# ebanalyse/ebnerd-benchmark

Hardware: AMD Instinct MI355X
Metric: training impressions/sec (higher is better)
Workload: dtype f32

## Files before the change

ebnerd-benchmark_amd/csrc/ebn_attention_mfma.hip:

```cpp
#include <stdlib.h>

#include "ebn_common.h"

namespace {

typedef float f32x16 __attribute__((ext_vector_type(16)));

constexpr int ATT_WAVES = 4;

struct MfmaAttnArgs {
  const float* qkv;
  int64_t ld_qkv;
  const float* dout;
  int64_t ld_dout;
  float* out;
  int64_t ld_out;
  int64_t n_prob;
  int32_t L, h;
  const uint32_t* key_ptr;
  uint32_t thresh;
  float scale;
  const float* pool_w;
  const float* pool_d;
  int64_t ld_pool;
// ... 268 lines not shown
  p.row0 = static_cast<int64_t>(p.seq) * L;
  return p;
}

template <int D>
__host__ __device__ constexpr int fwd_wave_floats(int L) {
  return L * Tile<D>::STRIDE > TP_FLOATS ? L * Tile<D>::STRIDE : TP_FLOATS;
}

template <int D, int LC>
__global__ __launch_bounds__(64 * ATT_WAVES) void attn_mfma_fwd_kernel(MfmaAttnArgs a) {
  extern __shared__ __attribute__((aligned(16))) float smem[];
  const int lane = threadIdx.x & 63;
  const int wv = __builtin_amdgcn_readfirstlane(threadIdx.x >> 6);
  const int64_t prob = static_cast<int64_t>(xcd_chunked_block()) * ATT_WAVES + wv;
  if (prob >= a.n_prob) return;
  const int L = LC ? LC : a.L, E = a.h * D;
  float* sv = smem + wv * fwd_wave_floats<D>(L);
  const int row = lane & 31, hi = lane >> 5;
  const float inv2 = 1.44269504088896341f / sqrtf(static_cast<float>(D));
  const bool drop = a.key_ptr != nullptr;
  const uint32_t key = drop ? *a.key_ptr : 0u;

  const AttnProb p = attn_prob(prob, a.h, L);
  const float* qb = a.qkv + p.row0 * a.ld_qkv + p.head * D;
  float qr[D / 2], kr[D / 2];
  {
    Staged<D> tv;
    stage_load<D>(tv, qb + 2 * E, a.ld_qkv, L, lane);
    global_row_form<D>(qr, qb, a.ld_qkv, L, row, hi);
    global_row_form<D>(kr, qb + E, a.ld_qkv, L, row, hi);
    stage_store<D, false>(sv, tv, L, lane, 0u, 0u, 0, 0u, 0.f);
  }
  wave_lds_sync();
  float vc[16];
  lds_col_form<D>(vc, sv, L, row, hi);

  f32x16 P = mm_rows<D / 2>(kr, qr);
  softmax_in_lane(P, L, hi, inv2);
  wave_lds_sync();
  tile_transpose(P, sv, L, row, hi);
  const f32x16 O = mm_col_tile(vc, P);
  float* ob = a.out + p.row0 * a.ld_out + p.head * D;
  const uint64_t e0 = static_cast<uint64_t>(p.row0) * E + p.head * D;
  if (drop) tile_rows_to_global<D, true>(ob, a.ld_out, O, L, row, hi, 1.0f, key, e0, E, a.thresh, a.scale);
  else tile_rows_to_global<D, false>(ob, a.ld_out, O, L, row, hi, 1.0f, 0u, 0u, 0, 0u, 0.f);
}

template <int D>
__host__ __device__ constexpr int fwd_group_v_offset(int L) {
  return 2 * L * Tile<D>::STRIDE > TP_FLOATS ? 2 * L * Tile<D>::STRIDE : TP_FLOATS;
}
__host__ __device__ constexpr int group_tile_pad(int L);
template <int D>
__host__ __device__ constexpr int fwd_group_wave_floats(int L) {
  return fwd_group_v_offset<D>(L) + L * Tile<D>::STRIDE + group_tile_pad(L);
}

template <int D, int LC, int G>
__global__ __launch_bounds__(64 * G) void attn_mfma_fwd_group_kernel(MfmaAttnArgs a) {
  using T = Tile<D>;
  constexpr int NT = 64 * G;
  constexpr int GV = G * T::VPR;
  constexpr int ROUNDS = (32 * GV + NT - 1) / NT;
  extern __shared__ __attribute__((aligned(16))) float smem[];
  const int tid = threadIdx.x;
  const int lane = tid & 63;
  const int wv = __builtin_amdgcn_readfirstlane(tid >> 6);
  const int L = LC ? LC : a.L, E = a.h * D;
  const int region = L * T::STRIDE;
  const int wave_floats = fwd_group_wave_floats<D>(L), v_off = fwd_group_v_offset<D>(L);
  const int row = lane & 31, hi = lane >> 5;
  const float inv2 = 1.44269504088896341f / sqrtf(static_cast<float>(D));
  const bool drop = a.key_ptr != nullptr;
  const uint32_t key = drop ? *a.key_ptr : 0u;

  const AttnProb p0 = attn_prob(static_cast<int64_t>(xcd_chunked_block()) * G, a.h, L);
  const uint32_t gcol = p0.head * D;
  const float* gq = a.qkv + p0.row0 * a.ld_qkv + gcol;
  const int nvec = L * GV;
  {
    float4 vq[ROUNDS], vk[ROUNDS], vv[ROUNDS];
    uint32_t dst[ROUNDS];
#pragma unroll
    for (int t = 0; t < ROUNDS; ++t) {
      const int idx = tid + NT * t;
      const int idc = idx < nvec ? idx : 0;
      const uint32_t r = static_cast<uint32_t>(idc) / static_cast<uint32_t>(GV), c4g = static_cast<uint32_t>(idc) - r * GV;
      const uint32_t head = c4g / T::VPR, c4 = c4g - head * T::VPR;
      dst[t] = head * wave_floats + r * T::STRIDE + c4 * 4;
      const uint32_t off = r * static_cast<uint32_t>(a.ld_qkv) + c4g * 4;
      vq[t] = *reinterpret_cast<const float4*>(gq + off);
      vk[t] = *reinterpret_cast<const float4*>(gq + E + off);
      vv[t] = *reinterpret_cast<const float4*>(gq + 2 * E + off);
    }
#pragma unroll
    for (int t = 0; t < ROUNDS; ++t) {
      if (tid + NT * t < nvec) {
        *reinterpret_cast<float4*>(smem + dst[t]) = vq[t];
        *reinterpret_cast<float4*>(smem + dst[t] + region) = vk[t];
        *reinterpret_cast<float4*>(smem + dst[t] + v_off) = vv[t];
      }
    }
  }
  __syncthreads();

  float* sq = smem + wv * wave_floats;
  float* sk = sq + region;
  float* sv = sq + v_off;
  f32x16 P;
  {
    float qr[D / 2], kr[D / 2];
    lds_row_form<D>(qr, sq, L, row, hi);
    lds_row_form<D>(kr, sk, L, row, hi);
    P = mm_rows<D / 2>(kr, qr);
  }
  float vc[16];
  lds_col_form<D>(vc, sv, L, row, hi);
  softmax_in_lane(P, L, hi, inv2);
  wave_lds_sync();
  tile_transpose(P, sq, L, row, hi);
  {
    const f32x16 O = mm_col_tile(vc, P);
    tile_rows_to_lds<D>(sv, O, L, row, hi, 1.0f);
  }
  __syncthreads();

  float* go = a.out + p0.row0 * a.ld_out + gcol;
#pragma unroll
  for (int t = 0; t < ROUNDS; ++t) {
    const int idx = tid + NT * t;
    if (idx < nvec) {
      const uint32_t r = static_cast<uint32_t>(idx) / static_cast<uint32_t>(GV), c4g = static_cast<uint32_t>(idx) - r * GV;
      const uint32_t head = c4g / T::VPR, c4 = c4g - head * T::VPR;
      float4 y = *reinterpret_cast<const float4*>(smem + head * wave_floats + v_off + r * T::STRIDE + c4 * 4);
      if (drop) {
        const uint64_t pr = ((static_cast<uint64_t>(p0.row0) * E + gcol) >> 1) + ((r * static_cast<uint32_t>(E) + c4g * 4) >> 1);
        const uint32_t h0 = ebn_dropout_pair_hash(key, pr), h1 = ebn_dropout_pair_hash(key, pr + 1);
        y.x *= ((h0 & 0xFFFFu) >= a.thresh) ? a.scale : 0.f;
        y.y *= ((h0 >> 16) >= a.thresh) ? a.scale : 0.f;
        y.z *= ((h1 & 0xFFFFu) >= a.thresh) ? a.scale : 0.f;
        y.w *= ((h1 >> 16) >= a.thresh) ? a.scale : 0.f;
      }
      *reinterpret_cast<float4*>(go + (r * static_cast<uint32_t>(a.ld_out) + c4g * 4)) = y;
    }
  }
}

template <int D>
__host__ __device__ constexpr int bwd_wave_floats(int L) {
  return 3 * L * Tile<D>::STRIDE > L * Tile<D>::STRIDE + TP_FLOATS ? 3 * L * Tile<D>::STRIDE : L * Tile<D>::STRIDE + TP_FLOATS;
}

template <int D, int LC>
__global__ __launch_bounds__(64 * ATT_WAVES) void attn_mfma_bwd_kernel(MfmaAttnArgs a) {
  using T = Tile<D>;
  constexpr int KH = D / 2;
  extern __shared__ __attribute__((aligned(16))) float smem[];
  const int lane = threadIdx.x & 63;
  const int wv = __builtin_amdgcn_readfirstlane(threadIdx.x >> 6);
  const int64_t prob = static_cast<int64_t>(xcd_chunked_block()) * ATT_WAVES + wv;
  if (prob >= a.n_prob) return;
  const int L = LC ? LC : a.L, E = a.h * D;
  const int region = L * T::STRIDE;
  float* sq = smem + wv * bwd_wave_floats<D>(L);
  float* sk = sq + region;
  float* sg = sk + region;
  const int row = lane & 31, hi = lane >> 5;
  const float inv = 1.0f / sqrtf(static_cast<float>(D));
  const float inv2 = inv * 1.44269504088896341f;
  const bool drop = a.key_ptr != nullptr, pooled = a.pool_w != nullptr;
  const uint32_t key = drop ? *a.key_ptr : 0u;

  const AttnProb p = attn_prob(prob, a.h, L);
  const float* qb = a.qkv + p.row0 * a.ld_qkv + p.head * D;
  float vr[KH];
  {
    Staged<D> tq, tk, tg;
    stage_load<D>(tq, qb, a.ld_qkv, L, lane);
    stage_load<D>(tk, qb + E, a.ld_qkv, L, lane);
    stage_load<D>(tg, a.dout + p.row0 * a.ld_dout + p.head * D, a.ld_dout, L, lane);
    global_row_form<D>(vr, qb + 2 * E, a.ld_qkv, L, row, hi);
    if (pooled) {
      PoolTerm<D> pt;
      pool_load<D>(pt, a.pool_w + p.row0, a.pool_d + p.seq * a.ld_pool + p.head * D, L, lane);
      pool_add<D>(tg, pt);
    }
    stage_store<D, false>(sq, tq, L, lane, 0u, 0u, 0, 0u, 0.f);
    stage_store<D, false>(sk, tk, L, lane, 0u, 0u, 0, 0u, 0.f);
    if (drop) stage_store<D, true>(sg, tg, L, lane, key, static_cast<uint64_t>(p.row0) * E + p.head * D, E, a.thresh, a.scale);
    else stage_store<D, false>(sg, tg, L, lane, 0u, 0u, 0, 0u, 0.f);
  }
  wave_lds_sync();

  float* ob = a.out + p.row0 * a.ld_out + p.head * D;
  f32x16 P, dP;
  {
    float qr[KH], kr[KH];
    lds_row_form<D>(qr, sq, L, row, hi);
    lds_row_form<D>(kr, sk, L, row, hi);
    P = mm_rows<KH>(kr, qr);
  }
  softmax_in_lane(P, L, hi, inv2);
  {
    float gr[KH];
    lds_row_form<D>(gr, sg, L, row, hi);
    dP = mm_rows<KH>(gr, vr);
  }
  float rowdot = 0.f;
#pragma unroll
  for (int r = 0; r < 16; ++r) rowdot = fmaf(P[r], dP[r], rowdot);
  rowdot += __shfl_xor(rowdot, 32, 64);

  float col[16];
  lds_col_form<D>(col, sg, L, row, hi);
  {
    const f32x16 dV = mm_col_tile(col, P);
    tile_rows_to_global<D, false>(ob + 2 * E, a.ld_out, dV, L, row, hi, 1.0f, 0u, 0u, 0, 0u, 0.f);
  }
#pragma unroll
  for (int r = 0; r < 16; ++r) P[r] = P[r] * (dP[r] - rowdot);
  lds_col_form<D>(col, sk, L, row, hi);
  {
    const f32x16 dQ = mm_col_tile(col, P);
    tile_rows_to_global<D, false>(ob, a.ld_out, dQ, L, row, hi, inv, 0u, 0u, 0, 0u, 0.f);
  }
  wave_lds_sync();
  tile_transpose(P, sk, L, row, hi);
  lds_col_form<D>(col, sq, L, row, hi);
  {
    const f32x16 dK = mm_col_tile(col, P);
    tile_rows_to_global<D, false>(ob + E, a.ld_out, dK, L, row, hi, inv, 0u, 0u, 0, 0u, 0.f);
  }
}


template <int D>
__host__ __device__ constexpr int bwd_group_g_offset(int L) {
  return 2 * L * Tile<D>::STRIDE > TP_FLOATS ? 2 * L * Tile<D>::STRIDE : TP_FLOATS;
}
__host__ __device__ constexpr int group_tile_pad(int L) { return L == 30 ? 12 : 0; }
template <int D>
__host__ __device__ constexpr int bwd_group_wave_floats(int L) {
  return bwd_group_g_offset<D>(L) + L * Tile<D>::STRIDE + group_tile_pad(L);
}

template <int D, int LC, int G>
__global__ __launch_bounds__(64 * G) void attn_mfma_bwd_group_kernel(MfmaAttnArgs a) {
  using T = Tile<D>;
  constexpr int KH = D / 2;
  constexpr int NT = 64 * G;
  constexpr int GV = G * T::VPR;
  constexpr int ROUNDS = (32 * GV + NT - 1) / NT;
  extern __shared__ __attribute__((aligned(16))) float smem[];
  const int tid = threadIdx.x;
  const int lane = tid & 63;
  const int wv = __builtin_amdgcn_readfirstlane(tid >> 6);
  const int L = LC ? LC : a.L, E = a.h * D;
  const int region = L * T::STRIDE;
  const int wave_floats = bwd_group_wave_floats<D>(L), g_off = bwd_group_g_offset<D>(L);
  const int row = lane & 31, hi = lane >> 5;
  const float inv = 1.0f / sqrtf(static_cast<float>(D));
  const float inv2 = inv * 1.44269504088896341f;
  const bool drop = a.key_ptr != nullptr, pooled = a.pool_w != nullptr;
  const uint32_t key = drop ? *a.key_ptr : 0u;

  stagger_first_round(a);
  const AttnProb p0 = attn_prob(static_cast<int64_t>(xcd_chunked_block()) * G, a.h, L);
  const uint32_t gcol = p0.head * D;
  const float* gq = a.qkv + p0.row0 * a.ld_qkv + gcol;
  const float* gd = a.dout + p0.row0 * a.ld_dout + gcol;
  const int nvec = L * GV;
  float vr[KH];
  global_row_form<D>(vr, gq + 2 * E + wv * D, a.ld_qkv, L, row, hi);
  {
    float4 vq[ROUNDS], vk[ROUNDS], vg[ROUNDS];
    uint32_t dst[ROUNDS];
#pragma unroll
    for (int t = 0; t < ROUNDS; ++t) {
      const int idx = tid + NT * t;
      const int idc = idx < nvec ? idx : 0;
      const uint32_t r = static_cast<uint32_t>(idc) / static_cast<uint32_t>(GV), c4g = static_cast<uint32_t>(idc) - r * GV;
      const uint32_t head = c4g / T::VPR, c4 = c4g - head * T::VPR;
      dst[t] = head * wave_floats + r * T::STRIDE + c4 * 4;
      const uint32_t off = r * static_cast<uint32_t>(a.ld_qkv) + c4g * 4;
      vq[t] = *reinterpret_cast<const float4*>(gq + off);
      vk[t] = *reinterpret_cast<const float4*>(gq + E + off);
      vg[t] = *reinterpret_cast<const float4*>(gd + (r * static_cast<uint32_t>(a.ld_dout) + c4g * 4));
      if (pooled) {
        const float w = a.pool_w[p0.row0 + r];
        const float4 pd = *reinterpret_cast<const float4*>(a.pool_d + p0.seq * a.ld_pool + gcol + c4g * 4);
        vg[t].x = fmaf(w, pd.x, vg[t].x);
        vg[t].y = fmaf(w, pd.y, vg[t].y);
        vg[t].z = fmaf(w, pd.z, vg[t].z);
        vg[t].w = fmaf(w, pd.w, vg[t].w);
      }
      if (drop) {
        const uint64_t pr = ((static_cast<uint64_t>(p0.row0) * E + gcol) >> 1) + ((r * static_cast<uint32_t>(E) + c4g * 4) >> 1);
        const uint32_t h0 = ebn_dropout_pair_hash(key, pr), h1 = ebn_dropout_pair_hash(key, pr + 1);
        vg[t].x *= ((h0 & 0xFFFFu) >= a.thresh) ? a.scale : 0.f;
        vg[t].y *= ((h0 >> 16) >= a.thresh) ? a.scale : 0.f;
        vg[t].z *= ((h1 & 0xFFFFu) >= a.thresh) ? a.scale : 0.f;
        vg[t].w *= ((h1 >> 16) >= a.thresh) ? a.scale : 0.f;
      }
    }
#pragma unroll
    for (int t = 0; t < ROUNDS; ++t) {
      if (tid + NT * t < nvec) {
        *reinterpret_cast<float4*>(smem + dst[t]) = vq[t];
        *reinterpret_cast<float4*>(smem + dst[t] + region) = vk[t];
        *reinterpret_cast<float4*>(smem + dst[t] + g_off) = vg[t];
      }
    }
  }
  __syncthreads();

  float* sq = smem + wv * wave_floats;
  float* sk = sq + region;
  float* sg = sq + g_off;
  f32x16 P, dP;
  {
    float qr[KH], kr[KH];
    lds_row_form<D>(qr, sq, L, row, hi);
    lds_row_form<D>(kr, sk, L, row, hi);
    P = mm_rows<KH>(kr, qr);
  }
  softmax_in_lane(P, L, hi, inv2);
  {
    float gr[KH];
    lds_row_form<D>(gr, sg, L, row, hi);
    dP = mm_rows<KH>(gr, vr);
  }
  float rowdot = 0.f;
#pragma unroll
  for (int r = 0; r < 16; ++r) rowdot = fmaf(P[r], dP[r], rowdot);
  rowdot += __shfl_xor(rowdot, 32, 64);

  float col[16], colq[16];
  lds_col_form<D>(col, sg, L, row, hi);
  lds_col_form<D>(colq, sq, L, row, hi);
  wave_lds_sync();
  {
    const f32x16 dV = mm_col_tile(col, P);
    tile_rows_to_lds<D>(sg, dV, L, row, hi, 1.0f);
  }
#pragma unroll
  for (int r = 0; r < 16; ++r) P[r] = P[r] * (dP[r] - rowdot);
  lds_col_form<D>(col, sk, L, row, hi);
  const f32x16 dQ = mm_col_tile(col, P);
  wave_lds_sync();
  tile_transpose(P, sq, L, row, hi);
  wave_lds_sync();
  tile_rows_to_lds<D>(sq, dQ, L, row, hi, inv);
  {
    const f32x16 dK = mm_col_tile(colq, P);
    tile_rows_to_lds<D>(sk, dK, L, row, hi, inv);
  }
  __syncthreads();

  float* go = a.out + p0.row0 * a.ld_out + gcol;
#pragma unroll
  for (int t = 0; t < ROUNDS; ++t) {
    const int idx = tid + NT * t;
    if (idx < nvec) {
      const uint32_t r = static_cast<uint32_t>(idx) / static_cast<uint32_t>(GV), c4g = static_cast<uint32_t>(idx) - r * GV;
      const uint32_t head = c4g / T::VPR, c4 = c4g - head * T::VPR;
      const float* src = smem + head * wave_floats + r * T::STRIDE + c4 * 4;
      const float4 q4 = *reinterpret_cast<const float4*>(src);
      const float4 k4 = *reinterpret_cast<const float4*>(src + region);
      const float4 v4 = *reinterpret_cast<const float4*>(src + g_off);
      float* d = go + (r * static_cast<uint32_t>(a.ld_out) + c4g * 4);
      *reinterpret_cast<float4*>(d) = q4;
      *reinterpret_cast<float4*>(d + E) = k4;
      *reinterpret_cast<float4*>(d + 2 * E) = v4;
    }
  }
}


constexpr int ATT2_WAVES = 2;
constexpr int NB2 = 2;

__device__ __forceinline__ void mm_col_tile_acc(f32x16& acc, const float (&a)[16], const f32x16& z) {
#pragma unroll
  for (int s = 0; s < 16; ++s) acc = __builtin_amdgcn_mfma_f32_32x32x2f32(a[s], z[s], acc, 0, 0, 0);
}
// ... 246 lines not shown
        const float rdi = __shfl(rowdot[ib], crow(r, hi), 64);
        P[r] = P[r] * (dP[r] - rdi);
      }
      float col[16];
      lds_col_form<D>(col, sq + 32 * ib * T::STRIDE, L - 32 * ib, row, hi);
      mm_col_tile_acc(dK, col, P);
    }
    wave_lds_sync();
    tile_rows_to_lds<D>(sv + 32 * jb * T::STRIDE, dK, L - 32 * jb, row, hi, inv);
    wave_lds_sync();
    stage_out<D, false>(sv + 32 * jb * T::STRIDE, ob + E + 32 * jb * a.ld_out, a.ld_out, L - 32 * jb, lane, 0u, 0u, 0, 0u, 0.f);
  }
}

}

constexpr int BWD_GROUP = 4;
constexpr int64_t FWD_GROUP_MIN_QKV_BYTES = 200'000'000;
constexpr int64_t BWD_GROUP_MIN_PROBLEMS = 4096;
static uint32_t stagger_shift_of_device() {
  static const uint32_t shift = [] {
    int dev = 0, cus = 0;
    if (hipGetDevice(&dev) != hipSuccess || hipDeviceGetAttribute(&cus, hipDeviceAttributeMultiprocessorCount, dev) != hipSuccess) return 0u;
    if (cus < 16 || (cus & (cus - 1)) != 0) return 0u;
    uint32_t s = 0;
    while ((1 << s) < cus) ++s;
    return s;
  }();
  return shift;
}

static bool bwd_group_off() {
  static const bool off = [] { const char* e = getenv("EBN_ATTN_BWD_PER_WAVE"); return e && e[0] == '1'; }();
  return off;
}

static bool mfma_path_ok(int32_t L, int32_t d, int64_t lda, int64_t ldb, int64_t ldc, const void* p0,
                         const void* p1, const void* p2) {
  if (L > 64 || !(d == 16 || d == 20 || d == 32)) return false;
  if ((lda % 4) || (ldb % 4) || (ldc % 4)) return false;
  if (lda >= (1 << 24) || ldb >= (1 << 24) || ldc >= (1 << 24)) return false;
  return ebn_aligned16(p0) && ebn_aligned16(p1) && ebn_aligned16(p2);
}

template <class K>
static void allow_lds(K kernel, size_t bytes) {
  if (bytes > 64 * 1024) (void)hipFuncSetAttribute(reinterpret_cast<const void*>(kernel), hipFuncAttributeMaxDynamicSharedMemorySize, static_cast<int>(bytes));
}

template <class K>
static void launch_waves(K kernel, size_t lds, const MfmaAttnArgs& a, hipStream_t s) {
#ifdef EBN_ATTN_EXP_PAD_LDS
  static const size_t pad = getenv("EBN_ATTN_PAD_LDS") ? static_cast<size_t>(atol(getenv("EBN_ATTN_PAD_LDS"))) : 0;
  lds += pad;
#endif
  allow_lds(kernel, lds);
  EBN_LAUNCH(kernel, dim3(static_cast<unsigned>(ebn_ceil_div(a.n_prob, ATT_WAVES))), dim3(64 * ATT_WAVES), lds, s, a);
}

template <int D, int LC>
static void launch_mfma2_lc(bool bwd, const MfmaAttnArgs& a, hipStream_t s) {
  const dim3 grid(static_cast<unsigned>(ebn_ceil_div(a.n_prob, ATT2_WAVES))), block(64 * ATT2_WAVES);
  const size_t lds = static_cast<size_t>(ATT2_WAVES) * (bwd ? 4 : 3) * a.L * Tile<D>::STRIDE * sizeof(float);
  if (bwd) {
    allow_lds(attn_mfma2_bwd_kernel<D, LC>, lds);
    EBN_LAUNCH((attn_mfma2_bwd_kernel<D, LC>), grid, block, lds, s, a);
  } else {
    allow_lds(attn_mfma2_fwd_kernel<D, LC>, lds);
    EBN_LAUNCH((attn_mfma2_fwd_kernel<D, LC>), grid, block, lds, s, a);
  }
}

template <int D>
static void launch_mfma2(bool bwd, const MfmaAttnArgs& a, hipStream_t s) {
  if (D == 20 && a.L == 50 && !bwd) launch_mfma2_lc<D, 50>(bwd, a, s);
  else launch_mfma2_lc<D, 0>(bwd, a, s);
}

int ebn_attn_mfma_fwd(const float* qkv, int64_t ld_qkv, float* out, int64_t ld_out, int64_t n_seq, int32_t L,
                      int32_t h, int32_t d, const EbnDrop& dr, hipStream_t s, bool* handled) {
  *handled = mfma_path_ok(L, d, ld_qkv, ld_out, ld_out, qkv, out, out) && n_seq * h < (int64_t{1} << 31);
  if (!*handled) return EBN_OK;
  MfmaAttnArgs a{qkv, ld_qkv, nullptr, 0, out, ld_out, n_seq * h, L, h, dr.key_ptr, dr.thresh, dr.scale, nullptr, nullptr, 0, 0u, 0u, 1u};
  if (L > 32) {
    if (d == 16) launch_mfma2<16>(false, a, s);
    else if (d == 20) launch_mfma2<20>(false, a, s);
    else launch_mfma2<32>(false, a, s);
    EBN_CHECK_LAUNCH();
    return EBN_OK;
  }
  const bool big = a.n_prob * L * 3 * d * static_cast<int64_t>(sizeof(float)) >= FWD_GROUP_MIN_QKV_BYTES;
  if (d == 20 && (h % BWD_GROUP) == 0 && big && !bwd_group_off()) {
    const size_t lds = static_cast<size_t>(BWD_GROUP) * fwd_group_wave_floats<20>(L) * sizeof(float);
    const dim3 grid(static_cast<unsigned>(a.n_prob / BWD_GROUP)), block(64 * BWD_GROUP);
    if (L == 30) {
      allow_lds(attn_mfma_fwd_group_kernel<20, 30, BWD_GROUP>, lds);
      EBN_LAUNCH((attn_mfma_fwd_group_kernel<20, 30, BWD_GROUP>), grid, block, lds, s, a);
    } else {
      allow_lds(attn_mfma_fwd_group_kernel<20, 0, BWD_GROUP>, lds);
      EBN_LAUNCH((attn_mfma_fwd_group_kernel<20, 0, BWD_GROUP>), grid, block, lds, s, a);
    }
    EBN_CHECK_LAUNCH();
    return EBN_OK;
  }
  const size_t wb = static_cast<size_t>(ATT_WAVES) * sizeof(float);
  if (d == 16) launch_waves(attn_mfma_fwd_kernel<16, 0>, wb * fwd_wave_floats<16>(L), a, s);
  else if (d == 20 && L == 30) launch_waves(attn_mfma_fwd_kernel<20, 30>, wb * fwd_wave_floats<20>(L), a, s);
  else if (d == 20 && L == 20) launch_waves(attn_mfma_fwd_kernel<20, 20>, wb * fwd_wave_floats<20>(L), a, s);
  else if (d == 20) launch_waves(attn_mfma_fwd_kernel<20, 0>, wb * fwd_wave_floats<20>(L), a, s);
  else launch_waves(attn_mfma_fwd_kernel<32, 0>, wb * fwd_wave_floats<32>(L), a, s);
  EBN_CHECK_LAUNCH();
  return EBN_OK;
}

int ebn_attn_mfma_bwd(const float* qkv, int64_t ld_qkv, const float* dout, int64_t ld_dout, float* dqkv,
                      int64_t ld_dqkv, int64_t n_seq, int32_t L, int32_t h, int32_t d, const EbnDrop& dr,
                      hipStream_t s, bool* handled, const float* pool_w, const float* pool_d, int64_t ld_pool) {
  *handled = mfma_path_ok(L, d, ld_qkv, ld_dout, ld_dqkv, qkv, dout, dqkv) && n_seq * h < (int64_t{1} << 31) &&
             (pool_w == nullptr || ((ld_pool % 4) == 0 && ebn_aligned16(pool_d)));
  if (!*handled) return EBN_OK;
  MfmaAttnArgs a{qkv, ld_qkv, dout, ld_dout, dqkv, ld_dqkv, n_seq * h, L, h, dr.key_ptr, dr.thresh, dr.scale, pool_w, pool_d, ld_pool, 0u, 0u, 1u};
  if (L > 32) {
    if (d == 16) launch_mfma2<16>(true, a, s);
    else if (d == 20) launch_mfma2<20>(true, a, s);
    else launch_mfma2<32>(true, a, s);
    EBN_CHECK_LAUNCH();
    return EBN_OK;
  }
  if (d == 20 && (h % BWD_GROUP) == 0 && a.n_prob >= BWD_GROUP_MIN_PROBLEMS && !bwd_group_off()) {
    const size_t lds = static_cast<size_t>(BWD_GROUP) * bwd_group_wave_floats<20>(L) * sizeof(float);
    const dim3 grid(static_cast<unsigned>(a.n_prob / BWD_GROUP)), block(64 * BWD_GROUP);
    a.stagger_shift = stagger_shift_of_device();
    a.stagger_units = a.stagger_shift != 0u ? 7u : 0u;
    a.stagger_mod = 5u;
    if (L == 30) {
      allow_lds(attn_mfma_bwd_group_kernel<20, 30, BWD_GROUP>, lds);
      EBN_LAUNCH((attn_mfma_bwd_group_kernel<20, 30, BWD_GROUP>), grid, block, lds, s, a);
    } else {
      allow_lds(attn_mfma_bwd_group_kernel<20, 0, BWD_GROUP>, lds);
      EBN_LAUNCH((attn_mfma_bwd_group_kernel<20, 0, BWD_GROUP>), grid, block, lds, s, a);
    }
    EBN_CHECK_LAUNCH();
    return EBN_OK;
  }
  const size_t wb = static_cast<size_t>(ATT_WAVES) * sizeof(float);
  if (d == 16) launch_waves(attn_mfma_bwd_kernel<16, 0>, wb * bwd_wave_floats<16>(L), a, s);
  else if (d == 20 && L == 30) launch_waves(attn_mfma_bwd_kernel<20, 30>, wb * bwd_wave_floats<20>(L), a, s);
  else if (d == 20 && L == 20) launch_waves(attn_mfma_bwd_kernel<20, 20>, wb * bwd_wave_floats<20>(L), a, s);
  else if (d == 20) launch_waves(attn_mfma_bwd_kernel<20, 0>, wb * bwd_wave_floats<20>(L), a, s);
  else launch_waves(attn_mfma_bwd_kernel<32, 0>, wb * bwd_wave_floats<32>(L), a, s);
  EBN_CHECK_LAUNCH();
  return EBN_OK;
}
```

ebnerd-benchmark_amd/csrc/ebn_encoder.hip:

```cpp
#include "ebn_common.h"

#define EBN_TRY(call)            \
  do {                           \
    int rc__ = (call);           \
    if (rc__ != EBN_OK) return rc__; \
  } while (0)

static int check_dims(const ebn_encoder_dims* d) {
  EBN_REQUIRE(d, EBN_ERR_BAD_ARG);
  EBN_REQUIRE(d->n_seq >= 0 && d->L > 0 && d->Din > 0 && d->h > 0 && d->d > 0 && d->A > 0, EBN_ERR_BAD_ARG);
  return EBN_OK;
}

extern "C" int ebn_encoder_fwd_f32(const ebn_encoder_dims* dims, const ebn_encoder_params* p,
                                   const ebn_encoder_acts* a, const ebn_encoder_scratch* s,
                                   const ebn_step_state* st, ebn_stream_t stream) {
  EBN_TRY(check_dims(dims));
  EBN_REQUIRE(p && a && p->Wqkv && p->W && p->b && p->q, EBN_ERR_BAD_ARG);
  EBN_REQUIRE(a->X && a->QKV && a->Y && a->U && a->w && a->out, EBN_ERR_BAD_ARG);
  const int64_t R = dims->n_seq * dims->L;
  const int E = dims->h * dims->d;
  if (R == 0) return EBN_OK;
  float* ws = s ? s->gemm_ws : nullptr;
  const int64_t ws_n = s ? s->gemm_ws_floats : 0;
  EBN_TRY(ebn_gemm_f32_site(0, 0, R, 3 * E, dims->Din, 1.0f, a->X, dims->Din, p->Wqkv, 3 * E, 0.0f, a->QKV, 3 * E, ws, ws_n,
                            1, stream));
  EBN_TRY(ebn_attn_fwd_f32(a->QKV, 3 * E, a->Y, E, dims->n_seq, dims->L, dims->h, dims->d, st, dims->drop_site,
                           dims->drop_p, stream));
  EBN_TRY(ebn_gemm_f32_ws(0, 0, R, dims->A, E, 1.0f, a->Y, E, p->W, dims->A, 0.0f, a->U, dims->A, ws, ws_n, stream));
  EBN_TRY(ebn_attpool_fwd_f32(a->U, p->b, p->q, a->Y, a->out, a->w, dims->n_seq, dims->L, E, dims->A, stream));
  return EBN_OK;
}

extern "C" int ebn_encoder_fwd_gather_f32(const ebn_encoder_dims* dims, const ebn_encoder_params* p, const ebn_encoder_acts* a,
                                          const ebn_encoder_scratch* s, const int32_t* ids, const float* table, int64_t table_rows,
                                          int32_t* oob_flag, ebn_stream_t stream) {
  EBN_TRY(check_dims(dims));
  EBN_REQUIRE(p && a && ids && table && p->Wqkv && p->W && p->b && p->q, EBN_ERR_BAD_ARG);
  EBN_REQUIRE(a->QKV && a->Y && a->U && a->w && a->out, EBN_ERR_BAD_ARG);
  EBN_REQUIRE(dims->drop_p <= 0.0f, EBN_ERR_UNSUPPORTED);
  const int64_t R = dims->n_seq * dims->L;
  const int E = dims->h * dims->d;
  if (R == 0) return EBN_OK;
  float* ws = s ? s->gemm_ws : nullptr;
  const int64_t ws_n = s ? s->gemm_ws_floats : 0;
  EBN_TRY(ebn_gemm_f32_rowmap(ids, table_rows, R, 3 * E, dims->Din, table, dims->Din, p->Wqkv, 3 * E, a->QKV, 3 * E, oob_flag, stream));
  EBN_TRY(ebn_attn_fwd_f32(a->QKV, 3 * E, a->Y, E, dims->n_seq, dims->L, dims->h, dims->d, nullptr, -1, 0.0f, stream));
  EBN_TRY(ebn_gemm_f32_ws(0, 0, R, dims->A, E, 1.0f, a->Y, E, p->W, dims->A, 0.0f, a->U, dims->A, ws, ws_n, stream));
  EBN_TRY(ebn_attpool_fwd_f32(a->U, p->b, p->q, a->Y, a->out, a->w, dims->n_seq, dims->L, E, dims->A, stream));
  return EBN_OK;
}

extern "C" int ebn_encoder_bwd_f32(const ebn_encoder_dims* dims, const ebn_encoder_params* p,
                                   const ebn_encoder_acts* a, const float* dout, const ebn_encoder_grads* g,
                                   const ebn_encoder_scratch* s, float* dX, int32_t accumulate,
                                   const ebn_step_state* st, ebn_stream_t stream) {
  EBN_TRY(check_dims(dims));
  EBN_REQUIRE(p && a && g && s && dout, EBN_ERR_BAD_ARG);
  EBN_REQUIRE(p->Wqkv && p->W && p->q, EBN_ERR_BAD_ARG);
  EBN_REQUIRE(a->X && a->QKV && a->Y && a->U && a->w, EBN_ERR_BAD_ARG);
  EBN_REQUIRE(g->dWqkv && g->dW && g->db && g->dq, EBN_ERR_BAD_ARG);
  EBN_REQUIRE(s->dY && s->dQKV && s->de && s->partials, EBN_ERR_BAD_ARG);
  const int64_t R = dims->n_seq * dims->L;
  const int E = dims->h * dims->d;
  const int A = dims->A;
  if (R == 0) return EBN_OK;
  const float beta = accumulate ? 1.0f : 0.0f;
  EBN_TRY(ebn_attpool_bwd_pool_f32(a->Y, a->w, dout, nullptr, s->de, dims->n_seq, dims->L, E, stream));
  EBN_TRY(ebn_attpool_bwd_dpre_f32(a->U, p->q, s->de, g->dq, g->db, s->partials, R, A, accumulate, stream));
  const bool fold = ebn_attn_bwd_pooled_supported(dims->L, dims->d) != 0 && (E % 4) == 0 && ebn_aligned16(dout) &&
                    ebn_aligned16(s->dY) && ebn_aligned16(a->QKV) && ebn_aligned16(s->dQKV);
  if (fold) {
    EBN_TRY(ebn_dense_bwd_pair_f32(R, E, A, a->Y, E, a->U, A, p->W, A, beta, g->dW, A, s->dY, E, s->gemm_ws, s->gemm_ws_floats,
                                   stream));
    EBN_TRY(ebn_attn_bwd_pooled_f32(a->QKV, 3 * E, s->dY, E, a->w, dout, E, s->dQKV, 3 * E, dims->n_seq, dims->L, dims->h,
                                    dims->d, st, dims->drop_site, dims->drop_p, stream));
  } else {
    EBN_TRY(ebn_gemm_f32_ws(1, 0, E, A, R, 1.0f, a->Y, E, a->U, A, beta, g->dW, A, s->gemm_ws, s->gemm_ws_floats, stream));
    EBN_TRY(ebn_gemm_f32_rank1(R, E, A, 1.0f, a->U, A, p->W, A, s->dY, E, a->w, dout, E, dims->L, s->gemm_ws,
                               s->gemm_ws_floats, stream));
    EBN_TRY(ebn_attn_bwd_f32(a->QKV, 3 * E, s->dY, E, s->dQKV, 3 * E, dims->n_seq, dims->L, dims->h, dims->d, st, dims->drop_site,
                             dims->drop_p, stream));
  }
  if (dX != nullptr)
    return ebn_dense_bwd_pair_f32(R, dims->Din, 3 * E, a->X, dims->Din, s->dQKV, 3 * E, p->Wqkv, 3 * E, beta, g->dWqkv, 3 * E, dX,
                                  dims->Din, s->gemm_ws, s->gemm_ws_floats, stream);
  EBN_TRY(ebn_gemm_f32_ws(1, 0, dims->Din, 3 * E, R, 1.0f, a->X, dims->Din, s->dQKV, 3 * E, beta, g->dWqkv, 3 * E,
                          s->gemm_ws, s->gemm_ws_floats, stream));
  return EBN_OK;
}

extern "C" int ebn_user_stage_train_f32(const ebn_encoder_dims* dims, const ebn_encoder_params* p, const ebn_encoder_acts* a,
                                        const float* cand, const float* labels, float* scores, float* probs, float* loss_rows,
                                        float* loss_out, float* dcand, float* duser, const ebn_encoder_grads* g,
                                        const ebn_encoder_scratch* s, float* head_partials, float* dX, int32_t C,
                                        int32_t loss_kind, float inv_batch, const ebn_step_state* st, ebn_stream_t stream) {
  EBN_TRY(check_dims(dims));
  EBN_REQUIRE(p && a && g && s && cand && labels && scores && probs && loss_rows && loss_out && dcand && duser && dX, EBN_ERR_BAD_ARG);
  EBN_REQUIRE(p->Wqkv && p->W && p->b && p->q && a->X && a->QKV && a->Y && a->U && a->w && a->out, EBN_ERR_BAD_ARG);
  EBN_REQUIRE(g->dWqkv && g->dW && g->db && g->dq && s->dY && s->dQKV && s->de && s->partials, EBN_ERR_BAD_ARG);
  EBN_REQUIRE(C > 0 && dims->drop_p <= 0.0f, EBN_ERR_BAD_ARG);
  const int64_t B = dims->n_seq, R = dims->n_seq * dims->L;
  const int E = dims->h * dims->d, A = dims->A, L = dims->L;
  if (R == 0) return EBN_OK;
  const bool fused = head_partials != nullptr && ebn_user_head_supported(L, C, E, A) != 0 &&
                     ebn_attn_bwd_pooled_supported(L, dims->d) != 0 && ebn_aligned16(a->U) && ebn_aligned16(a->Y) &&
                     ebn_aligned16(cand) && ebn_aligned16(dcand) && ebn_aligned16(duser) && ebn_aligned16(a->out) &&
                     ebn_aligned16(p->b) && ebn_aligned16(p->q) && ebn_aligned16(s->dY) && ebn_aligned16(a->QKV) &&
                     ebn_aligned16(s->dQKV);
  if (!fused) {
    EBN_TRY(ebn_encoder_fwd_f32(dims, p, a, s, st, stream));
    EBN_TRY(ebn_score_loss_train_f32(cand, a->out, labels, scores, probs, loss_rows, loss_out, dcand, duser, B, C, E, loss_kind,
                                     inv_batch, stream));
    return ebn_encoder_bwd_f32(dims, p, a, duser, g, s, dX, 0, st, stream);
  }
  float* ws = s->gemm_ws;
  const int64_t ws_n = s->gemm_ws_floats;
  EBN_TRY(ebn_gemm_f32_site(0, 0, R, 3 * E, dims->Din, 1.0f, a->X, dims->Din, p->Wqkv, 3 * E, 0.0f, a->QKV, 3 * E, ws, ws_n, 1, stream));
  EBN_TRY(ebn_attn_fwd_f32(a->QKV, 3 * E, a->Y, E, B, L, dims->h, dims->d, nullptr, -1, 0.0f, stream));
  EBN_TRY(ebn_gemm_f32_ws(0, 0, R, A, E, 1.0f, a->Y, E, p->W, A, 0.0f, a->U, A, ws, ws_n, stream));
  EBN_TRY(ebn_user_head_train_f32(a->U, p->b, p->q, a->Y, cand, labels, a->w, a->out, scores, probs, loss_rows, loss_out, dcand,
                                  duser, s->de, g->dq, g->db, head_partials, B, L, C, E, A, loss_kind, inv_batch, stream));
  EBN_TRY(ebn_dense_bwd_pair_f32(R, E, A, a->Y, E, a->U, A, p->W, A, 0.0f, g->dW, A, s->dY, E, ws, ws_n, stream));
  EBN_TRY(ebn_attn_bwd_pooled_f32(a->QKV, 3 * E, s->dY, E, a->w, duser, E, s->dQKV, 3 * E, B, L, dims->h, dims->d, nullptr, -1, 0.0f,
                                  stream));
  return ebn_dense_bwd_pair_f32(R, dims->Din, 3 * E, a->X, dims->Din, s->dQKV, 3 * E, p->Wqkv, 3 * E, 0.0f, g->dWqkv, 3 * E, dX,
                                dims->Din, ws, ws_n, stream);
}
```

ebnerd-benchmark_amd/csrc/ebn_gemm.hip:

```cpp
#include <stdlib.h>

#include "ebn_common.h"
#include "ebn_finish.h"
#include "ebn_tn_finale.h"

typedef float ebn_f32x4 __attribute__((ext_vector_type(4)));
typedef int ebn_i32x4 __attribute__((ext_vector_type(4)));
__device__ ebn_f32x4 ebn_raw_buffer_load_x4(ebn_i32x4 rsrc, int voffset, int soffset, int aux) __asm("llvm.amdgcn.raw.buffer.load.v4f32");
__device__ void ebn_raw_buffer_load_lds(ebn_i32x4 rsrc, __attribute__((address_space(3))) void* lds, int size, int voffset,
                                        int soffset, int offset, int aux) __asm("llvm.amdgcn.raw.buffer.load.lds");

int ebn_gemm_direct_tn_slices(int64_t M, int64_t N, int64_t K);
int ebn_gemm_direct_tn_launch(int64_t M, int64_t N, int64_t K, float alpha, const float* A, int64_t lda, const float* B, int64_t ldb,
                              float* part, hipStream_t s);
bool ebn_gemm_direct_wanted(int32_t transA, int32_t transB, int64_t M, int64_t N, int64_t K);
int ebn_gemm_direct_launch(int32_t transB, int64_t M, int64_t N, int64_t K, float alpha, const float* A, int64_t lda, const float* B,
                           int64_t ldb, float* C, int64_t ldc, hipStream_t s);

namespace {

typedef float f32x16 __attribute__((ext_vector_type(16)));


typedef float f32x4n __attribute__((ext_vector_type(4)));
// ... 728 lines not shown
        const bool okb__ = (B_KC ? (v__ % (SBK / 4)) * 4 : v__ / (T / 4)) < krem__;                     \
        const float4 ta__ = bload4(arsrc, oka__ ? oa[i] + sa__ : 0u, 0u);                                 \
        const float4 tb__ = bload4(brsrc, okb__ ? ob[i] + sb__ : 0u, 0u);                                 \
        ra[SET][i] = make_float4(oka__ ? ta__.x : 0.f, oka__ ? ta__.y : 0.f, oka__ ? ta__.z : 0.f, oka__ ? ta__.w : 0.f); \
        rb[SET][i] = make_float4(okb__ ? tb__.x : 0.f, okb__ ? tb__.y : 0.f, okb__ ? tb__.z : 0.f, okb__ ? tb__.w : 0.f); \
      }                                                                                                   \
    }                                                                                                     \
  } while (0)
#define EBN_SM_STORE(SET, BUF)                                            \
  do {                                                                    \
    small_store_t<A_KC, T>(smem_small + (BUF) * 2 * TILE, ra[SET], tid);       \
    small_store_t<B_KC, T>(smem_small + (BUF) * 2 * TILE + TILE, rb[SET], tid); \
    if (do_colsum) {                                                      \
      _Pragma("unroll") for (int i = 0; i < SPT; ++i) {                   \
        csum.x += rb[SET][i].x;                                           \
        csum.y += rb[SET][i].y;                                           \
        csum.z += rb[SET][i].z;                                           \
        csum.w += rb[SET][i].w;                                           \
      }                                                                   \
    }                                                                     \
  } while (0)
  const int r16 = lane & 15, kq = lane >> 4;
  const int ca0 = (4 * kq) ^ ((((wm * 16 + r16) >> 2) & 7) << 2), ca1 = ca0 ^ 16;
  const int cb0 = (4 * kq) ^ ((((wn * 16 + r16) >> 2) & 7) << 2), cb1 = cb0 ^ 16;
#define EBN_SM_READ(SET, g)                                                     \
  do {                                                                          \
    fa__[SET][0] = *reinterpret_cast<const float4*>(ap__ + 32 * (g) + ca0);     \
    fa__[SET][1] = *reinterpret_cast<const float4*>(ap__ + 32 * (g) + ca1);     \
    fb__[SET][0] = *reinterpret_cast<const float4*>(bp__ + 32 * (g) + cb0);     \
    fb__[SET][1] = *reinterpret_cast<const float4*>(bp__ + 32 * (g) + cb1);     \
  } while (0)
#define EBN_SM_MUL(SET)                                                                             \
  do {                                                                                              \
    acc0 = __builtin_amdgcn_mfma_f32_16x16x4f32(fa__[SET][0].x, fb__[SET][0].x, acc0, 0, 0, 0);     \
    acc1 = __builtin_amdgcn_mfma_f32_16x16x4f32(fa__[SET][0].y, fb__[SET][0].y, acc1, 0, 0, 0);     \
    acc2 = __builtin_amdgcn_mfma_f32_16x16x4f32(fa__[SET][0].z, fb__[SET][0].z, acc2, 0, 0, 0);     \
    acc3 = __builtin_amdgcn_mfma_f32_16x16x4f32(fa__[SET][0].w, fb__[SET][0].w, acc3, 0, 0, 0);     \
    acc0 = __builtin_amdgcn_mfma_f32_16x16x4f32(fa__[SET][1].x, fb__[SET][1].x, acc0, 0, 0, 0);     \
    acc1 = __builtin_amdgcn_mfma_f32_16x16x4f32(fa__[SET][1].y, fb__[SET][1].y, acc1, 0, 0, 0);     \
    acc2 = __builtin_amdgcn_mfma_f32_16x16x4f32(fa__[SET][1].z, fb__[SET][1].z, acc2, 0, 0, 0);     \
    acc3 = __builtin_amdgcn_mfma_f32_16x16x4f32(fa__[SET][1].w, fb__[SET][1].w, acc3, 0, 0, 0);     \
  } while (0)
#define EBN_SM_MMA(BUF, KT)                                                                                         \
  do {                                                                                                              \
    const float* ap__ = smem_small + (BUF) * 2 * TILE + (wm * 16 + r16) * SLV;                                      \
    const float* bp__ = smem_small + (BUF) * 2 * TILE + TILE + (wn * 16 + r16) * SLV;                               \
    float4 fa__[2][2], fb__[2][2];                                                                                  \
    if ((KT) < nk_full) {                                                                                           \
      EBN_SM_READ(0, 0);                                                                                            \
      EBN_SM_READ(1, 1);                                                                                            \
      __builtin_amdgcn_sched_barrier(0);      \
      EBN_SM_MUL(0);                                                                                                \
      __builtin_amdgcn_sched_barrier(0);                                                                            \
      EBN_SM_READ(0, 2);                                                                                            \
      __builtin_amdgcn_sched_barrier(0);                                                                            \
      EBN_SM_MUL(1);                                                                                                \
      __builtin_amdgcn_sched_barrier(0);                                                                            \
      EBN_SM_READ(1, 3);                                                                                            \
      __builtin_amdgcn_sched_barrier(0);                                                                            \
      EBN_SM_MUL(0);                                                                                                \
      EBN_SM_MUL(1);                                                                                                \
    } else {                                                                                                        \
      const int groups__ = static_cast<int>((K - static_cast<int64_t>(KT) * SBK + 31) / 32);                        \
      for (int g = 0; g < groups__; ++g) {                                                                          \
        EBN_SM_READ(0, g);                                                                                          \
        EBN_SM_MUL(0);                                                                                              \
      }                                                                                                             \
    }                                                                                                               \
  } while (0)
  EBN_SM_LOAD(0, 0);
  if (nk > 1) EBN_SM_LOAD(1, 1);
  EBN_SM_STORE(0, 0);
  __syncthreads();
  for (int kt = 0; kt < nk; kt += 2) {
    if (kt + 2 < nk) EBN_SM_LOAD(0, kt + 2);
    EBN_SM_MMA(0, kt);
    if (kt + 1 < nk) EBN_SM_STORE(1, 1);
    __syncthreads();
    if (kt + 1 >= nk) break;
    if (kt + 3 < nk) EBN_SM_LOAD(1, kt + 3);
    EBN_SM_MMA(1, kt + 1);
    if (kt + 2 < nk) EBN_SM_STORE(0, 0);
    __syncthreads();
  }
#undef EBN_SM_LOAD
#undef EBN_SM_STORE
#undef EBN_SM_MMA
#undef EBN_SM_READ
#undef EBN_SM_MUL
  const f32x4 acc = (acc0 + acc1) + (acc2 + acc3);
  if (do_colsum) {
    constexpr int CG = T / 4, KR = THREADS / CG;
    float* sc = smem_small;
    *reinterpret_cast<float4*>(&sc[(tid / CG) * (T + 4) + (tid % CG) * 4]) = csum;
    __syncthreads();
    if (tid < T && n0 + tid < N) {
      float t = 0.f;
      for (int r = 0; r < KR; ++r) t += sc[r * (T + 4) + tid];
      epi.colsum[n0 + tid] = t;
      if (FIN) ebn_adam_flat_apply(fin->adam, fin->adam.st->adam_alpha, (epi.colsum + n0 + tid) - fin->adam.grad, t);
    }
  }
  const int64_t col = n0 + wn * 16 + r16;
  if (col < N) {
    const float al = FIN ? fin->adam.st->adam_alpha : 0.f;
#pragma unroll
    for (int r = 0; r < 4; ++r) {
      const int64_t row = m0 + wm * 16 + 4 * kq + r;
      if (row >= M) continue;
      float v = alpha * acc[r];
      if (beta != 0.f) v += beta * C[row * ldc + col];
      if (epi.rs != nullptr)
        v = fmaf(epi.rs[row], epi.cv[static_cast<int64_t>(static_cast<uint32_t>(row) / static_cast<uint32_t>(epi.L)) * epi.ldcv + col], v);
      if (epi.bias != nullptr) v = fmaxf(v + epi.bias[col], 0.f);
      if (epi.l2w != nullptr) v = fmaf(epi.two_lambda, epi.l2w[row * ldc + col], v);
      C[row * ldc + col] = v;
      if (FIN) ebn_adam_flat_apply(fin->adam, al, (C + row * ldc + col) - fin->adam.grad, v);
    }
  }
}

template <bool TA, bool TB, int T>
__global__ __launch_bounds__(T * T / 4) void gemm_small_vec_kernel(int64_t M, int64_t N, int64_t K, float alpha,
                                                                      const float* __restrict__ A, int64_t lda,
                                                                      const float* __restrict__ B, int64_t ldb, float beta,
                                                                      float* __restrict__ C, int64_t ldc, GemmEpi epi) {
  small_vec_body<TA, TB, T>(M, N, K, alpha, A, lda, B, ldb, beta, C, ldc, epi, blockIdx.x, blockIdx.y);
}

struct SmallProblem {
  int64_t M, N, K;
  float alpha;
  const float* A;
  int64_t lda;
  const float* B;
  int64_t ldb;
  float beta;
  float* C;
  int64_t ldc;
  int32_t tiles_x, tiles;
};

__global__ __launch_bounds__(GEMM_THREADS) void gemm_small_pair_kernel(SmallProblem p0, SmallProblem p1) {
  const GemmEpi none{nullptr, nullptr, 0, 1, nullptr};
  const int b = blockIdx.x;
  if (b < p0.tiles)
    small_vec_body<true, false, 32>(p0.M, p0.N, p0.K, p0.alpha, p0.A, p0.lda, p0.B, p0.ldb, p0.beta, p0.C, p0.ldc, none,
                                    b % p0.tiles_x, b / p0.tiles_x);
  else
    small_vec_body<false, true, 32>(p1.M, p1.N, p1.K, p1.alpha, p1.A, p1.lda, p1.B, p1.ldb, p1.beta, p1.C, p1.ldc, none,
                                    (b - p0.tiles) % p1.tiles_x, (b - p0.tiles) / p1.tiles_x);
}

struct SmallGroup {
  SmallProblem p[EBN_TN_GROUP_MAX];
  float* colsum[EBN_TN_GROUP_MAX];
  const float* l2w[EBN_TN_GROUP_MAX];
  float two_lambda[EBN_TN_GROUP_MAX];
  int32_t first[EBN_TN_GROUP_MAX + 1];
  int32_t n;
};

__device__ __forceinline__ int xcd_chunked_tile(int v, int nwg) {
  const int q = nwg >> 3, r = nwg & 7, xcd = v & 7, idx = v >> 3;
  return ((xcd < r) ? xcd * (q + 1) : r * (q + 1) + (xcd - r) * q) + idx;
}

template <int T>
__global__ __launch_bounds__(T * T / 4) void gemm_small_tn_group_kernel(SmallGroup g) {
  const int b = xcd_chunked_tile(blockIdx.x, gridDim.x);
  int i = 0;
  while (i + 1 < g.n && b >= g.first[i + 1]) ++i;
  const SmallProblem& p = g.p[i];
  GemmEpi epi{nullptr, nullptr, 0, 1, nullptr};
  epi.colsum = g.colsum[i];
  epi.l2w = g.l2w[i];
  epi.two_lambda = g.two_lambda[i];
  const int t = b - g.first[i];
  small_vec_body<true, false, T>(p.M, p.N, p.K, p.alpha, p.A, p.lda, p.B, p.ldb, p.beta, p.C, p.ldc, epi, t % p.tiles_x, t / p.tiles_x);
}

static_assert(EBN_TN_FINALE_MAX_REST == EBN_DVN_FINALE_MAX_REST, "ebn_tn_finale.h / ebnerd_hip.h");
struct SmallGroupFin {
  SmallGroup g;
  EbnTnFinale f;
};

template <int T>
__global__ __launch_bounds__(T * T / 4) void gemm_small_tn_finale_kernel(SmallGroupFin gf) {
  extern __shared__ __attribute__((aligned(16))) float smem_small[];
  const SmallGroup& g = gf.g;
  const EbnTnFinale& f = gf.f;
  const int nwg = gridDim.x, tid = threadIdx.x, b = xcd_chunked_tile(blockIdx.x, nwg);
  constexpr int NT = T * T / 4;
  if (b < g.first[g.n]) {
    int i = 0;
    while (i + 1 < g.n && b >= g.first[i + 1]) ++i;
    const SmallProblem& p = g.p[i];
    GemmEpi epi{nullptr, nullptr, 0, 1, nullptr};
    epi.colsum = g.colsum[i];
    epi.l2w = g.l2w[i];
    epi.two_lambda = g.two_lambda[i];
    const int t = b - g.first[i];
    small_vec_body<true, false, T, true>(p.M, p.N, p.K, p.alpha, p.A, p.lda, p.B, p.ldb, p.beta, p.C, p.ldc, epi, t % p.tiles_x, t / p.tiles_x, &f);
  }
  const float al = f.adam.st->adam_alpha;
  {
    const int64_t per = (f.rest_total + nwg - 1) / nwg, e0 = static_cast<int64_t>(b) * per;
    const int64_t e1 = e0 + per < f.rest_total ? e0 + per : f.rest_total;
    for (int64_t e = e0 + tid; e < e1; e += NT) {
      int64_t off = e;
      int r = 0;
      while (r + 1 < f.n_rest && off >= f.rest_len[r]) off -= f.rest_len[r++];
      off += f.rest_off[r];
      ebn_adam_flat_apply(f.adam, al, off, f.adam.grad[off]);
    }
  }
  const int nh = (2 * f.A + 255) / 256 + 1;
  if (f.head_partials != nullptr && b < nh) {
    __syncthreads();
    ebn_user_head_finish_body(smem_small, b, nh, f.head_partials, f.B, f.A, f.dq, f.db, f.loss_rows, f.loss_out);
    if (b < nh - 1) {
      const int idx = b * 256 + tid;
      if (tid < 256 && idx < 2 * f.A) {
        const int sidx = idx / f.A, k = idx - sidx * f.A;
        float* gp = (sidx == 0 ? f.dq : f.db) + k;
        ebn_adam_flat_apply(f.adam, al, gp - f.adam.grad, *gp);
      }
    } else if (tid == 0 && f.n_l2 > 0) {
      float tot = 0.f;
      for (int l = 0; l < f.n_l2; ++l) {
        float tl = 0.f;
        for (int j = 0; j < f.l2_tiles[l]; ++j) tl += f.l2_part[l * f.l2_slots + j];
        tot += tl;
      }
      f.loss_out[0] += f.l2 * tot;
    }
  }
}

int launch_gemm_small(int transA, int transB, int64_t M, int64_t N, int64_t K, float alpha, const float* A, int64_t lda,
                      const float* B, int64_t ldb, float beta, float* C, int64_t ldc, int vecA, int vecB, hipStream_t s,
                      GemmEpi epi) {
  const dim3 grid(static_cast<unsigned>(ebn_ceil_div(N, SBN)), static_cast<unsigned>(ebn_ceil_div(M, SBM))), block(GEMM_THREADS);
  constexpr size_t lds = static_cast<size_t>(2) * 2 * SBM * SLD * sizeof(float);
#define EBN_SMALL_ONE(TA, TB, VA, VB)                                                                                     \
  do {                                                                                                                     \
    static const hipError_t attr__ = hipFuncSetAttribute(reinterpret_cast<const void*>(&gemm_small_kernel<TA, TB, VA, VB>), \
                                                         hipFuncAttributeMaxDynamicSharedMemorySize, static_cast<int>(lds)); \
    if (attr__ != hipSuccess) return static_cast<int>(attr__);                                                            \
    EBN_LAUNCH((gemm_small_kernel<TA, TB, VA, VB>), grid, block, lds, s, M, N, K, alpha, A, lda, B, ldb, beta, C, ldc, epi); \
  } while (0)
#define EBN_SMALL_VEC_T(TA, TB, T)                                                                                         \
  do {                                                                                                                     \
    constexpr size_t lds_t = static_cast<size_t>(2) * 2 * (T) * SLV * sizeof(float);                                       \
    static const hipError_t attr__ = hipFuncSetAttribute(reinterpret_cast<const void*>(&gemm_small_vec_kernel<TA, TB, T>), \
                                                         hipFuncAttributeMaxDynamicSharedMemorySize, static_cast<int>(lds_t)); \
    if (attr__ != hipSuccess) return static_cast<int>(attr__);                                                            \
    const dim3 grid_t(static_cast<unsigned>(ebn_ceil_div(N, T)), static_cast<unsigned>(ebn_ceil_div(M, T)));               \
    EBN_LAUNCH((gemm_small_vec_kernel<TA, TB, T>), grid_t, dim3((T) * (T) / 4), lds_t, s, M, N, K, alpha, A, lda, B, ldb, \
                       beta, C, ldc, epi);                                                                                 \
  } while (0)
#define EBN_SMALL_VEC(TA, TB) EBN_SMALL_VEC_T(TA, TB, 32)
  const bool fits32 = (K + SBK) * (transA ? lda : 1) * 4 + 64 * lda * 4 < (int64_t{1} << 31) &&
                      (K + SBK) * (transB ? 1 : ldb) * 4 + 64 * ldb * 4 < (int64_t{1} << 31);
#define EBN_SMALL(TA, TB)                              \
  do {                                                 \
    if (vecA && vecB && fits32) EBN_SMALL_VEC(TA, TB); \
    else EBN_SMALL_ONE(TA, TB, false, false);          \
  } while (0)
  if (!transA && !transB) EBN_SMALL(false, false);
  else if (!transA && transB) EBN_SMALL(false, true);
  else if (transA && !transB) EBN_SMALL(true, false);
  else EBN_SMALL(true, true);
#undef EBN_SMALL
#undef EBN_SMALL_VEC
#undef EBN_SMALL_VEC_T
#undef EBN_SMALL_ONE
  EBN_CHECK_LAUNCH();
  return EBN_OK;
}

}

struct GemmPlan {
  int bm, bn;
  int splits;
  int64_t kps;
  double cost;
};

static GemmPlan gemm_plan(int64_t M, int64_t N, int64_t K, int64_t ws_floats) {
  int64_t max_split = K / (4 * BK);
  if (max_split > 64) max_split = 64;
  const int64_t max_by_ws = (M * N > 0) ? ws_floats / (M * N) : 0;
  if (max_split > max_by_ws) max_split = max_by_ws;
  if (max_split < 1 || M * N >= (static_cast<int64_t>(1) << 31)) max_split = 1;
  static const struct {
    int bm, bn;
    double ts_full, ts_lone;
    int resident;
    int family;
  } kTiles[4] = {{128, 128, 1.15, 1.5, 3, 128}, {256, 64, 1.17, 1.5, 3, 256}, {64, 64, 0.32, 0.48, 4, 64}, {128, 64, 0.60, 0.8, 3, 96}};
  const double out_mb = static_cast<double>(M) * static_cast<double>(N) * 4e-6;
  GemmPlan best{128, 128, 1, ebn_ceil_div(K > 0 ? K : 1, BK) * BK, 1e300};
  {
// ... 102 lines not shown
    rc = launch_gemm<128, 64, 2>(transA, transB, M, N, K, alpha, A, lda, B, ldb, beta, C, ldc, vecA, vecB, splits, kps,
                                 workspace, s, site, epi);
  else if (plan.bm == 128)
    rc = launch_gemm<128, 128, 2>(transA, transB, M, N, K, alpha, A, lda, B, ldb, beta, C, ldc, vecA, vecB, splits, kps,
                                  workspace, s, site, epi);
  else
    rc = launch_gemm<64, 64, 2>(transA, transB, M, N, K, alpha, A, lda, B, ldb, beta, C, ldc, vecA, vecB, splits, kps,
                                workspace, s, site, epi);
  if (rc != EBN_OK) return rc;
  if (splits > 1 && defer_parts != nullptr) {
    *defer_parts = splits;
    return EBN_OK;
  }
  if (splits > 1) {
    int64_t grid = ebn_ceil_div(M * N, 256);
    if (grid > 4096) grid = 4096;
    EBN_LAUNCH(splitk_reduce_kernel, dim3(static_cast<unsigned>(grid)), dim3(256), 0, s, workspace,
                       splits, M, N, beta, C, ldc, epi);
    EBN_CHECK_LAUNCH();
  }
  return EBN_OK;
}

extern "C" int64_t ebn_gemm_partials_workspace_floats(int64_t M, int64_t N, int64_t K) {
  if (!ebn_dim_ok(M, N, K)) return 0;
  const GemmPlan p = gemm_plan(M, N, K, INT64_MAX / 4);
  int64_t slices = p.splits > 1 ? p.splits : 1;
  const int64_t tn = ebn_gemm_direct_tn_slices(M, N, K);
  if (tn > slices) slices = tn;
  return ebn_sat_mul(slices * M, N);
}

extern "C" int ebn_gemm_f32_partials(int32_t transA, int32_t transB, int64_t M, int64_t N, int64_t K, float alpha, const float* A,
                                     int64_t lda, const float* B, int64_t ldb, float* workspace, int64_t workspace_floats,
                                     int32_t* n_parts, ebn_stream_t stream) {
  EBN_REQUIRE(M > 0 && N > 0 && K >= 0 && n_parts, EBN_ERR_BAD_ARG);
  EBN_REQUIRE(A && B && workspace && workspace_floats >= M * N, EBN_ERR_BAD_ARG);
  EBN_REQUIRE(lda >= (transA ? M : K) && ldb >= (transB ? K : N), EBN_ERR_BAD_ARG);
  return gemm_dispatch(transA, transB, M, N, K, alpha, A, lda, B, ldb, 0.0f, workspace, N, workspace, workspace_floats, 0,
                       GemmEpi{nullptr, nullptr, 0, 1, nullptr}, ebn_stream(stream), n_parts);
}

extern "C" int ebn_gemm_f32_site(int32_t transA, int32_t transB, int64_t M, int64_t N, int64_t K, float alpha,
                                 const float* A, int64_t lda, const float* B, int64_t ldb, float beta, float* C,
                                 int64_t ldc, float* workspace, int64_t workspace_floats, int32_t site,
                                 ebn_stream_t stream) {
  EBN_REQUIRE(M >= 0 && N >= 0 && K >= 0, EBN_ERR_BAD_ARG);
  if (M == 0 || N == 0) return EBN_OK;
  EBN_REQUIRE(A && B && C, EBN_ERR_BAD_ARG);
  EBN_REQUIRE(lda >= (transA ? M : K) && ldb >= (transB ? K : N) && ldc >= N, EBN_ERR_BAD_ARG);
  return gemm_dispatch(transA, transB, M, N, K, alpha, A, lda, B, ldb, beta, C, ldc, workspace, workspace_floats, site,
                       GemmEpi{nullptr, nullptr, 0, 1, nullptr}, ebn_stream(stream));
}

namespace {
__global__ __launch_bounds__(256) void rank1_fill_kernel(float* __restrict__ C, int64_t ldc, int64_t M, int64_t N,
                                                         GemmEpi epi) {
  const int64_t total = M * N;
  for (int64_t i = static_cast<int64_t>(blockIdx.x) * 256 + threadIdx.x; i < total; i += static_cast<int64_t>(gridDim.x) * 256) {
    const int64_t row = i / N, col = i - row * N;
    C[row * ldc + col] = epi.rs[row] * epi.cv[(row / epi.L) * epi.ldcv + col];
  }
}
}

extern "C" int ebn_gemm_f32_rank1(int64_t M, int64_t N, int64_t K, float alpha, const float* A, int64_t lda,
                                  const float* B, int64_t ldb, float* C, int64_t ldc, const float* row_scale,
                                  const float* seq_rows, int64_t ld_seq, int32_t L, float* workspace,
                                  int64_t workspace_floats, ebn_stream_t stream) {
  EBN_REQUIRE(M >= 0 && N >= 0 && K >= 0 && L > 0, EBN_ERR_BAD_ARG);
  EBN_REQUIRE(M < (static_cast<int64_t>(1) << 31), EBN_ERR_UNSUPPORTED);
  if (M == 0 || N == 0) return EBN_OK;
  EBN_REQUIRE(A && B && C && row_scale && seq_rows, EBN_ERR_BAD_ARG);
  EBN_REQUIRE(lda >= K && ldb >= K && ldc >= N && ld_seq >= N, EBN_ERR_BAD_ARG);
  const GemmEpi epi{row_scale, seq_rows, ld_seq, L, nullptr};
  hipStream_t s = ebn_stream(stream);
  const bool vec = (lda % 4) == 0 && ebn_aligned16(A) && (ldb % 4) == 0 && ebn_aligned16(B) && (K % 4) == 0;
  if (vec)
    return gemm_dispatch(0, 1, M, N, K, alpha, A, lda, B, ldb, 0.0f, C, ldc, workspace, workspace_floats, 0, epi, s);
  int64_t grid = ebn_ceil_div(M * N, 256);
  if (grid > 4096) grid = 4096;
  EBN_LAUNCH(rank1_fill_kernel, dim3(static_cast<unsigned>(grid)), dim3(256), 0, s, C, ldc, M, N, epi);
  EBN_CHECK_LAUNCH();
  return gemm_dispatch(0, 1, M, N, K, alpha, A, lda, B, ldb, 1.0f, C, ldc, workspace, workspace_floats, 0,
                       GemmEpi{nullptr, nullptr, 0, 1, nullptr}, s);
}

extern "C" int ebn_dense_relu_fwd_f32(int64_t M, int64_t N, int64_t K, const float* A, int64_t lda, const float* B,
                                      int64_t ldb, const float* bias, float* C, int64_t ldc, float* workspace,
                                      int64_t workspace_floats, ebn_stream_t stream) {
  EBN_REQUIRE(M >= 0 && N >= 0 && K >= 0, EBN_ERR_BAD_ARG);
  if (M == 0 || N == 0) return EBN_OK;
  EBN_REQUIRE(A && B && C && bias, EBN_ERR_BAD_ARG);
  EBN_REQUIRE(lda >= K && ldb >= N && ldc >= N, EBN_ERR_BAD_ARG);
  hipStream_t s = ebn_stream(stream);
  const bool vec = (lda % 4) == 0 && ebn_aligned16(A) && (K % 4) == 0 && (ldb % 4) == 0 && ebn_aligned16(B) && (N % 4) == 0;
  if (vec)
    return gemm_dispatch(0, 0, M, N, K, 1.0f, A, lda, B, ldb, 0.0f, C, ldc, workspace, workspace_floats, 0,
                         GemmEpi{nullptr, nullptr, 0, 1, bias}, s);
  const int rc = gemm_dispatch(0, 0, M, N, K, 1.0f, A, lda, B, ldb, 0.0f, C, ldc, workspace, workspace_floats, 0,
                               GemmEpi{nullptr, nullptr, 0, 1, nullptr}, s);
  if (rc != EBN_OK) return rc;
  for (int64_t r = 0; ldc != N && r < M; ++r) {
    const int rr = ebn_bias_relu_f32(C + r * ldc, bias, C + r * ldc, 1, static_cast<int32_t>(N), stream);
    if (rr != EBN_OK) return rr;
  }
  return (ldc == N) ? ebn_bias_relu_f32(C, bias, C, M, static_cast<int32_t>(N), stream) : EBN_OK;
}

extern "C" int ebn_gemm_f32_ws(int32_t transA, int32_t transB, int64_t M, int64_t N, int64_t K, float alpha,
                               const float* A, int64_t lda, const float* B, int64_t ldb, float beta,
                               float* C, int64_t ldc, float* workspace, int64_t workspace_floats,
                               ebn_stream_t stream) {
  return ebn_gemm_f32_site(transA, transB, M, N, K, alpha, A, lda, B, ldb, beta, C, ldc, workspace, workspace_floats, 0,
                           stream);
}

extern "C" int ebn_dense_bwd_pair_f32(int64_t R, int64_t K_in, int64_t N_out, const float* X, int64_t ldx, const float* dY,
                                      int64_t lddy, const float* W, int64_t ldw, float beta_w, float* dW, int64_t lddw,
                                      float* dX, int64_t lddx, float* workspace, int64_t workspace_floats,
                                      ebn_stream_t stream) {
  EBN_REQUIRE(R >= 0 && K_in >= 0 && N_out >= 0, EBN_ERR_BAD_ARG);
  if (K_in == 0 || N_out == 0) return EBN_OK;
  EBN_REQUIRE(X && dY && W && dW && dX, EBN_ERR_BAD_ARG);
  EBN_REQUIRE(ldx >= K_in && lddy >= N_out && ldw >= N_out && lddw >= N_out && lddx >= K_in, EBN_ERR_BAD_ARG);
  hipStream_t s = ebn_stream(stream);
  const bool aligned = (ldx % 4) == 0 && (lddy % 4) == 0 && (ldw % 4) == 0 && ebn_aligned16(X) && ebn_aligned16(dY) &&
                       ebn_aligned16(W) && (K_in % 4) == 0 && (N_out % 4) == 0;
  const int64_t span = (R + SBK) * (ldx > lddy ? ldx : lddy) * 4 + 64 * ((ldx > lddy ? ldx : lddy) > ldw ? (ldx > lddy ? ldx : lddy) : ldw) * 4;
  const bool small = R > 0 && gemm_plan(K_in, N_out, R, workspace ? workspace_floats : 0).bm == 32 &&
                     gemm_plan(R, K_in, N_out, workspace ? workspace_floats : 0).bm == 32;
  if (aligned && small && span < (int64_t{1} << 31)) {
    SmallProblem p0{K_in, N_out, R, 1.0f, X, ldx, dY, lddy, beta_w, dW, lddw, static_cast<int32_t>(ebn_ceil_div(N_out, SBN)), 0};
    p0.tiles = p0.tiles_x * static_cast<int32_t>(ebn_ceil_div(K_in, SBM));
    SmallProblem p1{R, K_in, N_out, 1.0f, dY, lddy, W, ldw, 0.0f, dX, lddx, static_cast<int32_t>(ebn_ceil_div(K_in, SBN)), 0};
    p1.tiles = p1.tiles_x * static_cast<int32_t>(ebn_ceil_div(R, SBM));
    constexpr size_t lds = static_cast<size_t>(2) * 2 * SBM * SLV * sizeof(float);
    static const hipError_t attr = hipFuncSetAttribute(reinterpret_cast<const void*>(&gemm_small_pair_kernel),
                                                       hipFuncAttributeMaxDynamicSharedMemorySize, static_cast<int>(lds));
    if (attr != hipSuccess) return static_cast<int>(attr);
    EBN_LAUNCH(gemm_small_pair_kernel, dim3(static_cast<unsigned>(p0.tiles + p1.tiles)), dim3(GEMM_THREADS), lds, s, p0, p1);
    EBN_CHECK_LAUNCH();
    return EBN_OK;
  }
  const GemmEpi none{nullptr, nullptr, 0, 1, nullptr};
  if (R == 0) {
    return gemm_dispatch(1, 0, K_in, N_out, 0, 1.0f, X, ldx, dY, lddy, beta_w, dW, lddw, workspace, workspace_floats, 0, none, s);
  }
  const int rc = gemm_dispatch(1, 0, K_in, N_out, R, 1.0f, X, ldx, dY, lddy, beta_w, dW, lddw, workspace, workspace_floats, 0, none, s);
  if (rc != EBN_OK) return rc;
  return gemm_dispatch(0, 1, R, K_in, N_out, 1.0f, dY, lddy, W, ldw, 0.0f, dX, lddx, workspace, workspace_floats, 0, none, s);
}

extern "C" int ebn_gemm_f32_rowmap(const int32_t* ids, int64_t table_rows, int64_t M, int64_t N, int64_t K, const float* table,
                                   int64_t ldt, const float* B, int64_t ldb, float* C, int64_t ldc, int32_t* oob_flag, ebn_stream_t stream) {
  EBN_REQUIRE(ebn_dim_ok(M, N, K) && table_rows > 0, EBN_ERR_BAD_ARG);
  if (M == 0 || N == 0) return EBN_OK;
  EBN_REQUIRE(ids && table && B && C && ldt >= K && ldb >= N && ldc >= N && K > 0, EBN_ERR_BAD_ARG);
  const bool ok = M >= 256 && (ldt % 4) == 0 && (ldb % 4) == 0 && (K % 4) == 0 && (N % 4) == 0 && ebn_aligned16(table) && ebn_aligned16(B) &&
                  (table_rows * ldt + K + 16) * 4 < (int64_t{1} << 32) && ((K + 16) * ldb + 256) * 4 < (int64_t{1} << 32);
  if (!ok) return EBN_ERR_UNSUPPORTED;
  GemmEpi epi{nullptr, nullptr, 0, 1, nullptr};
  epi.rowmap = ids;
  epi.rowmap_rows = table_rows;
  epi.oob = oob_flag;
  return launch_gemm<256, 64, 4>(0, 0, M, N, K, 1.0f, table, ldt, B, ldb, 0.0f, C, ldc, 1, 1, 1, ebn_ceil_div(K, BK) * BK, nullptr,
                                 ebn_stream(stream), 0, epi);
}

extern "C" int ebn_gemm_tn_group_f32(const ebn_tn_problem* problems, int32_t n, ebn_stream_t stream) {
  EBN_REQUIRE(problems != nullptr && n >= 1 && n <= EBN_TN_GROUP_MAX, EBN_ERR_BAD_ARG);
  int64_t tiles64 = 0;
  for (int i = 0; i < n; ++i) {
    const ebn_tn_problem& q = problems[i];
    EBN_REQUIRE(ebn_dim_ok(q.M, q.N, q.K) && q.K >= 1, EBN_ERR_BAD_ARG);
    if (q.M == 0 || q.N == 0) continue;
    EBN_REQUIRE(q.A && q.B && q.C, EBN_ERR_BAD_ARG);
    EBN_REQUIRE(q.lda >= q.M && q.ldb >= q.N && q.ldc >= q.N, EBN_ERR_BAD_ARG);
    EBN_REQUIRE((q.lda % 4) == 0 && (q.ldb % 4) == 0 && (q.M % 4) == 0 && (q.N % 4) == 0 && ebn_aligned16(q.A) && ebn_aligned16(q.B),
                EBN_ERR_UNSUPPORTED);
    EBN_REQUIRE((q.K + SBK) * (q.lda > q.ldb ? q.lda : q.ldb) * 4 + 64 * 4 < (int64_t{1} << 31), EBN_ERR_UNSUPPORTED);
    tiles64 += ebn_ceil_div(q.M, 64) * ebn_ceil_div(q.N, 64);
  }
  const int T = tiles64 >= 192 ? 64 : 32;
  SmallGroup g{};
  int64_t total = 0;
  g.n = 0;
  for (int i = 0; i < n; ++i) {
    const ebn_tn_problem& q = problems[i];
    if (q.M == 0 || q.N == 0) continue;
    const int j = g.n++;
    g.p[j] = SmallProblem{q.M, q.N, q.K, 1.0f, q.A, q.lda, q.B, q.ldb, 0.0f, q.C, q.ldc, static_cast<int32_t>(ebn_ceil_div(q.N, T)), 0};
    g.p[j].tiles = g.p[j].tiles_x * static_cast<int32_t>(ebn_ceil_div(q.M, T));
    g.colsum[j] = q.colsum;
    g.l2w[j] = q.l2_W;
    g.two_lambda[j] = q.two_lambda;
    g.first[j] = static_cast<int32_t>(total);
    total += g.p[j].tiles;
    EBN_REQUIRE(total < (int64_t{1} << 30), EBN_ERR_UNSUPPORTED);
  }
  if (g.n == 0) return EBN_OK;
  g.first[g.n] = static_cast<int32_t>(total);
#define EBN_TN_GROUP(TT)                                                                                                          \
  do {                                                                                                                            \
    constexpr size_t lds = static_cast<size_t>(2) * 2 * (TT) * SLV * sizeof(float);                                               \
    static const hipError_t attr = hipFuncSetAttribute(reinterpret_cast<const void*>(&gemm_small_tn_group_kernel<TT>),            \
                                                       hipFuncAttributeMaxDynamicSharedMemorySize, static_cast<int>(lds));        \
    if (attr != hipSuccess) return static_cast<int>(attr);                                                                        \
    EBN_LAUNCH(gemm_small_tn_group_kernel<TT>, dim3(static_cast<unsigned>(total)), dim3((TT) * (TT) / 4), lds, ebn_stream(stream), g); \
  } while (0)
  if (T == 64) EBN_TN_GROUP(64);
  else EBN_TN_GROUP(32);
#undef EBN_TN_GROUP
  EBN_CHECK_LAUNCH();
  return EBN_OK;
}

int ebn_tn_group_finale_launch(const ebn_tn_problem* problems, int32_t n, const EbnTnFinale& fin, hipStream_t s) {
  EBN_REQUIRE(problems != nullptr && n >= 1 && n <= EBN_TN_GROUP_MAX, EBN_ERR_BAD_ARG);
  int64_t tiles64 = 0;
  for (int i = 0; i < n; ++i) {
    const ebn_tn_problem& q = problems[i];
    EBN_REQUIRE(ebn_dim_ok(q.M, q.N, q.K) && q.K >= 1 && q.M > 0 && q.N > 0, EBN_ERR_BAD_ARG);
    EBN_REQUIRE(q.A && q.B && q.C, EBN_ERR_BAD_ARG);
    EBN_REQUIRE(q.lda >= q.M && q.ldb >= q.N && q.ldc >= q.N, EBN_ERR_BAD_ARG);
    EBN_REQUIRE((q.lda % 4) == 0 && (q.ldb % 4) == 0 && (q.M % 4) == 0 && (q.N % 4) == 0 && ebn_aligned16(q.A) && ebn_aligned16(q.B),
                EBN_ERR_UNSUPPORTED);
    EBN_REQUIRE((q.K + SBK) * (q.lda > q.ldb ? q.lda : q.ldb) * 4 + 64 * 4 < (int64_t{1} << 31), EBN_ERR_UNSUPPORTED);
    tiles64 += ebn_ceil_div(q.M, 64) * ebn_ceil_div(q.N, 64);
  }
  const int T = tiles64 >= 192 ? 64 : 32;
  SmallGroupFin gf{};
  gf.f = fin;
  SmallGroup& g = gf.g;
  int64_t total = 0;
  g.n = n;
  for (int i = 0; i < n; ++i) {
    const ebn_tn_problem& q = problems[i];
    g.p[i] = SmallProblem{q.M, q.N, q.K, 1.0f, q.A, q.lda, q.B, q.ldb, 0.0f, q.C, q.ldc, static_cast<int32_t>(ebn_ceil_div(q.N, T)), 0};
    g.p[i].tiles = g.p[i].tiles_x * static_cast<int32_t>(ebn_ceil_div(q.M, T));
    g.colsum[i] = q.colsum;
    g.l2w[i] = q.l2_W;
    g.two_lambda[i] = q.two_lambda;
    g.first[i] = static_cast<int32_t>(total);
    total += g.p[i].tiles;
    EBN_REQUIRE(total < (int64_t{1} << 30), EBN_ERR_UNSUPPORTED);
  }
  g.first[n] = static_cast<int32_t>(total);
  const int64_t nh = (2 * static_cast<int64_t>(fin.A) + 255) / 256 + 1, nwg = total > nh ? total : nh;
#define EBN_TN_FINALE(TT)                                                                                                         \
  do {                                                                                                                            \
    constexpr size_t lds = static_cast<size_t>(2) * 2 * (TT) * SLV * sizeof(float);                                               \
    static const hipError_t attr = hipFuncSetAttribute(reinterpret_cast<const void*>(&gemm_small_tn_finale_kernel<TT>),           \
                                                       hipFuncAttributeMaxDynamicSharedMemorySize, static_cast<int>(lds));        \
    if (attr != hipSuccess) return static_cast<int>(attr);                                                                        \
    EBN_LAUNCH(gemm_small_tn_finale_kernel<TT>, dim3(static_cast<unsigned>(nwg)), dim3((TT) * (TT) / 4), lds, s, gf);             \
  } while (0)
  if (T == 64) EBN_TN_FINALE(64);
  else EBN_TN_FINALE(32);
#undef EBN_TN_FINALE
  EBN_CHECK_LAUNCH();
  return EBN_OK;
}

extern "C" int ebn_gemm_f32(int32_t transA, int32_t transB, int64_t M, int64_t N, int64_t K, float alpha,
                            const float* A, int64_t lda, const float* B, int64_t ldb, float beta, float* C,
                            int64_t ldc, ebn_stream_t stream) {
  return ebn_gemm_f32_ws(transA, transB, M, N, K, alpha, A, lda, B, ldb, beta, C, ldc, nullptr, 0, stream);
}
```

ebnerd-benchmark_amd/ebrec/models/newsrec/_engine.py:

```python
from __future__ import annotations

import ctypes
import math

import numpy as np
import torch

from ebrec import _hip

BETA1, BETA2, ADAM_EPS = 0.9, 0.999, 1e-7
_ALIGN = 64

from ._engine_segments import SegmentsMixin
from ._engine_staging import StagingMixin

LOSS_KIND = {"cross_entropy_loss": 0, "log_loss": 1}
BCE_ON = ("logits", "probs")


def loss_kind_of(loss: str, bce_on: str) -> int:
    if bce_on not in BCE_ON:
        raise ValueError(f"bce_on must be one of {BCE_ON}, got {bce_on}")
    return 0 if loss == "cross_entropy_loss" else (1 if bce_on == "logits" else 2)

# ... 2 lines not shown
    if not torch.cuda.is_available():
        raise RuntimeError("the MI355X NRMS path needs a visible GPU (no CPU fallback); "
                           "torch.cuda.is_available() is False")
    _hip.lib()
    return torch.device("cuda", torch.cuda.current_device())


def eval_loss_from_news(eng, news_all: torch.Tensor, his_idx, pred_idx, y):
    his_idx, pred_idx = np.asarray(his_idx), np.asarray(pred_idx)
    B, C = his_idx.shape[0], pred_idx.shape[1]
    H, E = his_idx.shape[1], eng.E
    idx = torch.from_numpy(np.ascontiguousarray(np.concatenate([his_idx.reshape(-1), pred_idx.reshape(-1)]), dtype=np.int32)).to(eng.device)
    NE = torch.empty(B * (H + C), E, device=eng.device)
    S = _hip.stream_handle
    _hip.call("ebn_gather_rows_f32", _hip.ptr(idx), _hip.ptr(news_all), _hip.ptr(NE), B * (H + C), E, news_all.shape[0], None, -1,
              ctypes.c_float(0.0), None, S())
    user = eng.encode_users_from_news(NE[: B * H].view(B, H, E))
    cand = NE[B * H:]
    scores, probs = torch.empty(B, C, device=eng.device), torch.empty(B, C, device=eng.device)
    _hip.call("ebn_score_fwd_f32", _hip.ptr(cand), _hip.ptr(user), _hip.ptr(scores), _hip.ptr(probs), B, C, E, 0, S())
    labels = (y if isinstance(y, torch.Tensor) else torch.from_numpy(np.ascontiguousarray(np.asarray(y, dtype=np.float32))))
    labels = labels.to(device=eng.device, dtype=torch.float32).reshape(B, C).contiguous()
    rows, junk_c, junk_u = torch.empty(B, device=eng.device), torch.empty(B * C, E, device=eng.device), torch.empty(B, E, device=eng.device)
    loss = torch.empty(1, device=eng.device)
    _hip.call("ebn_score_loss_bwd_f32", _hip.ptr(cand), _hip.ptr(user), _hip.ptr(scores), _hip.ptr(labels), _hip.ptr(rows),
              _hip.ptr(junk_c), _hip.ptr(junk_u), B, C, E, eng.loss_kind, ctypes.c_float(1.0 / B), S())
    _hip.call("ebn_sum_f32", _hip.ptr(rows), B, ctypes.c_float(1.0), _hip.ptr(loss), 0, S())
    return loss, probs


def glorot_uniform_np(shape, seed):
    rng = np.random.default_rng(seed)
    lim = math.sqrt(6.0 / (shape[0] + shape[-1]))
    return rng.uniform(-lim, lim, size=shape).astype(np.float32)


class FlatParams:

    def __init__(self, shapes: dict, device):
        self.shapes = dict(shapes)
        self.offsets = {}
        off = 0
        for name, shp in shapes.items():
            self.offsets[name] = off
            off += -(-int(np.prod(shp)) // _ALIGN) * _ALIGN
        self.numel = off
        self.data = torch.zeros(off, device=device)
        self.grad = torch.zeros(off, device=device)
        self.m = torch.zeros(off, device=device)
        self.v = torch.zeros(off, device=device)

    def view(self, name, buf=None):
        buf = self.data if buf is None else buf
        n = int(np.prod(self.shapes[name]))
        return buf[self.offsets[name]: self.offsets[name] + n].view(*self.shapes[name])

    def g(self, name):
        return self.view(name, self.grad)


class EncoderBuffers:

    def __init__(self, n_seq, L, Din, E, A, device, own_input, need_dx):
        R = n_seq * L
        self.n_seq, self.L, self.Din, self.E, self.A, self.R = n_seq, L, Din, E, A, R
        f = lambda *s: torch.empty(*s, device=device)
        self.X = f(R, Din) if own_input else None
        self.QKV, self.Y, self.U, self.w = f(R, 3 * E), f(R, E), f(R, A), f(R)
        self.out = f(n_seq, E)
        self.dY, self.dQKV, self.de = f(R, E), f(R, 3 * E), f(R)
        self.partials = f(int(_hip.lib().ebn_attpool_partials_len(R, A)))
        wsf = _hip.lib().ebn_gemm_workspace_floats
        ws = max(int(wsf(Din, 3 * E, R)), int(wsf(E, A, R)), int(wsf(R, 3 * E, Din)), int(wsf(R, A, E)), int(wsf(R, E, A)),
                 int(wsf(R, Din, 3 * E)), 1)
        self.ws = f(ws)
        self.fwd_scratch = _hip.EncoderScratch(None, None, None, None, self.ws.data_ptr(), self.ws.numel())
        self.dX = f(R, Din) if need_dx else None


class NRMSEngine(StagingMixin, SegmentsMixin):
    def __init__(self, table: np.ndarray, title_size: int, history_size: int, head_num: int, head_dim: int,
                 attention_hidden_dim: int, dropout: float, learning_rate: float, loss: str, seed=None,
                 train_embedding: bool = True, device=None, process_group=None, shard_table: bool = False,
                 shard_mode: str = "alltoall", deterministic: bool = True, units=None, l2: float = 0.0,
                 shard_partition: str | None = None, shard_capacity_factor: float = 1.25, table_grad_exchange: str = "auto",
                 bce_on: str = "logits", precision: str = "exact"):
        self.device = require_gpu() if device is None else torch.device(device)
        if precision not in ("exact", "split"):
            raise ValueError(f"precision must be 'exact' (fp32 MFMA, the default) or 'split' (bf16x6 split on the bf16 matrix pipe, "
                             f"fp32-accurate, fp32 accumulate), got {precision}")
        self.precision = precision
        if loss not in LOSS_KIND:
            raise ValueError(f"this loss not defined {loss}")
        loss_kind_of(loss, bce_on)
        self.bce_on = bce_on
        self.T, self.H = int(title_size), int(history_size)
        self.h, self.d, self.A = int(head_num), int(head_dim), int(attention_hidden_dim)
        self.E = self.h * self.d
        self.p = float(dropout)
        self.loss = loss
        self.seed = seed
        self.train_embedding = bool(train_embedding)
        if table_grad_exchange not in ("auto", "dense", "sparse"):
            raise ValueError(f"table_grad_exchange must be auto | dense | sparse, got {table_grad_exchange}")
        self.table_grad_exchange = table_grad_exchange
        self._sparse_pin = None
        self.pg = process_group
        table = np.ascontiguousarray(table, dtype=np.float32)
        self.V, self.D = table.shape
        self.exchange = None
        if shard_table:
            from ._dist import ShardedTableExchange

            self.exchange = ShardedTableExchange(self.V, self.D, group=process_group, mode=shard_mode, partition=shard_partition,
                                                 capacity_factor=shard_capacity_factor)
            table = self.exchange.shard_of(table)
        self.table = torch.from_numpy(np.ascontiguousarray(table)).to(self.device)
        D, E, A = self.D, self.E, self.A
        self.units = [int(u) for u in units] if units else []
        if self.units and self.precision == "split":
            raise ValueError("precision='split' covers the news encoder without the optional per-token Dense stack "
                             "(newsencoder_units_per_layer); use precision='exact' with it")
        if self.units and self.units[-1] != E:
            raise ValueError(f"newsencoder_units_per_layer must end with head_num*head_dim = {E} (the news vector is dotted with "
                             f"the {E}-wide user vector, nrms.py:201), got {self.units}")
        shapes = {"n_Wqkv": (D, 3 * E)}
        if self.units:
            from ._mlp import MLPStack

            shapes.update(MLPStack.shapes("n_", E, self.units))
        shapes.update({"n_W": (E, A), "n_b": (A,), "n_q": (A,), "u_Wqkv": (E, 3 * E), "u_W": (E, A), "u_b": (A,), "u_q": (A,)})
        self.params = FlatParams(shapes, self.device)
        self._graphs = {}
        self.mlp = MLPStack(self.params, "n_", E, self.units, self.device, l2, on_realloc=lambda: self._graphs.clear()) if self.units else None
        self._init_weights(seed)
        self.deterministic = bool(deterministic)
        if self.train_embedding:
            self.table_grad = torch.zeros_like(self.table)
            self.table_m = torch.zeros_like(self.table)
            self.table_v = torch.zeros_like(self.table)
            if self.deterministic:
                self.table_acc = torch.zeros(self.table.shape, dtype=torch.int64, device=self.device)
        st = _hip.StepState()
        st.step, st.seed, st.lr, st.adam_alpha = 0, (0 if seed is None else int(seed)) & 0xFFFFFFFF, learning_rate, 0.0
        self.state = torch.frombuffer(bytearray(bytes(st)), dtype=torch.uint8).to(self.device)
        self._lr = float(learning_rate)
        self._bufs = {}
        self.oob_flag = torch.zeros(1, dtype=torch.int32, device=self.device)
        self.keep_table_grad = False
        self.range_flag = torch.zeros(1, dtype=torch.int32, device=self.device)
        self.loss_dev = torch.zeros(1, device=self.device)
        self.use_graph = False
        self.fuse_user_head = True
        self.fuse_eval_gather = True
        self.defer_finish = True
        self.atomic_table_grad = False
        self.graph_collectives = False
        self.overlap_collectives = True
        self.skip_collectives = False
        self._pending = []
        self.defer_flag_checks = False
        self.trace = None
        self.world = 1
        if process_group is not None or (torch.distributed.is_available() and torch.distributed.is_initialized()):
            self.world = torch.distributed.get_world_size(process_group)
        self.guard = None
        if self.world > 1:
            from ._dist import LockStepGuard

            self.guard = LockStepGuard(process_group)
        self.force_collectives = False
        self.adam_in_finish = True
        self._adam_done_in_finish = False

    @property
    def multi(self) -> bool:
        return self.world > 1 or self.force_collectives

    @property
    def loss_kind(self) -> int:
        return loss_kind_of(self.loss, self.bce_on)

    def _init_weights(self, seed):
        D, E, A = self.D, self.E, self.A
        s = (lambda: seed) if seed is not None else (lambda: None)
        pv = self.params.view
        with torch.no_grad():
            for pre, din in (("n", D), ("u", E)):
                w = np.concatenate([glorot_uniform_np((din, E), s()) for _ in range(3)], axis=1)
                pv(f"{pre}_Wqkv").copy_(torch.from_numpy(w))
                pv(f"{pre}_W").copy_(torch.from_numpy(glorot_uniform_np((E, A), s())))
                pv(f"{pre}_b").zero_()
                pv(f"{pre}_q").copy_(torch.from_numpy(glorot_uniform_np((A, 1), s())[:, 0]))
        if self.mlp is not None:
            self.mlp.init_weights((lambda k: None) if seed is None else (lambda k: int(seed) * 1000 + k), glorot_uniform_np)

    def weight_names(self):
        base = ["news.emb", "news.attn.WQ", "news.attn.WK", "news.attn.WV"]
        if self.mlp is not None:
            base += self.mlp.weight_names("news")
        return base + ["news.att.W", "news.att.b", "news.att.q", "user.attn.WQ", "user.attn.WK", "user.attn.WV", "user.att.W",
                       "user.att.b", "user.att.q"]

    def get_weights(self):
        E = self.E
        out = [self._full_table().cpu().numpy()]
        for pre in ("n", "u"):
            w = self.params.view(f"{pre}_Wqkv").cpu().numpy()
            out += [w[:, :E].copy(), w[:, E:2 * E].copy(), w[:, 2 * E:].copy()]
            if pre == "n" and self.mlp is not None:
                out += self.mlp.get_weights()
            out += [self.params.view(f"{pre}_W").cpu().numpy(), self.params.view(f"{pre}_b").cpu().numpy(),
                    self.params.view(f"{pre}_q").cpu().numpy().reshape(-1, 1)]
        return out

    def set_weights(self, weights):
        n_mlp = 6 * len(self.units)
        if len(weights) != 13 + n_mlp:
            raise ValueError(f"expected {13 + n_mlp} weight arrays (emb, 2x[WQ,WK,WV,W,b,q]{' + 6 per Dense/BN layer' if n_mlp else ''}), "
                             f"got {len(weights)}")
        w = [np.asarray(a, dtype=np.float32) for a in weights]
        if n_mlp:
            self.mlp.set_weights([torch.from_numpy(np.ascontiguousarray(a)) for a in w[4:4 + n_mlp]])
            w = w[:4] + w[4 + n_mlp:]
        if w[0].shape != (self.V, self.D):
            raise ValueError(f"embedding shape {w[0].shape} != {(self.V, self.D)}")
        with torch.no_grad():
            t0 = w[0] if self.exchange is None else self.exchange.shard_of(w[0])
            self.table.copy_(torch.from_numpy(np.ascontiguousarray(t0)))
            i = 1
            for pre in ("n", "u"):
                self.params.view(f"{pre}_Wqkv").copy_(torch.from_numpy(np.concatenate(w[i:i + 3], axis=1)))
                self.params.view(f"{pre}_W").copy_(torch.from_numpy(w[i + 3]))
                self.params.view(f"{pre}_b").copy_(torch.from_numpy(w[i + 4].reshape(-1)))
                self.params.view(f"{pre}_q").copy_(torch.from_numpy(w[i + 5].reshape(-1)))
                i += 6

    def _full_table(self) -> torch.Tensor:
        if self.exchange is None or self.exchange.world == 1:
            return self.table
        per = self.exchange.per
        mine = torch.zeros(per, self.D, device=self.device)
        mine[: self.table.shape[0]] = self.table
        parts = [torch.empty_like(mine) for _ in range(self.exchange.world)]
        torch.distributed.all_gather(parts, mine, group=self.pg)
        return self.exchange.unshard(parts)

    def count_params(self):
        return self.V * self.D + sum(int(np.prod(s)) for s in self.params.shapes.values()) + 2 * sum(self.units)

    @property
    def _planned(self) -> bool:
        return self.exchange is not None and self.exchange.mode == "alltoall"

    @property
    def _adam_from_acc(self) -> bool:
        return (self.train_embedding and self.deterministic and self.exchange is None and not self.multi
                and not self.keep_table_grad)

    def _sparse_dp(self, n_tok: int) -> bool:
        if not (self.multi and self.train_embedding and self.exchange is None and self.deterministic and not self.keep_table_grad):
            return False
        if self.table_grad_exchange != "auto":
            return self.table_grad_exchange == "sparse"
        return self.pin_table_grad_exchange(n_tok)

    def pin_table_grad_exchange(self, n_tok_full: int) -> bool:
        if self._sparse_pin is None:
            self._sparse_pin = bool(self.world * int(n_tok_full) < self.V)
        return self._sparse_pin

    @property
    def needs_equal_batches(self) -> bool:
        if self.world <= 1:
            return False
        if self.exchange is not None:
            return True
        if not (self.train_embedding and self.deterministic and not self.keep_table_grad):
            return False
        if self.table_grad_exchange != "auto":
            return self.table_grad_exchange == "sparse"
        return True if self._sparse_pin is None else self._sparse_pin

    @property
    def graph_capable(self) -> bool:
        return self.exchange is None or self._planned

    def allreduce_bytes(self, n_tok: int = 0) -> int:
        n = self.params.numel * 4
        if self.train_embedding and self.exchange is None:
            n += n_tok * (4 + self.D * 4) if self._sparse_dp(n_tok) else self.table_grad.numel() * 4
        return n

    def enable_graphs(self, flag=True):
        self.use_graph = bool(flag)
        if not flag:
            self._graphs = {}
        return self

    @property
    def learning_rate(self):
        return self._lr

    @learning_rate.setter
    def learning_rate(self, lr):
        self._lr = float(lr)
# ... 394 lines not shown
        pred = pred if isinstance(pred, torch.Tensor) else np.asarray(pred)
        B, C = his.shape[0], pred.shape[1]
        advanced = False
        if indexed:
            if his.ndim != 2 or his.shape[1] != self.H or pred.ndim != 2 or pred.shape[0] != B:
                raise ValueError(f"indexed batches must be (B, {self.H}) and (B, C), got {tuple(his.shape)} {tuple(pred.shape)}")
            nb, ub = self._train_bufs(B, C)
            y, advanced = self._stage_indexed(nb, his, pred, y)
        else:
            self._check_shapes(his, pred)
            nb, ub = self._train_bufs(B, C)
            if self._device_batch(his, pred, y):
                nh = his.numel()
                _hip.call("ebn_copy3_advance", _hip.ptr(his), _hip.ptr(nb.ids), nh * 4, _hip.ptr(pred), _hip.ptr(nb.ids[nh:]),
                          pred.numel() * 4, _hip.ptr(y), _hip.ptr(nb.labels), y.numel() * 4, _hip.ptr(self.state), BETA1, BETA2,
                          _hip.stream_handle())
                y, advanced = None, True
            elif not isinstance(his, torch.Tensor) and not isinstance(pred, torch.Tensor) and not isinstance(y, torch.Tensor):
                for a in (his, pred):
                    if a.size and (a.min() < 0 or a.max() >= self.V):
                        raise IndexError(f"token id out of range [0, {self.V}) for the embedding table")
                self._stage_host([his, pred], nb.ids, y, nb.labels)
                y, advanced = None, True
            else:
                self._upload_ids(nb.ids, his, pred)
        if y is not None:
            labels = (y if isinstance(y, torch.Tensor) else torch.from_numpy(np.ascontiguousarray(np.asarray(y, dtype=np.float32))))
            nb.labels[: B * C].copy_(labels.reshape(-1).to(device=self.device, dtype=torch.float32), non_blocking=True)
        if self.use_graph and self.graph_capable:
            key = self._graph_key(B, C, advanced)
            run = self._graphs.get(key)
            if run is None:
                run = self._capture(B, C, advanced)
            if self.trace is not None:
                self.trace.run(run, self._graph_desc.get(key, []))
            else:
                for fn in run:
                    fn()
        elif self.trace is not None:
            segs = self._segments(B, C, advanced)
            self.trace.run([fn for _kind, fn in segs], [self.SEG_KINDS.get(kind, kind) + (f": {fn.what}" if hasattr(fn, "what") else "") for kind, fn in segs])
        else:
            for _kind, fn in self._segments(B, C, advanced):
                fn()
        if return_probs:
            return self.loss_dev, nb.probs[: B * C].view(B, C), nb.labels[: B * C].view(B, C)
        return self.loss_dev

    def _train_bufs(self, B, C):
        N, E = B * (self.H + C), self.E
        nb = self._news_bufs(N, True)
        ub = self._user_bufs(B, True)
        if not hasattr(nb, "dNE"):
            nb.dNE = torch.empty(nb.n_seq, E, device=self.device)
            nb.scores = torch.empty(nb.n_seq, device=self.device)
            nb.probs = torch.empty(nb.n_seq, device=self.device)
            nb.labels = torch.empty(nb.n_seq, device=self.device)
        if self._deferred(C):
            self._defer_bufs(nb)
        if not hasattr(ub, "duser"):
            ub.duser = torch.empty(ub.n_seq, E, device=self.device)
            ub.loss_rows = torch.empty(ub.n_seq, device=self.device)
            ub.head_partials = torch.empty(max(int(_hip.lib().ebn_user_head_partials_len(ub.n_seq, self.A)), 1), device=self.device)
        return nb, ub

    SEG_KINDS = {"k": "kernels", "c": "collective", "a": "collective started asynchronously", "w": "wait for the started collectives"}

    def _fwd_bwd_kernels(self, B, C, sparse_table_grads=False, part="all"):
        H, E = self.H, self.E
        N = B * (H + C)
        S = _hip.stream_handle
        nb, ub = self._train_bufs(B, C)
        st = _hip.ptr(self.state)
        site1, p1 = (1, self.p) if self.p > 0 else (-1, 0.0)
        deferred = self._deferred(C)
        if part in ("all", "a"):
            self._adam_done_in_finish = False
        if part == "b":
            if deferred:
                return self._news_bwd_deferred(nb, ub, B, N, "p2")
            return self._news_bwd_p2(nb, N, nb.X, nb.dNE, site1, p1)
        if part in ("all", "a"):
            if deferred:
                self._news_forward(nb, N, True, B * H, looked_up=True)
                self._user_stage_deferred(B, C, nb, ub)
            else:
                self._fwd_user_stage_kernels(B, C, nb, ub)
        if part == "a":
            if deferred:
                return self._news_bwd_deferred(nb, ub, B, N, "p1")
            return self._news_bwd_p1(nb, N, nb.dNE)
        if part == "all" and deferred:
            self._news_bwd_deferred(nb, ub, B, N, "p1")
            self._adam_done_in_finish = self._adam_fused(C)
            if self._adam_done_in_finish:
                self._news_bwd_deferred(nb, ub, B, N, "p2a")
                if nb.dX is not None:
                    self._news_bwd_p3(nb, N, nb.dX)
                self._news_bwd_deferred(nb, ub, B, N, "p2b")
            else:
                self._news_bwd_deferred(nb, ub, B, N, "p2")
                if nb.dX is not None:
                    self._news_bwd_p3(nb, N, nb.dX)
        elif part == "all":
            self._encoder_bwd("n", nb, N, nb.X, nb.dNE, nb.dX, B * H)
        elif nb.dX is not None:
            self._news_bwd_p3(nb, N, nb.dX)
        self._table_grad_kernels(nb, N, sparse_table_grads)

    def _deferred(self, C) -> bool:
        L = _hip.lib()
        return bool(self.defer_finish and self.mlp is None and self.precision == "exact" and self.fuse_user_head
                    and self._fold_pooling(self.T) and self._fold_pooling(self.H)
                    and int(L.ebn_user_head_supported(self.H, C, self.E, self.A)) != 0)

    def _adam_fused(self, C) -> bool:
        return bool(self.adam_in_finish and not self.multi and self._deferred(C))

    def _adam_flat_args(self):
        a = getattr(self, "_adam_flat", None)
        if a is None:
            P = self.params
            a = _hip.AdamFlat()
            a.theta, a.grad, a.m, a.v, a.numel = P.data.data_ptr(), P.grad.data_ptr(), P.m.data_ptr(), P.v.data_ptr(), P.numel
            a.beta1, a.beta2, a.eps, a.grad_scale = BETA1, BETA2, ADAM_EPS, 1.0
            rest = sorted((P.offsets[k], int(np.prod(P.shapes[k]))) for k in ("u_Wqkv", "u_W"))
            a.n_rest = len(rest)
            for i, (off, n) in enumerate(rest):
                a.rest_off[i], a.rest_len[i] = off, n
            self._adam_flat = a
        return a

    def _defer_bufs(self, nb):
        if getattr(nb, "ws_dw", None) is None:
            L = _hip.lib()
            nb.ws_dw = torch.empty(max(int(L.ebn_gemm_partials_workspace_floats(self.E, self.A, nb.R)), 1), device=self.device)
            nb.ws_dwqkv = torch.empty(max(int(L.ebn_gemm_partials_workspace_floats(self.D, 3 * self.E, nb.R)), 1), device=self.device)
            nb.finish_jobs = {}
        return nb

    def _user_stage_deferred(self, B, C, nb, ub):
        S, H, E, A = _hip.stream_handle, self.H, self.E, self.A
        R = B * H
        pv, g = self.params.view, self.params.g
        ws, wsn = _hip.ptr(ub.ws), ub.ws.numel()
        one, zero = ctypes.c_float(1.0), ctypes.c_float(0.0)
        X, cand, dcand = nb.out, nb.out[B * H:], nb.dNE[B * H:]
        _hip.call("ebn_gemm_f32_site", 0, 0, R, 3 * E, E, one, _hip.ptr(X), E, _hip.ptr(pv("u_Wqkv")), 3 * E, zero, _hip.ptr(ub.QKV), 3 * E, ws, wsn, 1, S())
        _hip.call("ebn_attn_fwd_f32", _hip.ptr(ub.QKV), 3 * E, _hip.ptr(ub.Y), E, B, H, self.h, self.d, None, -1, zero, S())
        _hip.call("ebn_gemm_f32_ws", 0, 0, R, A, E, one, _hip.ptr(ub.Y), E, _hip.ptr(pv("u_W")), A, zero, _hip.ptr(ub.U), A, ws, wsn, S())
        _hip.call("ebn_user_head_train_f32", _hip.ptr(ub.U), _hip.ptr(pv("u_b")), _hip.ptr(pv("u_q")), _hip.ptr(ub.Y), _hip.ptr(cand), _hip.ptr(nb.labels),
                  _hip.ptr(ub.w), _hip.ptr(ub.out), _hip.ptr(nb.scores), _hip.ptr(nb.probs), _hip.ptr(ub.loss_rows), _hip.ptr(self.loss_dev), _hip.ptr(dcand),
                  _hip.ptr(ub.duser), _hip.ptr(ub.de), None, None, _hip.ptr(ub.head_partials), B, H, C, E, A, self.loss_kind, ctypes.c_float(1.0 / B), S())
        _hip.call("ebn_dense_bwd_pair_f32", R, E, A, _hip.ptr(ub.Y), E, _hip.ptr(ub.U), A, _hip.ptr(pv("u_W")), A, zero, _hip.ptr(g("u_W")), A,
                  _hip.ptr(ub.dY), E, ws, wsn, S())
        _hip.call("ebn_attn_bwd_pooled_f32", _hip.ptr(ub.QKV), 3 * E, _hip.ptr(ub.dY), E, _hip.ptr(ub.w), _hip.ptr(ub.duser), E, _hip.ptr(ub.dQKV), 3 * E,
                  B, H, self.h, self.d, None, -1, zero, S())
        _hip.call("ebn_dense_bwd_pair_f32", R, E, 3 * E, _hip.ptr(X), E, _hip.ptr(ub.dQKV), 3 * E, _hip.ptr(pv("u_Wqkv")), 3 * E, zero, _hip.ptr(g("u_Wqkv")),
                  3 * E, _hip.ptr(nb.dNE), E, ws, wsn, S())

    def _news_bwd_deferred(self, nb, ub, B, N, part):
        S, E, A, T, D = _hip.stream_handle, self.E, self.A, self.T, self.D
        R = N * T
        pv, g = self.params.view, self.params.g
        one, zero = ctypes.c_float(1.0), ctypes.c_float(0.0)
        L = _hip.lib()
        self._defer_bufs(nb)
        if part == "p1":
            _hip.call("ebn_attpool_bwd_pool_f32", _hip.ptr(nb.Y), _hip.ptr(nb.w), _hip.ptr(nb.dNE), None, _hip.ptr(nb.de), N, T, E, S())
            _hip.call("ebn_attpool_bwd_dpre_f32", _hip.ptr(nb.U), _hip.ptr(pv("n_q")), _hip.ptr(nb.de), None, None, _hip.ptr(nb.partials), R, A, 0, S())
            n = ctypes.c_int32(0)
            _hip.call("ebn_gemm_f32_partials", 1, 0, E, A, R, one, _hip.ptr(nb.Y), E, _hip.ptr(nb.U), A, _hip.ptr(nb.ws_dw), nb.ws_dw.numel(), ctypes.byref(n), S())
            nb.finish_jobs["dW"] = int(n.value)
            _hip.call("ebn_gemm_f32_ws", 0, 1, R, E, A, one, _hip.ptr(nb.U), A, _hip.ptr(pv("n_W")), A, zero, _hip.ptr(nb.dY), E, _hip.ptr(nb.ws), nb.ws.numel(), S())
            return
        site, p = (1, self.p) if self.p > 0 else (-1, 0.0)
        if part in ("p2", "p2a"):
            _hip.call("ebn_attn_bwd_pooled_f32", _hip.ptr(nb.QKV), 3 * E, _hip.ptr(nb.dY), E, _hip.ptr(nb.w), _hip.ptr(nb.dNE), E, _hip.ptr(nb.dQKV), 3 * E,
                      N, T, self.h, self.d, _hip.ptr(self.state), site, ctypes.c_float(p), S())
            n = ctypes.c_int32(0)
            _hip.call("ebn_gemm_f32_partials", 1, 0, D, 3 * E, R, one, _hip.ptr(nb.X), D, _hip.ptr(nb.dQKV), 3 * E, _hip.ptr(nb.ws_dwqkv), nb.ws_dwqkv.numel(),
                      ctypes.byref(n), S())
            nb.finish_jobs["dWqkv"] = int(n.value)
            if part == "p2a":
                return
        jobs = (_hip.FinishJob * 4)()
        jobs[0] = _hip.FinishJob(_hip.FINISH_COLRED, int(L.ebn_attpool_partials_len(R, A)) // (2 * A), 1, A, nb.partials.data_ptr(), g("n_q").data_ptr(),
                                 g("n_b").data_ptr(), A, 0.0, 1.0, None, None)
        jobs[1] = _hip.FinishJob(_hip.FINISH_HEAD, 1, B, A, ub.head_partials.data_ptr(), g("u_q").data_ptr(), g("u_b").data_ptr(), A, 0.0, 1.0,
                                 ub.loss_rows.data_ptr(), self.loss_dev.data_ptr())
        jobs[2] = _hip.FinishJob(_hip.FINISH_SPLITK, nb.finish_jobs["dW"], E, A, nb.ws_dw.data_ptr(), g("n_W").data_ptr(), None, A, 0.0, 1.0, None, None)
        jobs[3] = _hip.FinishJob(_hip.FINISH_SPLITK, nb.finish_jobs["dWqkv"], D, 3 * E, nb.ws_dwqkv.data_ptr(), g("n_Wqkv").data_ptr(), None, 3 * E, 0.0, 1.0, None, None)
        if part == "p2b":
            _hip.call("ebn_grad_finish_adam_f32", jobs, 4, ctypes.byref(self._adam_flat_args()), _hip.ptr(self.state), S())
        else:
            _hip.call("ebn_grad_finish_f32", jobs, 4, S())

    def _fwd_user_stage_kernels(self, B, C, nb, ub):
        H, E = self.H, self.E
        N = B * (H + C)
        S = _hip.stream_handle
        st = _hip.ptr(self.state)
        self._news_forward(nb, N, True, B * H, looked_up=True)
        cand, dcand = nb.out[B * H:], nb.dNE[B * H:]
        dims, params, acts = self._enc_structs("u", ub, B, nb.out, -1, 0.0)
        g = self.params.g
        grads = _hip.EncoderGrads(g("u_Wqkv").data_ptr(), g("u_W").data_ptr(), g("u_b").data_ptr(), g("u_q").data_ptr())
        scratch = _hip.EncoderScratch(ub.dY.data_ptr(), ub.dQKV.data_ptr(), ub.de.data_ptr(), ub.partials.data_ptr(),
                                      ub.ws.data_ptr(), ub.ws.numel())
        _hip.call("ebn_user_stage_train_f32", ctypes.byref(dims), ctypes.byref(params), ctypes.byref(acts), _hip.ptr(cand),
                  _hip.ptr(nb.labels), _hip.ptr(nb.scores), _hip.ptr(nb.probs), _hip.ptr(ub.loss_rows), _hip.ptr(self.loss_dev),
                  _hip.ptr(dcand), _hip.ptr(ub.duser), ctypes.byref(grads), ctypes.byref(scratch),
                  _hip.ptr(ub.head_partials) if self.fuse_user_head else None, _hip.ptr(nb.dNE), C, self.loss_kind,
                  ctypes.c_float(1.0 / B), st, S())

    def _accumulate_fixed(self, ids, dX, n_tok, st, site, p):
        _hip.call("ebn_embedding_grad_scatter_fixed_atomic" if self.atomic_table_grad else "ebn_embedding_grad_scatter_fixed", _hip.ptr(ids),
                  _hip.ptr(dX), _hip.ptr(self.table_acc), n_tok, self.D, self.V, st, site, ctypes.c_float(p), _hip.ptr(self.range_flag),
                  _hip.stream_handle())

    def _table_grad_kernels(self, nb, N, sparse_table_grads):
        S = _hip.stream_handle
        st = _hip.ptr(self.state)
        if self.train_embedding and not self._planned and not sparse_table_grads:
            if self.exchange is not None or not self.deterministic:
                self.table_grad.zero_()
            site, p = (0, self.p) if self.p > 0 else (-1, 0.0)
            if self.exchange is not None:
                d_uniq = torch.zeros_like(nb.rows_uniq)
                _hip.call("ebn_embedding_grad_scatter_f32", _hip.ptr(nb.plan.inv), _hip.ptr(nb.dX), _hip.ptr(d_uniq),
                          N * self.T, self.D, d_uniq.shape[0], st, site, ctypes.c_float(p), S())
                self.exchange.scatter_grads(nb.plan, d_uniq, self._local_scatter_add)
            elif self.deterministic:
                self._accumulate_fixed(nb.ids, nb.dX, N * self.T, st, site, p)
                if not self._adam_from_acc:
                    _hip.call("ebn_fixed_to_f32", _hip.ptr(self.table_acc), _hip.ptr(self.table_grad), self.table.numel(),
                              _hip.ptr(self.range_flag), S())
            else:
                _hip.call("ebn_embedding_grad_scatter_f32", _hip.ptr(nb.ids), _hip.ptr(nb.dX), _hip.ptr(self.table_grad),
                          N * self.T, self.D, self.V, st, site, ctypes.c_float(p), S())

    def _optimizer_kernels(self, from_acc=None):
        from_acc = self._adam_from_acc if from_acc is None else from_acc
        S = _hip.stream_handle
        st = _hip.ptr(self.state)
        gs = ctypes.c_float(1.0 / self.world)
        P = self.params
        if not self._adam_done_in_finish:
            _hip.call("ebn_adam_keras_step_f32", _hip.ptr(P.data), _hip.ptr(P.grad), _hip.ptr(P.m), _hip.ptr(P.v), P.numel,
                      st, BETA1, BETA2, ADAM_EPS, gs, S())
        if self.train_embedding and from_acc:
            _hip.call("ebn_adam_keras_step_fixed_f32", _hip.ptr(self.table), _hip.ptr(self.table_acc), _hip.ptr(self.table_m),
                      _hip.ptr(self.table_v), self.table.numel(), st, BETA1, BETA2, ADAM_EPS, gs, _hip.ptr(self.range_flag), S())
        elif self.train_embedding:
            _hip.call("ebn_adam_keras_step_f32", _hip.ptr(self.table), _hip.ptr(self.table_grad), _hip.ptr(self.table_m),
                      _hip.ptr(self.table_v), self.table.numel(), st, BETA1, BETA2, ADAM_EPS, gs, S())
```

ebnerd-benchmark_amd/ebrec/models/newsrec/_engine_docvec.py:

```python
from __future__ import annotations

import ctypes

import numpy as np
import torch

from ebrec import _hip

from ._engine import ADAM_EPS, BETA1, BETA2, LOSS_KIND, loss_kind_of, EncoderBuffers, FlatParams, glorot_uniform_np, require_gpu
from ._mlp import MLPStack


class DocVecEngine:
    def __init__(self, doc_dim: int, units, history_size: int, head_num: int, head_dim: int, attention_hidden_dim: int,
                 dropout: float, learning_rate: float, loss: str, l2: float, seed=None, device=None, process_group=None,
                 bce_on: str = "logits"):
        self.device = require_gpu() if device is None else torch.device(device)
        if loss not in LOSS_KIND:
            raise ValueError(f"this loss not defined {loss}")
        loss_kind_of(loss, bce_on)
        self.bce_on = bce_on
        self.Din, self.units, self.H = int(doc_dim), [int(u) for u in (units or [])], int(history_size)
        self.h, self.d, self.A = int(head_num), int(head_dim), int(attention_hidden_dim)
        self.E = self.h * self.d
        self.p, self.loss, self.l2, self.seed, self.pg = float(dropout), loss, float(l2), seed, process_group
        E, A = self.E, self.A
        shapes = MLPStack.shapes("", self.Din, self.units)
        prev = self.units[-1] if self.units else self.Din
        shapes.update({"out_W": (prev, E), "out_b": (E,), "u_Wqkv": (E, 3 * E), "u_W": (E, A), "u_b": (A,), "u_q": (A,)})
        self.params = FlatParams(shapes, self.device)
        self.use_graph, self._graphs = False, {}
        self.fuse_user_head = True
        self.fuse_news_mlp = True
        self.fuse_finale = True
        self._dvn_dirty = False
        self.mlp = MLPStack(self.params, "", self.Din, self.units, self.device, self.l2, on_realloc=lambda: self._graphs.clear())
        self.bn_mean, self.bn_var = self.mlp.bn_mean, self.mlp.bn_var
        self._init_weights(seed)
        st = _hip.StepState()
        st.step, st.seed, st.lr, st.adam_alpha = 0, (0 if seed is None else int(seed)) & 0xFFFFFFFF, learning_rate, 0.0
        self.state = torch.frombuffer(bytearray(bytes(st)), dtype=torch.uint8).to(self.device)
        self._lr = float(learning_rate)
        self._bufs = {}
        self.loss_dev = torch.zeros(1, device=self.device)
        self.reg_dev = torch.zeros(1, device=self.device)
        self.range_flag = torch.zeros(1, dtype=torch.int32, device=self.device)
        self.world = 1
        if process_group is not None or (torch.distributed.is_available() and torch.distributed.is_initialized()):
            self.world = torch.distributed.get_world_size(process_group)
        self.guard = None
        if self.world > 1:
            from ._dist import LockStepGuard

            self.guard = LockStepGuard(process_group)
        self.force_collectives = False

    @property
    def multi(self) -> bool:
        return self.world > 1 or self.force_collectives

    @property
    def loss_kind(self) -> int:
        return loss_kind_of(self.loss, self.bce_on)

    def _init_weights(self, seed):
        rng_seed = (lambda k: None) if seed is None else (lambda k: int(seed) * 1000 + k)
        pv = self.params.view
        self.mlp.init_weights(rng_seed, glorot_uniform_np)
        with torch.no_grad():
            prev = self.mlp.out_dim
            pv("out_W").copy_(torch.from_numpy(glorot_uniform_np((prev, self.E), rng_seed(99))))
            s = (lambda: seed) if seed is not None else (lambda: None)
            pv("u_Wqkv").copy_(torch.from_numpy(np.concatenate([glorot_uniform_np((self.E, self.E), s()) for _ in range(3)], 1)))
            pv("u_W").copy_(torch.from_numpy(glorot_uniform_np((self.E, self.A), s())))
            pv("u_q").copy_(torch.from_numpy(glorot_uniform_np((self.A, 1), s())[:, 0]))

    def weight_names(self):
        return self.mlp.weight_names("news") + ["news.out.kernel", "news.out.bias", "user.attn.WQ", "user.attn.WK",
                                                 "user.attn.WV", "user.att.W", "user.att.b", "user.att.q"]

    def get_weights(self):
        pv, E = self.params.view, self.E
        w = pv("u_Wqkv").cpu().numpy()
        return self.mlp.get_weights() + [pv("out_W").cpu().numpy(), pv("out_b").cpu().numpy(), w[:, :E].copy(), w[:, E:2 * E].copy(),
                                         w[:, 2 * E:].copy(), pv("u_W").cpu().numpy(), pv("u_b").cpu().numpy(),
                                         pv("u_q").cpu().numpy().reshape(-1, 1)]

    def set_weights(self, weights):
        n = 6 * len(self.units) + 8
        if len(weights) != n:
            raise ValueError(f"expected {n} weight arrays, got {len(weights)}")
        w = [torch.from_numpy(np.ascontiguousarray(np.asarray(a, dtype=np.float32))) for a in weights]
        pv = self.params.view
        self.mlp.set_weights(w)
        i = 6 * len(self.units)
        with torch.no_grad():
            pv("out_W").copy_(w[i]); pv("out_b").copy_(w[i + 1])
            pv("u_Wqkv").copy_(torch.cat(w[i + 2:i + 5], dim=1))
            pv("u_W").copy_(w[i + 5]); pv("u_b").copy_(w[i + 6].reshape(-1)); pv("u_q").copy_(w[i + 7].reshape(-1))

    def count_params(self):
        return sum(int(np.prod(s)) for s in self.params.shapes.values()) + 2 * sum(self.units)

    @property
    def learning_rate(self):
        return self._lr

    @learning_rate.setter
    def learning_rate(self, lr):
        self._lr = float(lr)
        st = self.read_state()
        st.lr = self._lr
        self.state.copy_(torch.frombuffer(bytearray(bytes(st)), dtype=torch.uint8))

    def read_state(self):
        return _hip.StepState.from_buffer_copy(self.state.cpu().numpy().tobytes())

    def _mlp_bufs(self, N):
        b = self._bufs.get("mlp")
        if b is None or b["N"] < N:
            f = lambda *s: torch.empty(*s, device=self.device)
            b = {"N": N, "X0": f(N, self.Din), "NE": f(N, self.E), "dNE": f(N, self.E), "dXl": f(N, self.mlp.out_dim),
                 "scores": f(N), "probs": f(N), "labels": f(N)}
            b["partials"] = f(int(_hip.lib().ebn_colsum_partials_len(N, self.E)))
            wsf = _hip.lib().ebn_gemm_workspace_floats
            b["ws"] = f(max(int(wsf(self.mlp.out_dim, self.E, N)), int(wsf(N, self.E, self.mlp.out_dim)), int(wsf(N, self.mlp.out_dim, self.E)), 1))
            self.mlp.bufs(N)
            self._bufs["mlp"] = b
            self._graphs.clear()
        return b

    def _user_bufs(self, B, H=None):
        H = self.H if H is None else int(H)
        key = "user" if H == self.H else ("user", H)
        b = self._bufs.get(key)
        if b is None or b.n_seq < B:
            b = EncoderBuffers(B, H, self.E, self.E, self.A, self.device, own_input=False, need_dx=False)
            b.duser = torch.empty(B, self.E, device=self.device)
            b.loss_rows = torch.empty(B, device=self.device)
            b.head_partials = torch.empty(max(int(_hip.lib().ebn_user_head_partials_len(B, self.A)), 1), device=self.device)
            self._bufs[key] = b
            if H == self.H:
                self._graphs.clear()
        return b

    def _gemm(self, tA, tB, M, N, K, A, lda, B, ldb, beta, C, ldc, ws=None):
        _hip.call("ebn_gemm_f32_ws", tA, tB, M, N, K, ctypes.c_float(1.0), _hip.ptr(A), lda, _hip.ptr(B), ldb,
                  ctypes.c_float(beta), _hip.ptr(C), ldc, _hip.ptr(ws), 0 if ws is None else ws.numel(), _hip.stream_handle())

    def _dvn(self, mb, n_hist, n_cand):
        if self._dvn_dirty:
            for k, v in mb.items():
                if isinstance(k, tuple) and k[0] == "dvn_stat":
                    v.zero_()
            self._dvn_dirty = False
        if not (self.fuse_news_mlp and self.units):
            return None
        fin_args = self._finale_args() if self._finale_live(n_cand // max(n_hist // self.H, 1) if n_hist else 0) else None
        fin = fin_args is not None
        key = ("dvn", n_hist, n_cand, self.p, self.l2, fin)
        a = mb.get(key)
        if a is None:
            L, N, pv, g, b = len(self.units), mb["N"], self.params.view, self.params.g, self.mlp.bufs(mb["N"])
            a = _hip.DvnArgs()
            a.n_layers, a.din, a.e_out, a.n0, a.n1, a.drop_p, a.l2 = L, self.Din, self.E, n_hist, n_cand, self.p, self.l2
            for l, u in enumerate(self.units):
                a.units[l] = u
            if not _hip.lib().ebn_dvn_supported(ctypes.byref(a)):
                mb[key] = False
                return None
            f = lambda *s: torch.empty(*s, device=self.device)
            if "dvn_dY" not in mb:
                mb["dvn_dY"] = [f(N, u) for u in self.units]
                mb["dvn_dP"] = [f(N, u) for u in self.units] + [f(N, self.E)]
            mb[("dvn_stat", n_hist, n_cand, self.p, self.l2, fin)] = stat = torch.zeros(int(_hip.lib().ebn_dvn_stat_floats(ctypes.byref(a))), device=self.device)
            for l in range(L):
                a.W[l], a.b[l] = pv(f"d{l}_W").data_ptr(), pv(f"d{l}_b").data_ptr()
                a.gamma[l], a.beta[l] = pv(f"bn{l}_g").data_ptr(), pv(f"bn{l}_b").data_ptr()
                a.moving_mean[l], a.moving_var[l] = self.bn_mean[l].data_ptr(), self.bn_var[l].data_ptr()
                a.R[l], a.Xn[l] = b["R"][l].data_ptr(), b["Xn"][l].data_ptr()
                a.dY[l], a.dP[l] = mb["dvn_dY"][l].data_ptr(), mb["dvn_dP"][l].data_ptr()
                a.ggamma[l], a.gbeta[l] = g(f"bn{l}_g").data_ptr(), g(f"bn{l}_b").data_ptr()
            a.W[L], a.b[L], a.dP[L] = pv("out_W").data_ptr(), pv("out_b").data_ptr(), mb["dvn_dP"][L].data_ptr()
            a.X0, a.NE, a.dNE, a.stat = mb["X0"].data_ptr(), mb["NE"].data_ptr(), mb["dNE"].data_ptr(), stat.data_ptr()
            a.loss = None if fin else self.loss_dev.data_ptr()
# ... 99 lines not shown
        B, C = his.shape[0], pred.shape[1]
        n_hist, n_cand = B * self.H, B * C
        for arr, r0, n in ((his, 0, n_hist), (pred, n_hist, n_cand)):
            t = arr if isinstance(arr, torch.Tensor) else torch.from_numpy(np.ascontiguousarray(np.asarray(arr, dtype=np.float32)))
            mb["X0"][r0:r0 + n].copy_(t.reshape(n, self.Din).to(device=self.device, dtype=torch.float32), non_blocking=True)
        return n_hist, n_cand

    def _check_shapes(self, his, pred):
        if his.ndim != 3 or his.shape[1] != self.H or his.shape[2] != self.Din:
            raise ValueError(f"his_input_title must be (B, {self.H}, {self.Din}), got {tuple(his.shape)}")
        if pred.ndim != 3 or pred.shape[0] != his.shape[0] or pred.shape[2] != self.Din:
            raise ValueError(f"pred_input_title must be (B, C, {self.Din}), got {tuple(pred.shape)}")

    def encode_news(self, vecs, chunk=65536) -> torch.Tensor:
        vecs = vecs if isinstance(vecs, torch.Tensor) else np.asarray(vecs, dtype=np.float32)
        N = vecs.shape[0]
        out = torch.empty(N, self.E, device=self.device)
        for s in range(0, N, chunk):
            n = min(chunk, N - s)
            mb = self._mlp_bufs(min(chunk, N))
            t = vecs[s:s + n] if isinstance(vecs, torch.Tensor) else torch.from_numpy(np.ascontiguousarray(vecs[s:s + n]))
            mb["X0"][:n].copy_(t.to(device=self.device, dtype=torch.float32))
            self._news_forward(mb, n, 0, False)
            out[s:s + n].copy_(mb["NE"][:n])
        return out

    def encode_users_from_news(self, NEh: torch.Tensor) -> torch.Tensor:
        B, H = NEh.shape[0], NEh.shape[1]
        ub = self._user_bufs(B, H)
        X = NEh.reshape(B * H, self.E).contiguous()
        dims, params, acts = self._enc(ub, B, X)
        _hip.call("ebn_encoder_fwd_f32", ctypes.byref(dims), ctypes.byref(params), ctypes.byref(acts), ctypes.byref(self._fwd_scratch(ub)), None, _hip.stream_handle())
        return ub.out[:B].clone()

    def encode_users(self, his) -> torch.Tensor:
        his = np.asarray(his, dtype=np.float32) if not isinstance(his, torch.Tensor) else his
        B, H = his.shape[0], his.shape[1]
        return self.encode_users_from_news(self.encode_news(his.reshape(B * H, self.Din)).view(B, H, self.E))

    def forward(self, his, pred, mode="softmax"):
        his = his if isinstance(his, torch.Tensor) else np.asarray(his)
        pred = pred if isinstance(pred, torch.Tensor) else np.asarray(pred)
        self._check_shapes(his, pred)
        B, C = his.shape[0], pred.shape[1]
        mb, ub = self._mlp_bufs(B * (self.H + C)), self._user_bufs(B)
        n_hist, n_cand = self._upload(mb, his, pred)
        self._news_forward(mb, n_hist, n_cand, False)
        dims, params, acts = self._enc(ub, B, mb["NE"])
        _hip.call("ebn_encoder_fwd_f32", ctypes.byref(dims), ctypes.byref(params), ctypes.byref(acts), ctypes.byref(self._fwd_scratch(ub)), None, _hip.stream_handle())
        scores, probs = torch.empty(B, C, device=self.device), torch.empty(B, C, device=self.device)
        _hip.call("ebn_score_fwd_f32", _hip.ptr(mb["NE"][n_hist:]), _hip.ptr(ub.out), _hip.ptr(scores), _hip.ptr(probs), B, C,
                  self.E, 0 if mode == "softmax" else 1, _hip.stream_handle())
        return probs, scores

    def eval_loss(self, his, pred, y):
        probs, scores = self.forward(his, pred)
        B, C = scores.shape
        labels = torch.as_tensor(np.asarray(y, dtype=np.float32)).to(self.device).reshape(B, C).contiguous()
        mb, ub = self._mlp_bufs(B * (self.H + C)), self._user_bufs(B)
        rows, jc, ju = torch.empty(B, device=self.device), torch.empty(B * C, self.E, device=self.device), torch.empty(B, self.E, device=self.device)
        loss = torch.empty(1, device=self.device)
        _hip.call("ebn_score_loss_bwd_f32", _hip.ptr(mb["NE"][B * self.H:]), _hip.ptr(ub.out), _hip.ptr(scores), _hip.ptr(labels),
                  _hip.ptr(rows), _hip.ptr(jc), _hip.ptr(ju), B, C, self.E, self.loss_kind, ctypes.c_float(1.0 / B), _hip.stream_handle())
        _hip.call("ebn_sum_f32", _hip.ptr(rows), B, ctypes.c_float(1.0), _hip.ptr(loss), 0, _hip.stream_handle())
        return loss, probs

    def pair_scores(self, user, news, u_idx, n_idx, sigmoid=True):
        n = u_idx.numel()
        out = torch.empty(n, device=self.device)
        _hip.call("ebn_pair_score_f32", _hip.ptr(user), _hip.ptr(news), _hip.ptr(u_idx), _hip.ptr(n_idx), _hip.ptr(out), n,
                  self.E, 1 if sigmoid else 0, _hip.stream_handle())
        return out

    def enable_graphs(self, flag=True):
        self.use_graph = bool(flag)
        if not flag:
            self._graphs = {}
        return self

    def set_article_matrix(self, matrix) -> None:
        m = np.asarray(matrix)
        if m.ndim != 2 or m.shape[1] != self.Din or not np.issubdtype(m.dtype, np.floating):
            raise ValueError(f"article matrix must be float (n_articles+1, {self.Din}), got {m.dtype} {m.shape}")
        self.article_matrix = torch.from_numpy(np.ascontiguousarray(m.astype(np.float32))).to(self.device)
        self._article_matrix_src = matrix
        self._oob = torch.zeros(1, dtype=torch.int32, device=self.device)

    def _stage_indexed(self, mb, his_idx, pred_idx, y=None):
        n = his_idx.shape[0] * (self.H + pred_idx.shape[1])
        if "art_idx" not in mb:
            mb["art_idx"] = torch.empty(mb["N"], dtype=torch.int32, device=self.device)
        same_dev = lambda t: t.is_cuda and (self.device.index is None or t.device.index == self.device.index)
        ok = lambda t, dt: isinstance(t, torch.Tensor) and same_dev(t) and t.dtype == dt and t.is_contiguous()
        if ok(his_idx, torch.int32) and ok(pred_idx, torch.int32) and ok(y, torch.float32):
            _hip.call("ebn_docvec_stage_gather_f32", _hip.ptr(his_idx), his_idx.numel(), _hip.ptr(pred_idx), pred_idx.numel(), _hip.ptr(y),
                      _hip.ptr(mb["labels"]), y.numel(), _hip.ptr(self.article_matrix), self.article_matrix.shape[0], self.Din,
                      _hip.ptr(mb["X0"]), _hip.ptr(self._oob), _hip.ptr(self.state), BETA1, BETA2, _hip.stream_handle())
            self._advanced = True
            return None
        elif not isinstance(his_idx, torch.Tensor) and not isinstance(pred_idx, torch.Tensor) and y is not None and not isinstance(y, torch.Tensor):
            B, C = his_idx.shape[0], pred_idx.shape[1]
            n_lab, tot = B * C, n + B * C
            st = getattr(self, "_host_stage", None)
            if st is None or st["pinned"][0].numel() < tot:
                st = self._host_stage = {"pinned": [torch.empty(2 * tot, dtype=torch.int32).pin_memory() for _ in range(2)],
                                         "dev": torch.empty(2 * tot, dtype=torch.int32, device=self.device), "ev": [None, None], "k": 0}
            k = st["k"] = st["k"] ^ 1
            if st["ev"][k] is not None:
                st["ev"][k].synchronize()
            hs = st["pinned"][k].numpy()
            nh = B * self.H
            hs[:nh] = np.asarray(his_idx).reshape(-1)
            hs[nh:n] = np.asarray(pred_idx).reshape(-1)
            hs[n:tot].view(np.float32)[:] = np.asarray(y, dtype=np.float32).reshape(-1)
            st["dev"][:tot].copy_(st["pinned"][k][:tot], non_blocking=True)
            st["ev"][k] = torch.cuda.Event()
            st["ev"][k].record()
            _hip.call("ebn_docvec_stage_gather_f32", _hip.ptr(st["dev"]), n, None, 0, _hip.ptr(st["dev"][n:]), _hip.ptr(mb["labels"]), n_lab,
                      _hip.ptr(self.article_matrix), self.article_matrix.shape[0], self.Din, _hip.ptr(mb["X0"]), _hip.ptr(self._oob),
                      _hip.ptr(self.state), BETA1, BETA2, _hip.stream_handle())
            self._advanced = True
            return None
        else:
            off = 0
            for a in (his_idx, pred_idx):
                t = a if isinstance(a, torch.Tensor) else torch.from_numpy(np.ascontiguousarray(np.asarray(a).reshape(-1).astype(np.int32, copy=False)))
                t = t.reshape(-1)
                mb["art_idx"][off: off + t.numel()].copy_(t.to(device=self.device, dtype=torch.int32), non_blocking=True)
                off += t.numel()
        _hip.call("ebn_gather_rows_f32", _hip.ptr(mb["art_idx"]), _hip.ptr(self.article_matrix), _hip.ptr(mb["X0"]), n, self.Din,
                  self.article_matrix.shape[0], None, -1, ctypes.c_float(0.0), _hip.ptr(self._oob), _hip.stream_handle())
        return y

    def train_step(self, his, pred, y, return_probs=False, indexed=False):
        his = his if isinstance(his, torch.Tensor) else np.asarray(his)
        pred = pred if isinstance(pred, torch.Tensor) else np.asarray(pred)
        if not indexed:
            self._check_shapes(his, pred)
        elif his.ndim != 2 or his.shape[1] != self.H or pred.ndim != 2 or pred.shape[0] != his.shape[0]:
            raise ValueError(f"indexed batches must be (B, {self.H}) and (B, C), got {tuple(his.shape)} {tuple(pred.shape)}")
        B, C = his.shape[0], pred.shape[1]
        mb, ub = self._mlp_bufs(B * (self.H + C)), self._user_bufs(B)
        self._dvn(mb, B * self.H, B * C)
        self._advanced = False
        if indexed:
            y = self._stage_indexed(mb, his, pred, y)
        else:
            self._upload(mb, his, pred)
        if y is not None:
            labels = (y if isinstance(y, torch.Tensor) else torch.from_numpy(np.ascontiguousarray(np.asarray(y, dtype=np.float32))))
            mb["labels"][: B * C].copy_(labels.reshape(-1).to(device=self.device, dtype=torch.float32))
        if self.use_graph:
            adv = self._advanced
            gkey = (B, C, adv, bool(self.fuse_news_mlp), self.p, self.l2, bool(self.fuse_finale), bool(self.multi))
            g = self._graphs.get(gkey)
            if g is None:
                torch.cuda.synchronize()
                g1, g2 = torch.cuda.CUDAGraph(), torch.cuda.CUDAGraph()
                with _hip.capture(g1):
                    self._fwd_bwd_kernels(B, C, adv)
                if self._step_applied_adam(mb):
                    g2 = None
                else:
                    with _hip.capture(g2, pool=g1.pool()):
                        self._optimizer_kernels()
                g = self._graphs[gkey] = (g1, g2)
            g[0].replay()
            if g[1] is not None:
                self._allreduce_grads()
                g[1].replay()
        else:
            self._fwd_bwd_kernels(B, C, self._advanced)
            if not self._step_applied_adam(mb):
                self._allreduce_grads()
                self._optimizer_kernels()
        if return_probs:
            return self.loss_dev, mb["probs"][: B * C].view(B, C), mb["labels"][: B * C].view(B, C)
        return self.loss_dev

    @staticmethod
    def _step_applied_adam(mb) -> bool:
        a = mb.get("dvn_live")
        return a is not None and a._finale is not None

    def _fwd_bwd_kernels(self, B, C, advanced=False):
        E = self.E
        S = _hip.stream_handle
        mb, ub = self._mlp_bufs(B * (self.H + C)), self._user_bufs(B)
        n_hist, n_cand = B * self.H, B * C
        st = _hip.ptr(self.state)
        if not advanced:
            _hip.call("ebn_step_advance", st, BETA1, BETA2, S())
        self._news_forward(mb, n_hist, n_cand, True)
        a = mb.get("dvn_live")
        if a is not None and a._finale is not None:
            self._user_stage_deferred(B, C, mb, ub)
            self._news_backward(mb, n_hist, n_cand)
            return
        dims, params, acts = self._enc(ub, B, mb["NE"])
        cand = mb["NE"][n_hist:]
        g = self.params.g
        grads = _hip.EncoderGrads(g("u_Wqkv").data_ptr(), g("u_W").data_ptr(), g("u_b").data_ptr(), g("u_q").data_ptr())
        scratch = _hip.EncoderScratch(ub.dY.data_ptr(), ub.dQKV.data_ptr(), ub.de.data_ptr(), ub.partials.data_ptr(),
                                      ub.ws.data_ptr(), ub.ws.numel())
        _hip.call("ebn_user_stage_train_f32", ctypes.byref(dims), ctypes.byref(params), ctypes.byref(acts), _hip.ptr(cand),
                  _hip.ptr(mb["labels"]), _hip.ptr(mb["scores"]), _hip.ptr(mb["probs"]), _hip.ptr(ub.loss_rows), _hip.ptr(self.loss_dev),
                  _hip.ptr(mb["dNE"][n_hist:]), _hip.ptr(ub.duser), ctypes.byref(grads), ctypes.byref(scratch),
                  _hip.ptr(ub.head_partials) if self.fuse_user_head else None, _hip.ptr(mb["dNE"]), C, self.loss_kind,
                  ctypes.c_float(1.0 / B), st, S())
        self._news_backward(mb, n_hist, n_cand)

    def _user_stage_deferred(self, B, C, mb, ub):
        S, H, E, A = _hip.stream_handle, self.H, self.E, self.A
        R = B * H
        pv, g = self.params.view, self.params.g
        ws, wsn = _hip.ptr(ub.ws), ub.ws.numel()
        one, zero = ctypes.c_float(1.0), ctypes.c_float(0.0)
        X, cand, dcand = mb["NE"], mb["NE"][R:], mb["dNE"][R:]
        _hip.call("ebn_gemm_f32_site", 0, 0, R, 3 * E, E, one, _hip.ptr(X), E, _hip.ptr(pv("u_Wqkv")), 3 * E, zero, _hip.ptr(ub.QKV), 3 * E, ws, wsn, 1, S())
        _hip.call("ebn_attn_fwd_f32", _hip.ptr(ub.QKV), 3 * E, _hip.ptr(ub.Y), E, B, H, self.h, self.d, None, -1, zero, S())
        _hip.call("ebn_gemm_f32_ws", 0, 0, R, A, E, one, _hip.ptr(ub.Y), E, _hip.ptr(pv("u_W")), A, zero, _hip.ptr(ub.U), A, ws, wsn, S())
        _hip.call("ebn_user_head_train_f32", _hip.ptr(ub.U), _hip.ptr(pv("u_b")), _hip.ptr(pv("u_q")), _hip.ptr(ub.Y), _hip.ptr(cand), _hip.ptr(mb["labels"]),
                  _hip.ptr(ub.w), _hip.ptr(ub.out), _hip.ptr(mb["scores"]), _hip.ptr(mb["probs"]), _hip.ptr(ub.loss_rows), _hip.ptr(self.loss_dev), _hip.ptr(dcand),
                  _hip.ptr(ub.duser), _hip.ptr(ub.de), None, None, _hip.ptr(ub.head_partials), B, H, C, E, A, self.loss_kind, ctypes.c_float(1.0 / B), S())
        _hip.call("ebn_dense_bwd_pair_f32", R, E, A, _hip.ptr(ub.Y), E, _hip.ptr(ub.U), A, _hip.ptr(pv("u_W")), A, zero, _hip.ptr(g("u_W")), A,
                  _hip.ptr(ub.dY), E, ws, wsn, S())
        _hip.call("ebn_attn_bwd_pooled_f32", _hip.ptr(ub.QKV), 3 * E, _hip.ptr(ub.dY), E, _hip.ptr(ub.w), _hip.ptr(ub.duser), E, _hip.ptr(ub.dQKV), 3 * E,
                  B, H, self.h, self.d, None, -1, zero, S())
        _hip.call("ebn_dense_bwd_pair_f32", R, E, 3 * E, _hip.ptr(X), E, _hip.ptr(ub.dQKV), 3 * E, _hip.ptr(pv("u_Wqkv")), 3 * E, zero, _hip.ptr(g("u_Wqkv")),
                  3 * E, _hip.ptr(mb["dNE"]), E, ws, wsn, S())

    def _allreduce_grads(self):
        if self.multi:
            torch.distributed.all_reduce(self.params.grad, group=self.pg)

    def _optimizer_kernels(self):
        S = _hip.stream_handle
        st = _hip.ptr(self.state)
        P = self.params
        _hip.call("ebn_adam_keras_step_f32", _hip.ptr(P.data), _hip.ptr(P.grad), _hip.ptr(P.m), _hip.ptr(P.v), P.numel, st,
                  BETA1, BETA2, ADAM_EPS, ctypes.c_float(1.0 / self.world), S())

    def roofline_kernels(self, B, C):
        mb = self._mlp_bufs(B * (self.H + C))
        n = B * (self.H + C)
        S = _hip.stream_handle

        def make_gather(rows):
            def gather():
                _hip.call("ebn_gather_rows_f32", _hip.ptr(rows), _hip.ptr(self.article_matrix), _hip.ptr(mb["X0"]), n, self.Din,
                          self.article_matrix.shape[0], None, -1, ctypes.c_float(0.0), _hip.ptr(self._oob), S())

            return gather

        out = {"gather": make_gather}
        a = self._dvn(mb, B * self.H, B * C)
        if a is not None:
            out["dw_group_flops"] = float(sum(2.0 * q.M * q.N * q.K for q in a._probs))
            out["dw_group_bytes"] = float(sum(4.0 * (q.K * (q.M + q.N) + q.M * q.N) for q in a._probs))
            if a._finale is not None:
                P, f = self.params, _hip.DvnFinale()
                ctypes.memmove(ctypes.byref(f), ctypes.byref(a._finale), ctypes.sizeof(f))
                shadow = mb.setdefault("finale_shadow", [P.data.clone(), P.m.clone(), P.v.clone()])
                f.theta, f.m, f.v = (t.data_ptr() for t in shadow)
                ub = self._user_bufs(B)
                f.head_partials, f.loss_rows, f.B = ub.head_partials.data_ptr(), ub.loss_rows.data_ptr(), B
                out["dw_group"] = lambda: _hip.call("ebn_dvn_finale_f32", ctypes.byref(a), a._probs, len(a._probs), ctypes.byref(f), _hip.ptr(self.state), S())
                out["dw_group_bytes"] += 4.0 * 7 * P.numel
                out["dw_group_is_finale"] = True
            else:
                out["dw_group"] = lambda: _hip.call("ebn_gemm_tn_group_f32", a._probs, len(a._probs), S())
        return out

    def check_oob(self):
        oob = getattr(self, "_oob", None)
        flags = torch.cat([oob if oob is not None else torch.zeros(1, dtype=torch.int32, device=self.device), self.range_flag])
        if self.world > 1:
            torch.distributed.all_reduce(flags, op=torch.distributed.ReduceOp.MAX, group=self.pg)
        bad_rows, bad_range = (int(v) != 0 for v in flags.cpu().tolist())
        if bad_rows and oob is not None:
            oob.zero_()
        if bad_range:
            self.range_flag.zero_()
            self._dvn_dirty = True
        if bad_rows:
            raise IndexError(f"article row out of range [0, {self.article_matrix.shape[0]}) for the document-vector matrix")
        if bad_range:
            raise FloatingPointError("a column sum of the news encoder's BatchNormalization left the range of its fixed-point accumulator or was not "
                                     "finite: the run has diverged (fuse_news_mlp=False runs the separate passes, which propagate NaN instead)")

    def sync_moving_statistics(self) -> None:
        if self.world > 1:
            self.mlp.sync_moving_statistics(self.pg)

    def l2_penalty(self) -> float:
        return self.mlp.l2_penalty()

    def extra_state(self):
        return {}
```

ebnerd-benchmark_amd/ebrec/models/newsrec/_engine_segments.py:

```python
from __future__ import annotations

import ctypes

import numpy as np
import torch

from ebrec import _hip

BETA1, BETA2, ADAM_EPS = 0.9, 0.999, 1e-7


def _named(kind, fn, what):
    fn.what = what
    return kind, fn


class SegmentsMixin:
    def _lookup_segments(self, b, N):
        ex, n_tok = self.exchange, N * self.T

        def plan(ids, n, cap, ws, slot_rows, inv, counts):
            _hip.call("ebn_shard_plan_i32", _hip.ptr(ids), n, self.V, ex.world, 1 if ex.cyclic else 0, cap, _hip.ptr(ws),
                      _hip.ptr(slot_rows), _hip.ptr(inv), _hip.ptr(counts), _hip.stream_handle())

        def serve(local_rows, out):
            _hip.call("ebn_gather_rows_f32", _hip.ptr(local_rows), _hip.ptr(self.table), _hip.ptr(out), local_rows.numel(), self.D,
                      self.table.shape[0], None, -1, ctypes.c_float(0.0), None, _hip.stream_handle())

        return ex.lookup_segments(b.ids, n_tok, b.xb, plan, serve)

    def _table_grad_segments(self, b, N):
        ex, n_tok = self.exchange, N * self.T
        site, p = (0, self.p) if self.p > 0 else (-1, 0.0)

        def reduce_local(inv, d_slot):
            d_slot.zero_()
            _hip.call("ebn_embedding_grad_scatter_f32", _hip.ptr(inv), _hip.ptr(b.dX), _hip.ptr(d_slot), n_tok, self.D,
                      d_slot.shape[0], _hip.ptr(self.state), site, ctypes.c_float(p), _hip.stream_handle())

        def accumulate(local_rows, grads):
            self.table_grad.zero_()
            _hip.call("ebn_embedding_grad_scatter_f32", _hip.ptr(local_rows), _hip.ptr(grads), _hip.ptr(self.table_grad),
                      local_rows.numel(), self.D, self.table.shape[0], None, -1, ctypes.c_float(0.0), _hip.stream_handle())

        return ex.grad_segments(n_tok, b.xb, reduce_local, accumulate)

    def _local_gather(self, local_rows: torch.Tensor) -> torch.Tensor:
        m = local_rows.numel()
        out = torch.empty(m, self.D, device=self.device)
        if m:
            _hip.call("ebn_gather_rows_f32", _hip.ptr(local_rows), _hip.ptr(self.table), _hip.ptr(out), m, self.D,
                      self.table.shape[0], None, -1, ctypes.c_float(0.0), _hip.ptr(self.oob_flag), _hip.stream_handle())
        return out

    def _local_scatter_add(self, local_rows: torch.Tensor, grads: torch.Tensor) -> None:
        m = local_rows.numel()
        if m:
            _hip.call("ebn_embedding_grad_scatter_f32", _hip.ptr(local_rows), _hip.ptr(grads), _hip.ptr(self.table_grad),
                      m, self.D, self.table.shape[0], None, -1, ctypes.c_float(0.0), _hip.stream_handle())

    def _state_tensors(self):
        ts = [self.params.data, self.params.grad, self.params.m, self.params.v, self.state, self.loss_dev]
        if self.train_embedding:
            ts += [self.table, self.table_grad, self.table_m, self.table_v] + ([self.table_acc] if self.deterministic else [])
        return ts

    def verify_graph_collectives(self, his, pred, y) -> bool:
        if not (self.use_graph and self.graph_capable and self.multi):
            self.graph_collectives = False
            return False
        if torch.distributed.get_backend(self.pg) != "nccl":
            self.graph_collectives = False
            return False
        torch.cuda.synchronize()
        snap = [t.clone() for t in self._state_tensors()]

        def restore():
            for t, s in zip(self._state_tensors(), snap):
                t.copy_(s)

        def one_step(flag):
            self.graph_collectives = flag
            self._graphs.clear()
            self.train_step(his, pred, y)
            restore()
            self.train_step(his, pred, y)
            torch.cuda.synchronize()
            out = [t.clone() for t in self._state_tensors()]
            restore()
            return out

        ok = True
        try:
            ref = one_step(False)
            got = one_step(True)
            ok = all(torch.equal(a, b) for a, b in zip(ref, got))
        except Exception:
            ok = False
            restore()
        verdict = torch.tensor([1 if ok else 0], dtype=torch.int32, device=self.device)
        torch.distributed.all_reduce(verdict, op=torch.distributed.ReduceOp.MIN, group=self.pg)
        self.graph_collectives = bool(int(verdict.item()))
        self._graphs.clear()
        return self.graph_collectives

    def _graph_key(self, B, C, advanced=False):
        return (B, C, advanced, bool(self.adam_in_finish), bool(self.defer_finish), bool(self.multi))

    def _capture(self, B, C, advanced=False):
        torch.cuda.synchronize()
        key = self._graph_key(B, C, advanced)
        segs, run, pool, i = self._segments(B, C, advanced), [], None, 0
        desc = self.__dict__.setdefault("_graph_desc", {}).setdefault(key, [])
        desc.clear()
        if self.graph_collectives and self.multi:
            g = torch.cuda.CUDAGraph()
            with _hip.capture(g):
                for _kind, fn in segs:
                    fn()
            self._graph_objs = getattr(self, "_graph_objs", []) + [g]
            self._graphs[key] = [g.replay]
            desc.append("ONE hipGraph: " + " | ".join(self.SEG_KINDS[k] for k, _fn in segs))
            return self._graphs[key]
        while i < len(segs):
            if segs[i][0] != "k":
                run.append(segs[i][1])
                desc.append(f"{self.SEG_KINDS[segs[i][0]]}: {getattr(segs[i][1], 'what', 'unnamed')} (segment {i} of the step's {len(segs)})")
                i += 1
                continue
            j = i
            while j < len(segs) and segs[j][0] == "k":
                j += 1
            g = torch.cuda.CUDAGraph()
            with _hip.capture(g, pool=pool):
                for _kind, fn in segs[i:j]:
                    fn()
            pool = pool or g.pool()
            run.append(g.replay)
            desc.append(f"hipGraph replay of kernel segments {i}..{j - 1} of the step's {len(segs)}")
            self._graph_objs = getattr(self, "_graph_objs", []) + [g]
            i = j
        self._graphs[key] = run
        return run

    def _segments(self, B, C, advanced=False):
        N = B * (self.H + C)
        nb, _ub = self._train_bufs(B, C)
        multi = self.multi
        segs = [] if advanced else [("k", lambda: _hip.call("ebn_step_advance", _hip.ptr(self.state), BETA1, BETA2, _hip.stream_handle()))]
        if self._planned:
            segs += self._lookup_segments(nb, N)
        sparse = self._sparse_dp(N * self.T)
        if multi and self.mlp is None and self.overlap_collectives and self.train_embedding:
            segs.append(("k", lambda: (self._fwd_bwd_kernels(B, C, sparse, part="a"), self._fwd_bwd_kernels(B, C, sparse, part="b"))))
            segs.append(_named("a", lambda: self._allreduce_async(self.params.grad), "all-reduce of the flat dense-gradient bucket"))
            segs.append(("k", lambda: self._fwd_bwd_kernels(B, C, sparse, part="c")))
            if self._planned:
                segs += self._table_grad_segments(nb, N)
            if self.exchange is None and not sparse:
                segs.append(_named("c", lambda: self._allreduce_table_grad(), "all-reduce of the dense (V, D) table gradient"))
            if sparse:
                segs += self._sparse_table_grad_segments(nb, N)
            segs.append(("w", self._wait_collectives))
        else:
            segs.append(("k", lambda: self._fwd_bwd_kernels(B, C, sparse)))
            if self._planned and self.train_embedding:
                segs += self._table_grad_segments(nb, N)
            if multi:
                segs.append(_named("c", lambda: self._allreduce_grads(dense_table=not sparse),
                                   "all-reduce of the flat dense-gradient bucket" + (" and of the dense table gradient" if (self.train_embedding and self.exchange is None and not sparse) else "")))
            if sparse:
                segs += self._sparse_table_grad_segments(nb, N)
        segs.append(("k", lambda: self._optimizer_kernels(from_acc=self._adam_from_acc or sparse)))
        return segs

    def _allreduce_async(self, t):
        if self.multi and not self.skip_collectives:
            self._pending.append(torch.distributed.all_reduce(t, group=self.pg, async_op=True))

    def _wait_collectives(self):
        for w in self._pending:
            w.wait()
        self._pending = []

    def _allreduce_table_grad(self):
        if self.multi and not self.skip_collectives:
            torch.distributed.all_reduce(self.table_grad, group=self.pg)

    def _sparse_table_grad_segments(self, nb, N):
        n_tok, W = N * self.T, self.world
        if getattr(nb, "ids_all", None) is None or nb.ids_all.numel() < W * n_tok:
            nb.ids_all = torch.empty(W * nb.n_seq * self.T, dtype=torch.int32, device=self.device)
            nb.dX_all = torch.empty(W * nb.n_seq * self.T, self.D, device=self.device)
        ids_all, dX_all = nb.ids_all[: W * n_tok], nb.dX_all[: W * n_tok]
        site, p = (0, self.p) if self.p > 0 else (-1, 0.0)

        def gather():
            if self.skip_collectives:
                return
            torch.distributed.all_gather_into_tensor(ids_all, nb.ids[:n_tok], group=self.pg)
            torch.distributed.all_gather_into_tensor(dX_all, nb.dX[:n_tok], group=self.pg)

        def accumulate():
            for r in range(W):
                self._accumulate_fixed(ids_all[r * n_tok:], dX_all[r * n_tok:], n_tok, _hip.ptr(self.state), site, p)

        return [_named("c", gather, "all-gather of the per-token (id, gradient row) pairs (sparse table-gradient exchange)"), ("k", accumulate)]

    def _allreduce_grads(self, dense_table=True):
        if self.multi and not self.skip_collectives:
            torch.distributed.all_reduce(self.params.grad, group=self.pg)
            if self.train_embedding and self.exchange is None and dense_table:
                torch.distributed.all_reduce(self.table_grad, group=self.pg)
```

include/ebnerd_hip.h:

```cpp
#ifndef EBNERD_HIP_H
#define EBNERD_HIP_H

#include <stdint.h>

#ifdef __cplusplus
extern "C" {
#endif

#define EBN_ABI_VERSION 1

#define EBN_OK 0
#define EBN_ERR_BAD_ARG (-1)
#define EBN_ERR_UNSUPPORTED (-2)
#define EBN_ERR_ALIGN (-3)

typedef void* ebn_stream_t;

#define EBN_SITE_NEWS_IN 0
#define EBN_SITE_NEWS_ATT 1
#define EBN_SITE_MLP0 8
#define EBN_N_SITES 12

typedef struct ebn_step_state {
  uint32_t step;
  uint32_t seed;
  float adam_alpha;
  float lr;
  uint32_t drop_key[EBN_N_SITES];
} ebn_step_state;

int ebn_abi_version(void);
const char* ebn_error_string(int code);
int64_t ebn_launch_count(void);

int ebn_step_advance(ebn_step_state* st, double beta1, double beta2, ebn_stream_t stream);

int ebn_gather_rows_f32(const int32_t* ids, const float* table, float* out, int64_t n_tok,
                        int32_t D, int64_t V, const ebn_step_state* st, int32_t site,
                        float drop_p, int32_t* oob_flag, ebn_stream_t stream);

int ebn_expand_titles_i32(const int32_t* art_idx, const int32_t* token_matrix, int32_t* ids_out,
                          int64_t n_titles, int32_t T, int64_t n_rows, int32_t* oob_flag,
                          ebn_stream_t stream);

int ebn_embedding_grad_scatter_f32(const int32_t* ids, const float* dX, float* dTable,
                                   int64_t n_tok, int32_t D, int64_t V,
                                   const ebn_step_state* st, int32_t site, float drop_p,
                                   ebn_stream_t stream);

int ebn_embedding_grad_scatter_fixed(const int32_t* ids, const float* dX, int64_t* acc, int64_t n_tok,
                                     int32_t D, int64_t V, const ebn_step_state* st, int32_t site,
                                     float drop_p, int32_t* range_flag, ebn_stream_t stream);
int ebn_embedding_grad_scatter_fixed_atomic(const int32_t* ids, const float* dX, int64_t* acc, int64_t n_tok,
                                            int32_t D, int64_t V, const ebn_step_state* st, int32_t site,
                                            float drop_p, int32_t* range_flag, ebn_stream_t stream);
int ebn_fixed_to_f32(int64_t* acc, float* out, int64_t n, int32_t* range_flag, ebn_stream_t stream);
int ebn_adam_keras_step_fixed_f32(float* theta, int64_t* acc, float* m, float* v, int64_t n, const ebn_step_state* st,
                                  double beta1, double beta2, double eps, float grad_scale, int32_t* range_flag,
                                  ebn_stream_t stream);

int64_t ebn_gemm_split_workspace_bytes(int64_t M, int64_t N, int64_t K);
int ebn_gemm_f32_split(int32_t transA, int32_t transB, int64_t M, int64_t N, int64_t K, float alpha, const float* A,
                       int64_t lda, const float* B, int64_t ldb, float beta, float* C, int64_t ldc, void* workspace,
                       int64_t workspace_bytes, ebn_stream_t stream);
int64_t ebn_planes_bytes(int64_t rows, int64_t K);
int ebn_split_planes_f32(const float* src, int64_t ld, int64_t rows, int64_t K, int32_t trans, void* planes,
                         ebn_stream_t stream);
int ebn_gather_split_planes_f32(const int32_t* ids, const float* table, int64_t n_rows, int32_t D, int64_t V,
                                const ebn_step_state* st, int32_t site, float drop_p, int32_t* oob_flag, void* planes_n,
                                void* planes_t, ebn_stream_t stream);
int64_t ebn_gemm_planes_workspace_floats(int64_t M, int64_t N, int64_t K);
int ebn_gemm_planes_f32(const void* a_planes, int64_t M, const void* b_planes, int64_t N, int64_t K, float alpha, float beta,
                        float* C, int64_t ldc, float* workspace, int64_t workspace_floats, ebn_stream_t stream);
int64_t ebn_gemm_prec_workspace_bytes(int64_t M, int64_t N, int64_t K, int32_t precision);
int ebn_gemm_f32_prec(int32_t transA, int32_t transB, int64_t M, int64_t N, int64_t K, float alpha, const float* A,
                      int64_t lda, const float* B, int64_t ldb, float beta, float* C, int64_t ldc, void* workspace,
                      int64_t workspace_bytes, int32_t precision, ebn_stream_t stream);

int64_t ebn_shard_plan_workspace_ints(int64_t V, int32_t world);
int ebn_shard_plan_i32(const int32_t* ids, int64_t n_tok, int64_t V, int32_t world, int32_t cyclic, int64_t cap,
                       int32_t* workspace, int32_t* slot_rows, int32_t* inv, int32_t* counts, ebn_stream_t stream);

int ebn_gemm_f32(int32_t transA, int32_t transB, int64_t M, int64_t N, int64_t K, float alpha,
                 const float* A, int64_t lda, const float* B, int64_t ldb, float beta, float* C,
                 int64_t ldc, ebn_stream_t stream);
int64_t ebn_gemm_workspace_floats(int64_t M, int64_t N, int64_t K);
int ebn_gemm_plan(int64_t M, int64_t N, int64_t K, int64_t workspace_floats, int32_t* bm, int32_t* bn, int32_t* splits);
int ebn_gemm_f32_ws(int32_t transA, int32_t transB, int64_t M, int64_t N, int64_t K, float alpha,
                    const float* A, int64_t lda, const float* B, int64_t ldb, float beta, float* C,
                    int64_t ldc, float* workspace, int64_t workspace_floats, ebn_stream_t stream);

int64_t ebn_gemm_partials_workspace_floats(int64_t M, int64_t N, int64_t K);
int ebn_gemm_f32_partials(int32_t transA, int32_t transB, int64_t M, int64_t N, int64_t K, float alpha, const float* A,
                          int64_t lda, const float* B, int64_t ldb, float* workspace, int64_t workspace_floats,
                          int32_t* n_parts, ebn_stream_t stream);

#define EBN_FINISH_SPLITK 0
#define EBN_FINISH_COLRED 1
#define EBN_FINISH_HEAD 2
#define EBN_FINISH_MAX_JOBS 6
typedef struct {
  int32_t kind;
  int32_t n_parts;
  int64_t rows, cols;
  const float* partials;
  float* out0;
  float* out1;
  int64_t ld;
  float beta, scale;
  const float* loss_rows;
  float* loss_out;
} ebn_finish_job;
int ebn_grad_finish_f32(const ebn_finish_job* jobs, int32_t n_jobs, ebn_stream_t stream);

#define EBN_ADAM_FLAT_MAX_REST 12
typedef struct ebn_adam_flat {
  float* theta;
  const float* grad;
  float* m;
  float* v;
  int64_t numel;
  double beta1, beta2, eps;
  float grad_scale;
  int32_t n_rest;
  int64_t rest_off[EBN_ADAM_FLAT_MAX_REST];
  int64_t rest_len[EBN_ADAM_FLAT_MAX_REST];
} ebn_adam_flat;
int ebn_grad_finish_adam_f32(const ebn_finish_job* jobs, int32_t n_jobs, const ebn_adam_flat* adam, const ebn_step_state* st,
                             ebn_stream_t stream);

int ebn_gemm_f32_site(int32_t transA, int32_t transB, int64_t M, int64_t N, int64_t K, float alpha,
                      const float* A, int64_t lda, const float* B, int64_t ldb, float beta, float* C,
                      int64_t ldc, float* workspace, int64_t workspace_floats, int32_t site,
                      ebn_stream_t stream);

int ebn_attn_fwd_f32(const float* qkv, int64_t ld_qkv, float* out, int64_t ld_out, int64_t n_seq,
                     int32_t L, int32_t h, int32_t d, const ebn_step_state* st, int32_t site,
                     float drop_p, ebn_stream_t stream);
int ebn_attn_bwd_f32(const float* qkv, int64_t ld_qkv, const float* dout, int64_t ld_dout,
                     float* dqkv, int64_t ld_dqkv, int64_t n_seq, int32_t L, int32_t h, int32_t d,
                     const ebn_step_state* st, int32_t site, float drop_p, ebn_stream_t stream);
int ebn_attn_bwd_pooled_f32(const float* qkv, int64_t ld_qkv, const float* dout, int64_t ld_dout, const float* pool_w,
                            const float* pool_dout, int64_t ld_pool, float* dqkv, int64_t ld_dqkv, int64_t n_seq,
                            int32_t L, int32_t h, int32_t d, const ebn_step_state* st, int32_t site, float drop_p,
                            ebn_stream_t stream);
int ebn_attn_bwd_pooled_supported(int32_t L, int32_t d);

int ebn_gemm_f32_rank1(int64_t M, int64_t N, int64_t K, float alpha, const float* A, int64_t lda, const float* B,
                       int64_t ldb, float* C, int64_t ldc, const float* row_scale, const float* seq_rows,
                       int64_t ld_seq, int32_t L, float* workspace, int64_t workspace_floats, ebn_stream_t stream);

int ebn_dense_bwd_pair_f32(int64_t R, int64_t K_in, int64_t N_out, const float* X, int64_t ldx, const float* dY,
                           int64_t lddy, const float* W, int64_t ldw, float beta_w, float* dW, int64_t lddw, float* dX,
                           int64_t lddx, float* workspace, int64_t workspace_floats, ebn_stream_t stream);

int ebn_dense_relu_fwd_f32(int64_t M, int64_t N, int64_t K, const float* A, int64_t lda, const float* B, int64_t ldb,
                           const float* bias, float* C, int64_t ldc, float* workspace, int64_t workspace_floats,
                           ebn_stream_t stream);

int ebn_attpool_fwd_f32(float* U, const float* b, const float* q, const float* X, float* out,
                        float* w, int64_t n_seq, int32_t L, int32_t E, int32_t A,
                        ebn_stream_t stream);
int ebn_attpool_bwd_pool_f32(const float* X, const float* w, const float* dout, float* dX,
                             float* de, int64_t n_seq, int32_t L, int32_t E,
                             ebn_stream_t stream);
int64_t ebn_attpool_partials_len(int64_t R, int32_t A);
int ebn_attpool_bwd_dpre_f32(float* U, const float* q, const float* de, float* dq, float* db,
                             float* partials, int64_t R, int32_t A, int32_t accumulate,
                             ebn_stream_t stream);
typedef struct ebn_encoder_dims {
  int64_t n_seq;
  int32_t L;
  int32_t Din;
  int32_t h, d;
  int32_t A;
  int32_t drop_site;
  float drop_p;
} ebn_encoder_dims;

typedef struct ebn_encoder_params {
  const float* Wqkv;
  const float* W;
  const float* b;
  const float* q;
} ebn_encoder_params;

typedef struct ebn_encoder_acts {
  const float* X;
  float* QKV;
  float* Y;
  float* U;
  float* w;
  float* out;
} ebn_encoder_acts;

typedef struct ebn_encoder_grads {
  float* dWqkv;
  float* dW;
  float* db;
  float* dq;
} ebn_encoder_grads;

typedef struct ebn_encoder_scratch {
  float* dY;
  float* dQKV;
  float* de;
  float* partials;
  float* gemm_ws;
  int64_t gemm_ws_floats;
} ebn_encoder_scratch;

int ebn_encoder_fwd_f32(const ebn_encoder_dims* dims, const ebn_encoder_params* params,
                        const ebn_encoder_acts* acts, const ebn_encoder_scratch* scratch,
                        const ebn_step_state* st, ebn_stream_t stream);
int ebn_encoder_fwd_gather_f32(const ebn_encoder_dims* dims, const ebn_encoder_params* params, const ebn_encoder_acts* acts,
                               const ebn_encoder_scratch* scratch, const int32_t* ids, const float* table, int64_t table_rows,
                               int32_t* oob_flag, ebn_stream_t stream);
int ebn_gemm_f32_rowmap(const int32_t* ids, int64_t table_rows, int64_t M, int64_t N, int64_t K, const float* table,
                        int64_t ldt, const float* B, int64_t ldb, float* C, int64_t ldc, int32_t* oob_flag, ebn_stream_t stream);

int ebn_encoder_bwd_f32(const ebn_encoder_dims* dims, const ebn_encoder_params* params,
                        const ebn_encoder_acts* acts, const float* dout,
                        const ebn_encoder_grads* grads, const ebn_encoder_scratch* scratch,
                        float* dX, int32_t accumulate, const ebn_step_state* st,
                        ebn_stream_t stream);

int ebn_user_stage_train_f32(const ebn_encoder_dims* dims, const ebn_encoder_params* p, const ebn_encoder_acts* a,
                             const float* cand, const float* labels, float* scores, float* probs, float* loss_rows,
                             float* loss_out, float* dcand, float* duser, const ebn_encoder_grads* g,
                             const ebn_encoder_scratch* s, float* head_partials, float* dX, int32_t C, int32_t loss_kind,
                             float inv_batch, const ebn_step_state* st, ebn_stream_t stream);

int ebn_score_fwd_f32(const float* cand, const float* user, float* scores, float* probs,
                      int64_t B, int32_t C, int32_t E, int32_t mode, ebn_stream_t stream);
int ebn_score_loss_bwd_f32(const float* cand, const float* user, const float* scores,
                           const float* labels, float* loss_rows, float* dcand, float* duser,
                           int64_t B, int32_t C, int32_t E, int32_t loss_kind, float inv_batch,
                           ebn_stream_t stream);
int ebn_score_loss_train_f32(const float* cand, const float* user, const float* labels, float* scores, float* probs,
                             float* loss_rows, float* loss_out, float* dcand, float* duser, int64_t B, int32_t C,
                             int32_t E, int32_t loss_kind, float inv_batch, ebn_stream_t stream);
int ebn_user_head_supported(int32_t L, int32_t C, int32_t E, int32_t A);
int64_t ebn_user_head_partials_len(int64_t B, int32_t A);
int ebn_user_head_train_f32(float* U, const float* b, const float* q, const float* X, const float* cand, const float* labels,
                            float* w, float* user, float* scores, float* probs, float* loss_rows, float* loss_out,
                            float* dcand, float* duser, float* de, float* dq, float* db, float* partials, int64_t B,
                            int32_t L, int32_t C, int32_t E, int32_t A, int32_t loss_kind, float inv_batch,
                            ebn_stream_t stream);
int ebn_auc_hist_f32(const float* probs, const float* labels, int64_t n, const double* thresholds, int32_t n_thresholds,
                     int64_t* pos_hist, int64_t* neg_hist, ebn_stream_t stream);
int ebn_pair_score_f32(const float* user, const float* news, const int32_t* u_idx,
                       const int32_t* n_idx, float* out, int64_t n_pairs, int32_t E, int32_t mode,
                       ebn_stream_t stream);

int ebn_adam_keras_step_f32(float* theta, const float* g, float* m, float* v, int64_t n,
                            const ebn_step_state* st, double beta1, double beta2, double eps,
                            float grad_scale, ebn_stream_t stream);

int ebn_bias_relu_f32(const float* X, const float* bias, float* Y, int64_t R, int32_t Ccols,
                      ebn_stream_t stream);
int64_t ebn_colsum_partials_len(int64_t R, int32_t Ccols);
int ebn_bias_relu_bwd_f32(const float* Y, const float* dY, float* dX, float* dbias,
                          float* partials, int64_t R, int32_t Ccols, int32_t accumulate,
                          ebn_stream_t stream);
int ebn_batchnorm_fwd_f32(const float* X, const float* gamma, const float* beta,
                          float* moving_mean, float* moving_var, float* Y, float* xhat,
                          float* mean_out, float* istd_out, float* partials, int64_t R,
                          int32_t Ccols, int32_t training, const ebn_step_state* st,
                          int32_t site, float drop_p, int64_t elem_offset,
                          ebn_stream_t stream);
int ebn_batchnorm_bwd_f32(const float* dY, const float* xhat, const float* gamma,
                          const float* istd, float* dX, float* dgamma, float* dbeta,
                          float* partials, int64_t R, int32_t Ccols, int32_t training,
                          int32_t accumulate, const ebn_step_state* st, int32_t site,
                          float drop_p, int64_t elem_offset, ebn_stream_t stream);
int ebn_batchnorm2_fwd_f32(const float* X, const float* gamma, const float* beta, float* moving_mean, float* moving_var,
                           float* Y, float* xhat, float* mean_out0, float* istd_out0, float* mean_out1, float* istd_out1,
                           int64_t R0, int64_t R1, int32_t Ccols, const ebn_step_state* st, int32_t site, float drop_p,
                           ebn_stream_t stream);
int ebn_batchnorm2_relu_bwd_f32(const float* dY, const float* xhat, const float* relu_out, const float* gamma,
                                const float* istd0, const float* istd1, float* dX, float* dgamma, float* dbeta,
                                float* dbias, int64_t R0, int64_t R1, int32_t Ccols, const ebn_step_state* st, int32_t site,
                                float drop_p, ebn_stream_t stream);

#define EBN_DVN_MAX_LAYERS 4
typedef struct ebn_dvn_args {
  int32_t n_layers, din, e_out;
  int32_t units[EBN_DVN_MAX_LAYERS];
  int32_t n0, n1;
  float drop_p, l2;
  const float* W[EBN_DVN_MAX_LAYERS + 1];
  const float* b[EBN_DVN_MAX_LAYERS + 1];
  const float* gamma[EBN_DVN_MAX_LAYERS];
  const float* beta[EBN_DVN_MAX_LAYERS];
  float* moving_mean[EBN_DVN_MAX_LAYERS];
  float* moving_var[EBN_DVN_MAX_LAYERS];
  const float* X0;
  float* R[EBN_DVN_MAX_LAYERS];
  float* Xn[EBN_DVN_MAX_LAYERS];
  float* NE;
  float* stat;
  const float* dNE;
  float* dY[EBN_DVN_MAX_LAYERS];
  float* dP[EBN_DVN_MAX_LAYERS + 1];
  float* ggamma[EBN_DVN_MAX_LAYERS];
  float* gbeta[EBN_DVN_MAX_LAYERS];
  float* loss;
  int32_t* range_flag;
} ebn_dvn_args;
int ebn_dvn_supported(const ebn_dvn_args* args);
int64_t ebn_dvn_stat_floats(const ebn_dvn_args* args);
int ebn_dvn_fwd_train_f32(const ebn_dvn_args* args, const ebn_step_state* st, ebn_stream_t stream);
int ebn_dvn_bwd_f32(const ebn_dvn_args* args, const ebn_step_state* st, ebn_stream_t stream);

int ebn_docvec_stage_gather_f32(const int32_t* idx0, int64_t n0, const int32_t* idx1, int64_t n1, const float* labels_src,
                                float* labels_dst, int64_t n_labels, const float* matrix, int64_t n_rows, int32_t din, float* X0,
                                int32_t* oob_flag, ebn_step_state* st, double beta1, double beta2, ebn_stream_t stream);

#define EBN_TN_GROUP_MAX 8
typedef struct ebn_tn_problem {
  int64_t M, N, K;
  const float* A;
  int64_t lda;
  const float* B;
  int64_t ldb;
  float* C;
  int64_t ldc;
  float* colsum;
  const float* l2_W;
  float two_lambda;
} ebn_tn_problem;
int ebn_gemm_tn_group_f32(const ebn_tn_problem* problems, int32_t n, ebn_stream_t stream);

#define EBN_DVN_FINALE_MAX_REST 12
typedef struct ebn_dvn_finale {
  float* theta;
  const float* grad;
  float* m;
  float* v;
  int64_t numel;
  double beta1, beta2, eps;
  float grad_scale;
  int32_t n_rest;
  int64_t rest_off[EBN_DVN_FINALE_MAX_REST];
  int64_t rest_len[EBN_DVN_FINALE_MAX_REST];
  const float* head_partials;
  int64_t B;
  int32_t A;
  float* dq;
  float* db;
  const float* loss_rows;
  float* loss_out;
} ebn_dvn_finale;
int ebn_dvn_finale_f32(const ebn_dvn_args* args, const ebn_tn_problem* problems, int32_t n, const ebn_dvn_finale* fin,
                       const ebn_step_state* st, ebn_stream_t stream);

#define EBN_SITE_NPA_CONV 2
#define EBN_SITE_NPA_NEWS_PAP 3
#define EBN_SITE_NPA_USER_PAP 4

int ebn_conv1d_fwd_f32(const float* X, const float* W, const float* bias, float* Vd, int64_t n_titles, int32_t T, int32_t E,
                       int32_t F, int32_t window, const ebn_step_state* st, int32_t conv_site, float conv_p, int32_t pap_site,
                       float pap_p, ebn_stream_t stream);
int ebn_conv1d_bwd_data_f32(const float* dVd, const float* Vd, const float* W, float* dX, int64_t n_titles, int32_t T, int32_t E,
                            int32_t F, int32_t window, const ebn_step_state* st, float conv_p, float pap_p, ebn_stream_t stream);
int ebn_conv1d_wgrad_splits(int64_t n_titles, int32_t T, int32_t E, int32_t F, int32_t window);
int64_t ebn_conv1d_wgrad_workspace_floats(int64_t n_titles, int32_t T, int32_t E, int32_t F, int32_t window, int32_t splits);
int ebn_conv1d_bwd_weight_f32(const float* X, const float* dVd, const float* Vd, float* partials, int32_t splits, int64_t n_titles,
                              int32_t T, int32_t E, int32_t F, int32_t window, const ebn_step_state* st, float conv_p, float pap_p,
                              ebn_stream_t stream);

int ebn_pap_fwd_f32(float* U, const float* ba, const float* Q, const int32_t* q_idx, int64_t n_q, const float* V, float* out,
                    float* w, float* out_d, int64_t n_drop, int64_t n_seq, int32_t L, int32_t F, int32_t A,
                    const ebn_step_state* st, int32_t site, float drop_p, ebn_stream_t stream);
int ebn_pap_bwd_f32(float* U, const float* Q, const int32_t* q_idx, int64_t n_q, const float* V, const float* w, float* dout,
                    float* dV, float* dq, int64_t n_drop, int64_t n_seq, int32_t L, int32_t F, int32_t A,
                    const ebn_step_state* st, int32_t site, float drop_p, ebn_stream_t stream);
int ebn_pap_dq_reduce_f32(const float* dq, const int32_t* q_idx, int64_t n_seq, float* dQ, int64_t n_q, int32_t A,
                          ebn_stream_t stream);
// ... 122 lines not shown
```

Baseline: 25490.

## Fuse user-encoder dY projection into attention backward and batch three backward GEMMs

Adds a user-attention backward kernel that computes dY = dU·Wᵀ with MFMA inside each wave, adds the pooled term, and stores it straight to LDS, so the separate dX GEMM and its dY round trip through global memory are gone. A new trio GEMM kernel then launches dWqkv, dX and dW in a single grid instead of a pair call plus a separate dispatch. The fused path is taken by default when the shape checks pass, otherwise it falls back to the old path. Graph cache keys now include the fusion flags. The cost is redundant work: every head recomputes its dY slice over the full A reduction, and trio eligibility depends on all three problems fitting the small-tile plan.

```diff
diff --git a/ebnerd-benchmark_amd/csrc/ebn_attention_mfma.hip b/ebnerd-benchmark_amd/csrc/ebn_attention_mfma.hip
--- a/ebnerd-benchmark_amd/csrc/ebn_attention_mfma.hip
+++ b/ebnerd-benchmark_amd/csrc/ebn_attention_mfma.hip
@@ -444,6 +444,53 @@
   return 3 * L * Tile<D>::STRIDE > L * Tile<D>::STRIDE + TP_FLOATS ? 3 * L * Tile<D>::STRIDE : L * Tile<D>::STRIDE + TP_FLOATS;
 }
 
+template <int D>
+__device__ __forceinline__ void bwd_wave_from_lds(float* __restrict__ sq, float* __restrict__ sk, float* __restrict__ sg,
+                                                  const float (&vr)[D / 2], float* __restrict__ ob, uint32_t ld_out, int E, int L,
+                                                  int row, int hi) {
+  constexpr int KH = D / 2;
+  const float inv = 1.0f / sqrtf(static_cast<float>(D));
+  const float inv2 = inv * 1.44269504088896341f;
+  f32x16 P, dP;
+  {
+    float qr[KH], kr[KH];
+    lds_row_form<D>(qr, sq, L, row, hi);
+    lds_row_form<D>(kr, sk, L, row, hi);
+    P = mm_rows<KH>(kr, qr);
+  }
+  softmax_in_lane(P, L, hi, inv2);
+  {
+    float gr[KH];
+    lds_row_form<D>(gr, sg, L, row, hi);
+    dP = mm_rows<KH>(gr, vr);
+  }
+  float rowdot = 0.f;
+#pragma unroll
+  for (int r = 0; r < 16; ++r) rowdot = fmaf(P[r], dP[r], rowdot);
+  rowdot += __shfl_xor(rowdot, 32, 64);
+
+  float col[16];
+  lds_col_form<D>(col, sg, L, row, hi);
+  {
+    const f32x16 dV = mm_col_tile(col, P);
+    tile_rows_to_global<D, false>(ob + 2 * E, ld_out, dV, L, row, hi, 1.0f, 0u, 0u, 0, 0u, 0.f);
+  }
+#pragma unroll
+  for (int r = 0; r < 16; ++r) P[r] = P[r] * (dP[r] - rowdot);
+  lds_col_form<D>(col, sk, L, row, hi);
+  {
+    const f32x16 dQ = mm_col_tile(col, P);
+    tile_rows_to_global<D, false>(ob, ld_out, dQ, L, row, hi, inv, 0u, 0u, 0, 0u, 0.f);
+  }
+  wave_lds_sync();
+  tile_transpose(P, sk, L, row, hi);
+  lds_col_form<D>(col, sq, L, row, hi);
+  {
+    const f32x16 dK = mm_col_tile(col, P);
+    tile_rows_to_global<D, false>(ob + E, ld_out, dK, L, row, hi, inv, 0u, 0u, 0, 0u, 0.f);
+  }
+}
+
 template <int D, int LC>
 __global__ __launch_bounds__(64 * ATT_WAVES) void attn_mfma_bwd_kernel(MfmaAttnArgs a) {
   using T = Tile<D>;
@@ -459,8 +506,6 @@
   float* sk = sq + region;
   float* sg = sk + region;
   const int row = lane & 31, hi = lane >> 5;
-  const float inv = 1.0f / sqrtf(static_cast<float>(D));
-  const float inv2 = inv * 1.44269504088896341f;
   const bool drop = a.key_ptr != nullptr, pooled = a.pool_w != nullptr;
   const uint32_t key = drop ? *a.key_ptr : 0u;
 
@@ -484,46 +529,96 @@
     else stage_store<D, false>(sg, tg, L, lane, 0u, 0u, 0, 0u, 0.f);
   }
   wave_lds_sync();
-
-  float* ob = a.out + p.row0 * a.ld_out + p.head * D;
-  f32x16 P, dP;
-  {
-    float qr[KH], kr[KH];
-    lds_row_form<D>(qr, sq, L, row, hi);
-    lds_row_form<D>(kr, sk, L, row, hi);
-    P = mm_rows<KH>(kr, qr);
-  }
-  softmax_in_lane(P, L, hi, inv2);
-  {
-    float gr[KH];
-    lds_row_form<D>(gr, sg, L, row, hi);
-    dP = mm_rows<KH>(gr, vr);
-  }
-  float rowdot = 0.f;
-#pragma unroll
-  for (int r = 0; r < 16; ++r) rowdot = fmaf(P[r], dP[r], rowdot);
-  rowdot += __shfl_xor(rowdot, 32, 64);
-
-  float col[16];
-  lds_col_form<D>(col, sg, L, row, hi);
-  {
-    const f32x16 dV = mm_col_tile(col, P);
-    tile_rows_to_global<D, false>(ob + 2 * E, a.ld_out, dV, L, row, hi, 1.0f, 0u, 0u, 0, 0u, 0.f);
-  }
-#pragma unroll
-  for (int r = 0; r < 16; ++r) P[r] = P[r] * (dP[r] - rowdot);
-  lds_col_form<D>(col, sk, L, row, hi);
-  {
-    const f32x16 dQ = mm_col_tile(col, P);
-    tile_rows_to_global<D, false>(ob, a.ld_out, dQ, L, row, hi, inv, 0u, 0u, 0, 0u, 0.f);
-  }
-  wave_lds_sync();
-  tile_transpose(P, sk, L, row, hi);
-  lds_col_form<D>(col, sq, L, row, hi);
-  {
-    const f32x16 dK = mm_col_tile(col, P);
-    tile_rows_to_global<D, false>(ob + E, a.ld_out, dK, L, row, hi, inv, 0u, 0u, 0, 0u, 0.f);
-  }
+  bwd_wave_from_lds<D>(sq, sk, sg, vr, a.out + p.row0 * a.ld_out + p.head * D, a.ld_out, E, L, row, hi);
+}
+
+struct UserAttnBwdArgs {
+  const float* qkv;
+  int64_t ld_qkv;
+  const float* dpre;
+  int64_t ld_dpre;
+  const float* w_att;
+  int64_t ld_w;
+  const float* pool_w;
+  const float* pool_d;
+  int64_t ld_pool;
+  float* dqkv;
+  int64_t ld_dqkv;
+  int64_t n_prob;
+  int32_t L, h, A;
+};
+
+constexpr int UAB_BATCH = 5;
+
+template <int D, int LC>
+__global__ __launch_bounds__(64 * ATT_WAVES) void user_attn_bwd_kernel(UserAttnBwdArgs a) {
+  using T = Tile<D>;
+  constexpr int KH = D / 2;
+  extern __shared__ __attribute__((aligned(16))) float smem[];
+  const int lane = threadIdx.x & 63;
+  const int wv = __builtin_amdgcn_readfirstlane(threadIdx.x >> 6);
+  const int64_t prob = static_cast<int64_t>(xcd_chunked_block()) * ATT_WAVES + wv;
+  if (prob >= a.n_prob) return;
+  const int L = LC ? LC : a.L, E = a.h * D, A = a.A;
+  const int region = L * T::STRIDE;
+  float* sq = smem + wv * bwd_wave_floats<D>(L);
+  float* sk = sq + region;
+  float* sg = sk + region;
+  const int row = lane & 31, hi = lane >> 5;
+
+  const AttnProb p = attn_prob(prob, a.h, L);
+  const float* qb = a.qkv + p.row0 * a.ld_qkv + p.head * D;
+  float vr[KH];
+  Staged<D> tq, tk;
+  stage_load<D>(tq, qb, a.ld_qkv, L, lane);
+  stage_load<D>(tk, qb + E, a.ld_qkv, L, lane);
+  global_row_form<D>(vr, qb + 2 * E, a.ld_qkv, L, row, hi);
+
+  f32x16 dY;
+#pragma unroll
+  for (int r = 0; r < 16; ++r) dY[r] = 0.f;
+  {
+    const float* xp = a.dpre + p.row0 * a.ld_dpre + static_cast<uint32_t>(row < L ? row : 0) * static_cast<uint32_t>(a.ld_dpre);
+    const float* wp = a.w_att + static_cast<int64_t>(p.head * D + (row < D ? row : 0)) * a.ld_w;
+    for (int k0 = 0; k0 < A; k0 += 8 * UAB_BATCH) {
+      float4 xv[UAB_BATCH], wv4[UAB_BATCH];
+#pragma unroll
+      for (int t = 0; t < UAB_BATCH; ++t) {
+        const int k = k0 + 8 * t + 4 * hi;
+        const bool ok = k < A;
+        xv[t] = *reinterpret_cast<const float4*>(xp + (ok ? k : 0));
+        wv4[t] = *reinterpret_cast<const float4*>(wp + (ok ? k : 0));
+        if (!ok) xv[t] = wv4[t] = make_float4(0.f, 0.f, 0.f, 0.f);
+      }
+#pragma unroll
+      for (int t = 0; t < UAB_BATCH; ++t) {
+        dY = __builtin_amdgcn_mfma_f32_32x32x2f32(wv4[t].x, xv[t].x, dY, 0, 0, 0);
+        dY = __builtin_amdgcn_mfma_f32_32x32x2f32(wv4[t].y, xv[t].y, dY, 0, 0, 0);
+        dY = __builtin_amdgcn_mfma_f32_32x32x2f32(wv4[t].z, xv[t].z, dY, 0, 0, 0);
+        dY = __builtin_amdgcn_mfma_f32_32x32x2f32(wv4[t].w, xv[t].w, dY, 0, 0, 0);
+      }
+    }
+  }
+  {
+    const float w = a.pool_w[p.row0 + (row < L ? row : 0)];
+    const float* pd = a.pool_d + p.seq * a.ld_pool + p.head * D;
+#pragma unroll
+    for (int g = 0; g < 4; ++g) {
+      const int c0 = 8 * g + 4 * hi;
+      if (c0 < D) {
+        const float4 v = *reinterpret_cast<const float4*>(pd + c0);
+        dY[4 * g] = fmaf(w, v.x, dY[4 * g]);
+        dY[4 * g + 1] = fmaf(w, v.y, dY[4 * g + 1]);
+        dY[4 * g + 2] = fmaf(w, v.z, dY[4 * g + 2]);
+        dY[4 * g + 3] = fmaf(w, v.w, dY[4 * g + 3]);
+      }
+    }
+  }
+  stage_store<D, false>(sq, tq, L, lane, 0u, 0u, 0, 0u, 0.f);
+  stage_store<D, false>(sk, tk, L, lane, 0u, 0u, 0, 0u, 0.f);
+  tile_rows_to_lds<D>(sg, dY, L, row, hi, 1.0f);
+  wave_lds_sync();
+  bwd_wave_from_lds<D>(sq, sk, sg, vr, a.dqkv + p.row0 * a.ld_dqkv + p.head * D, a.ld_dqkv, E, L, row, hi);
 }
 
 
@@ -1076,3 +1171,51 @@
   EBN_CHECK_LAUNCH();
   return EBN_OK;
 }
+
+static size_t user_attn_bwd_lds(int32_t L, int32_t d) {
+  const int f = d == 16 ? bwd_wave_floats<16>(L) : d == 20 ? bwd_wave_floats<20>(L) : bwd_wave_floats<32>(L);
+  return static_cast<size_t>(ATT_WAVES) * f * sizeof(float);
+}
+
+extern "C" int ebn_user_attn_bwd_supported(int32_t L, int32_t h, int32_t d, int32_t A) {
+  return (L > 0 && L <= 32 && h > 0 && (d == 16 || d == 20 || d == 32) && A > 0 && (A % 4) == 0) ? 1 : 0;
+}
+
+extern "C" int64_t ebn_user_attn_bwd_grid(int64_t n_seq, int32_t h) {
+  return (ebn_dim_ok(n_seq, h) && n_seq * h < (int64_t{1} << 31)) ? ebn_ceil_div(n_seq * h, ATT_WAVES) : 0;
+}
+
+extern "C" int64_t ebn_user_attn_bwd_lds_bytes(int32_t L, int32_t d) {
+  return (L > 0 && L <= 32 && (d == 16 || d == 20 || d == 32)) ? static_cast<int64_t>(user_attn_bwd_lds(L, d)) : 0;
+}
+
+extern "C" int ebn_user_attn_bwd_f32(const float* qkv, int64_t ld_qkv, const float* dpre, int64_t ld_dpre, const float* w_att,
+                                     int64_t ld_w, const float* pool_w, const float* pool_dout, int64_t ld_pool, float* dqkv,
+                                     int64_t ld_dqkv, int64_t n_seq, int32_t L, int32_t h, int32_t d, int32_t A,
+                                     ebn_stream_t stream) {
+  EBN_REQUIRE(n_seq >= 0 && L > 0 && h > 0 && d > 0 && A > 0, EBN_ERR_BAD_ARG);
+  if (n_seq == 0) return EBN_OK;
+  EBN_REQUIRE(qkv && dpre && w_att && pool_w && pool_dout && dqkv, EBN_ERR_BAD_ARG);
+  const int64_t E = static_cast<int64_t>(h) * d;
+  EBN_REQUIRE(ld_qkv >= 3 * E && ld_dqkv >= 3 * E && ld_dpre >= A && ld_w >= A && ld_pool >= E, EBN_ERR_BAD_ARG);
+  const bool ok = ebn_user_attn_bwd_supported(L, h, d, A) != 0 && mfma_path_ok(L, d, ld_qkv, ld_dpre, ld_dqkv, qkv, dpre, dqkv) &&
+                  (ld_w % 4) == 0 && (ld_pool % 4) == 0 && ld_w < (1 << 24) && ebn_aligned16(w_att) && ebn_aligned16(pool_dout) &&
+                  n_seq * h < (int64_t{1} << 31);
+  EBN_REQUIRE(ok, EBN_ERR_UNSUPPORTED);
+  const UserAttnBwdArgs a{qkv, ld_qkv, dpre, ld_dpre, w_att, ld_w, pool_w, pool_dout, ld_pool, dqkv, ld_dqkv, n_seq * h, L, h, A};
+  const dim3 grid(static_cast<unsigned>(ebn_user_attn_bwd_grid(n_seq, h))), block(64 * ATT_WAVES);
+  const size_t lds = user_attn_bwd_lds(L, d);
+  hipStream_t s = ebn_stream(stream);
+#define EBN_UAB(DD, LL)                                             \
+  do {                                                              \
+    allow_lds(user_attn_bwd_kernel<DD, LL>, lds);                   \
+    EBN_LAUNCH((user_attn_bwd_kernel<DD, LL>), grid, block, lds, s, a); \
+  } while (0)
+  if (d == 16) EBN_UAB(16, 0);
+  else if (d == 20 && L == 20) EBN_UAB(20, 20);
+  else if (d == 20) EBN_UAB(20, 0);
+  else EBN_UAB(32, 0);
+#undef EBN_UAB
+  EBN_CHECK_LAUNCH();
+  return EBN_OK;
+}
diff --git a/ebnerd-benchmark_amd/csrc/ebn_encoder.hip b/ebnerd-benchmark_amd/csrc/ebn_encoder.hip
--- a/ebnerd-benchmark_amd/csrc/ebn_encoder.hip
+++ b/ebnerd-benchmark_amd/csrc/ebn_encoder.hip
@@ -90,6 +90,13 @@
   return EBN_OK;
 }
 
+extern "C" int ebn_user_stage_fused_supported(int32_t L, int32_t C, int32_t h, int32_t d, int32_t A) {
+  if (L <= 0 || C <= 0 || h <= 0 || d <= 0 || A <= 0 || h > INT32_MAX / d) return 0;
+  const int32_t E = h * d;
+  return (ebn_user_head_supported(L, C, E, A) != 0 && ebn_attn_bwd_pooled_supported(L, d) != 0 &&
+          ebn_user_attn_bwd_supported(L, h, d, A) != 0 && (E % 4) == 0) ? 1 : 0;
+}
+
 extern "C" int ebn_user_stage_train_f32(const ebn_encoder_dims* dims, const ebn_encoder_params* p, const ebn_encoder_acts* a,
                                         const float* cand, const float* labels, float* scores, float* probs, float* loss_rows,
                                         float* loss_out, float* dcand, float* duser, const ebn_encoder_grads* g,
@@ -121,6 +128,12 @@
   EBN_TRY(ebn_gemm_f32_ws(0, 0, R, A, E, 1.0f, a->Y, E, p->W, A, 0.0f, a->U, A, ws, ws_n, stream));
   EBN_TRY(ebn_user_head_train_f32(a->U, p->b, p->q, a->Y, cand, labels, a->w, a->out, scores, probs, loss_rows, loss_out, dcand,
                                   duser, s->de, g->dq, g->db, head_partials, B, L, C, E, A, loss_kind, inv_batch, stream));
+  if (ebn_user_stage_fused_supported(L, C, dims->h, dims->d, A) != 0 && dims->Din % 4 == 0 && ebn_aligned16(p->W) &&
+      ebn_aligned16(p->Wqkv) && ebn_aligned16(a->X)) {
+    EBN_TRY(ebn_user_attn_bwd_f32(a->QKV, 3 * E, a->U, A, p->W, A, a->w, duser, E, s->dQKV, 3 * E, B, L, dims->h, dims->d, A, stream));
+    return ebn_dense_bwd_trio_f32(R, dims->Din, 3 * E, a->X, dims->Din, s->dQKV, 3 * E, p->Wqkv, 3 * E, g->dWqkv, 3 * E, dX, dims->Din,
+                                  E, A, a->Y, E, a->U, A, g->dW, A, ws, ws_n, stream);
+  }
   EBN_TRY(ebn_dense_bwd_pair_f32(R, E, A, a->Y, E, a->U, A, p->W, A, 0.0f, g->dW, A, s->dY, E, ws, ws_n, stream));
   EBN_TRY(ebn_attn_bwd_pooled_f32(a->QKV, 3 * E, s->dY, E, a->w, duser, E, s->dQKV, 3 * E, B, L, dims->h, dims->d, nullptr, -1, 0.0f,
                                   stream));
diff --git a/ebnerd-benchmark_amd/csrc/ebn_gemm.hip b/ebnerd-benchmark_amd/csrc/ebn_gemm.hip
--- a/ebnerd-benchmark_amd/csrc/ebn_gemm.hip
+++ b/ebnerd-benchmark_amd/csrc/ebn_gemm.hip
@@ -904,6 +904,20 @@
                                     (b - p0.tiles) % p1.tiles_x, (b - p0.tiles) / p1.tiles_x);
 }
 
+__global__ __launch_bounds__(GEMM_THREADS) void gemm_small_trio_kernel(SmallProblem p0, SmallProblem p1, SmallProblem p2) {
+  const GemmEpi none{nullptr, nullptr, 0, 1, nullptr};
+  const int b = blockIdx.x;
+  if (b < p1.tiles) {
+    small_vec_body<false, true, 32>(p1.M, p1.N, p1.K, p1.alpha, p1.A, p1.lda, p1.B, p1.ldb, p1.beta, p1.C, p1.ldc, none,
+                                    b % p1.tiles_x, b / p1.tiles_x);
+  } else {
+    const bool first = b - p1.tiles < p0.tiles;
+    const SmallProblem& p = first ? p0 : p2;
+    const int t = b - p1.tiles - (first ? 0 : p0.tiles);
+    small_vec_body<true, false, 32>(p.M, p.N, p.K, p.alpha, p.A, p.lda, p.B, p.ldb, p.beta, p.C, p.ldc, none, t % p.tiles_x, t / p.tiles_x);
+  }
+}
+
 struct SmallGroup {
   SmallProblem p[EBN_TN_GROUP_MAX];
   float* colsum[EBN_TN_GROUP_MAX];
@@ -1312,6 +1326,44 @@
   return gemm_dispatch(0, 1, R, K_in, N_out, 1.0f, dY, lddy, W, ldw, 0.0f, dX, lddx, workspace, workspace_floats, 0, none, s);
 }
 
+extern "C" int ebn_dense_bwd_trio_f32(int64_t R, int64_t K_in, int64_t N_out, const float* X, int64_t ldx, const float* dY,
+                                      int64_t lddy, const float* W, int64_t ldw, float* dW, int64_t lddw, float* dX, int64_t lddx,
+                                      int64_t K2, int64_t N2, const float* X2, int64_t ldx2, const float* dY2, int64_t lddy2,
+                                      float* dW2, int64_t lddw2, float* workspace, int64_t workspace_floats, ebn_stream_t stream) {
+  EBN_REQUIRE(R >= 0 && K_in >= 0 && N_out >= 0 && K2 >= 0 && N2 >= 0, EBN_ERR_BAD_ARG);
+  const bool have2 = K2 > 0 && N2 > 0;
+  if (have2) EBN_REQUIRE(X2 && dY2 && dW2 && ldx2 >= K2 && lddy2 >= N2 && lddw2 >= N2, EBN_ERR_BAD_ARG);
+  const int64_t ws_n = workspace ? workspace_floats : 0;
+  const int64_t ld2 = ldx2 > lddy2 ? ldx2 : lddy2, ld1 = ldx > lddy ? ldx : lddy;
+  const bool one = have2 && K_in > 0 && N_out > 0 && R > 0 && X && dY && W && dW && dX && ldx >= K_in && lddy >= N_out && ldw >= N_out &&
+                   lddw >= N_out && lddx >= K_in && (ldx % 4) == 0 && (lddy % 4) == 0 && (ldw % 4) == 0 && (ldx2 % 4) == 0 &&
+                   (lddy2 % 4) == 0 && ebn_aligned16(X) && ebn_aligned16(dY) && ebn_aligned16(W) && ebn_aligned16(X2) &&
+                   ebn_aligned16(dY2) && (K_in % 4) == 0 && (N_out % 4) == 0 && (K2 % 4) == 0 && (N2 % 4) == 0 &&
+                   gemm_plan(K_in, N_out, R, ws_n).bm == 32 && gemm_plan(R, K_in, N_out, ws_n).bm == 32 &&
+                   gemm_plan(K2, N2, R, ws_n).bm == 32 &&
+                   (R + SBK) * ld1 * 4 + 64 * (ld1 > ldw ? ld1 : ldw) * 4 < (int64_t{1} << 31) && (R + SBK) * ld2 * 4 < (int64_t{1} << 31);
+  if (!one) {
+    const int rc = ebn_dense_bwd_pair_f32(R, K_in, N_out, X, ldx, dY, lddy, W, ldw, 0.0f, dW, lddw, dX, lddx, workspace, workspace_floats, stream);
+    if (rc != EBN_OK || !have2) return rc;
+    return gemm_dispatch(1, 0, K2, N2, R, 1.0f, X2, ldx2, dY2, lddy2, 0.0f, dW2, lddw2, workspace, workspace_floats, 0,
+                         GemmEpi{nullptr, nullptr, 0, 1, nullptr}, ebn_stream(stream));
+  }
+  hipStream_t s = ebn_stream(stream);
+  SmallProblem p0{K_in, N_out, R, 1.0f, X, ldx, dY, lddy, 0.0f, dW, lddw, static_cast<int32_t>(ebn_ceil_div(N_out, SBN)), 0};
+  p0.tiles = p0.tiles_x * static_cast<int32_t>(ebn_ceil_div(K_in, SBM));
+  SmallProblem p1{R, K_in, N_out, 1.0f, dY, lddy, W, ldw, 0.0f, dX, lddx, static_cast<int32_t>(ebn_ceil_div(K_in, SBN)), 0};
+  p1.tiles = p1.tiles_x * static_cast<int32_t>(ebn_ceil_div(R, SBM));
+  SmallProblem p2{K2, N2, R, 1.0f, X2, ldx2, dY2, lddy2, 0.0f, dW2, lddw2, static_cast<int32_t>(ebn_ceil_div(N2, SBN)), 0};
+  p2.tiles = p2.tiles_x * static_cast<int32_t>(ebn_ceil_div(K2, SBM));
+  constexpr size_t lds = static_cast<size_t>(2) * 2 * SBM * SLV * sizeof(float);
+  static const hipError_t attr = hipFuncSetAttribute(reinterpret_cast<const void*>(&gemm_small_trio_kernel),
+                                                     hipFuncAttributeMaxDynamicSharedMemorySize, static_cast<int>(lds));
+  if (attr != hipSuccess) return static_cast<int>(attr);
+  EBN_LAUNCH(gemm_small_trio_kernel, dim3(static_cast<unsigned>(p0.tiles + p1.tiles + p2.tiles)), dim3(GEMM_THREADS), lds, s, p0, p1, p2);
+  EBN_CHECK_LAUNCH();
+  return EBN_OK;
+}
+
 extern "C" int ebn_gemm_f32_rowmap(const int32_t* ids, int64_t table_rows, int64_t M, int64_t N, int64_t K, const float* table,
                                    int64_t ldt, const float* B, int64_t ldb, float* C, int64_t ldc, int32_t* oob_flag, ebn_stream_t stream) {
   EBN_REQUIRE(ebn_dim_ok(M, N, K) && table_rows > 0, EBN_ERR_BAD_ARG);
diff --git a/ebnerd-benchmark_amd/ebrec/models/newsrec/_engine.py b/ebnerd-benchmark_amd/ebrec/models/newsrec/_engine.py
--- a/ebnerd-benchmark_amd/ebrec/models/newsrec/_engine.py
+++ b/ebnerd-benchmark_amd/ebrec/models/newsrec/_engine.py
@@ -178,6 +178,7 @@
         self.loss_dev = torch.zeros(1, device=self.device)
         self.use_graph = False
         self.fuse_user_head = True
+        self.fuse_user_stage = True
         self.fuse_eval_gather = True
         self.defer_finish = True
         self.atomic_table_grad = False
@@ -878,6 +879,12 @@
         _hip.call("ebn_user_head_train_f32", _hip.ptr(ub.U), _hip.ptr(pv("u_b")), _hip.ptr(pv("u_q")), _hip.ptr(ub.Y), _hip.ptr(cand), _hip.ptr(nb.labels),
                   _hip.ptr(ub.w), _hip.ptr(ub.out), _hip.ptr(nb.scores), _hip.ptr(nb.probs), _hip.ptr(ub.loss_rows), _hip.ptr(self.loss_dev), _hip.ptr(dcand),
                   _hip.ptr(ub.duser), _hip.ptr(ub.de), None, None, _hip.ptr(ub.head_partials), B, H, C, E, A, self.loss_kind, ctypes.c_float(1.0 / B), S())
+        if self.fuse_user_stage and int(_hip.lib().ebn_user_stage_fused_supported(H, C, self.h, self.d, A)) != 0:
+            _hip.call("ebn_user_attn_bwd_f32", _hip.ptr(ub.QKV), 3 * E, _hip.ptr(ub.U), A, _hip.ptr(pv("u_W")), A, _hip.ptr(ub.w), _hip.ptr(ub.duser), E,
+                      _hip.ptr(ub.dQKV), 3 * E, B, H, self.h, self.d, A, S())
+            _hip.call("ebn_dense_bwd_trio_f32", R, E, 3 * E, _hip.ptr(X), E, _hip.ptr(ub.dQKV), 3 * E, _hip.ptr(pv("u_Wqkv")), 3 * E, _hip.ptr(g("u_Wqkv")),
+                      3 * E, _hip.ptr(nb.dNE), E, E, A, _hip.ptr(ub.Y), E, _hip.ptr(ub.U), A, _hip.ptr(g("u_W")), A, ws, wsn, S())
+            return
         _hip.call("ebn_dense_bwd_pair_f32", R, E, A, _hip.ptr(ub.Y), E, _hip.ptr(ub.U), A, _hip.ptr(pv("u_W")), A, zero, _hip.ptr(g("u_W")), A,
                   _hip.ptr(ub.dY), E, ws, wsn, S())
         _hip.call("ebn_attn_bwd_pooled_f32", _hip.ptr(ub.QKV), 3 * E, _hip.ptr(ub.dY), E, _hip.ptr(ub.w), _hip.ptr(ub.duser), E, _hip.ptr(ub.dQKV), 3 * E,
diff --git a/ebnerd-benchmark_amd/ebrec/models/newsrec/_engine_docvec.py b/ebnerd-benchmark_amd/ebrec/models/newsrec/_engine_docvec.py
--- a/ebnerd-benchmark_amd/ebrec/models/newsrec/_engine_docvec.py
+++ b/ebnerd-benchmark_amd/ebrec/models/newsrec/_engine_docvec.py
@@ -31,6 +31,7 @@
         self.params = FlatParams(shapes, self.device)
         self.use_graph, self._graphs = False, {}
         self.fuse_user_head = True
+        self.fuse_user_stage = True
         self.fuse_news_mlp = True
         self.fuse_finale = True
         self._dvn_dirty = False
@@ -436,7 +437,8 @@
             mb["labels"][: B * C].copy_(labels.reshape(-1).to(device=self.device, dtype=torch.float32))
         if self.use_graph:
             adv = self._advanced
-            gkey = (B, C, adv, bool(self.fuse_news_mlp), self.p, self.l2, bool(self.fuse_finale), bool(self.multi))
+            gkey = (B, C, adv, bool(self.fuse_news_mlp), self.p, self.l2, bool(self.fuse_finale), bool(self.multi), bool(self.fuse_user_head),
+                    bool(self.fuse_user_stage))
             g = self._graphs.get(gkey)
             if g is None:
                 torch.cuda.synchronize()
@@ -507,6 +509,12 @@
         _hip.call("ebn_user_head_train_f32", _hip.ptr(ub.U), _hip.ptr(pv("u_b")), _hip.ptr(pv("u_q")), _hip.ptr(ub.Y), _hip.ptr(cand), _hip.ptr(mb["labels"]),
                   _hip.ptr(ub.w), _hip.ptr(ub.out), _hip.ptr(mb["scores"]), _hip.ptr(mb["probs"]), _hip.ptr(ub.loss_rows), _hip.ptr(self.loss_dev), _hip.ptr(dcand),
                   _hip.ptr(ub.duser), _hip.ptr(ub.de), None, None, _hip.ptr(ub.head_partials), B, H, C, E, A, self.loss_kind, ctypes.c_float(1.0 / B), S())
+        if self.fuse_user_stage and int(_hip.lib().ebn_user_stage_fused_supported(H, C, self.h, self.d, A)) != 0:
+            _hip.call("ebn_user_attn_bwd_f32", _hip.ptr(ub.QKV), 3 * E, _hip.ptr(ub.U), A, _hip.ptr(pv("u_W")), A, _hip.ptr(ub.w), _hip.ptr(ub.duser), E,
+                      _hip.ptr(ub.dQKV), 3 * E, B, H, self.h, self.d, A, S())
+            _hip.call("ebn_dense_bwd_trio_f32", R, E, 3 * E, _hip.ptr(X), E, _hip.ptr(ub.dQKV), 3 * E, _hip.ptr(pv("u_Wqkv")), 3 * E, _hip.ptr(g("u_Wqkv")),
+                      3 * E, _hip.ptr(mb["dNE"]), E, E, A, _hip.ptr(ub.Y), E, _hip.ptr(ub.U), A, _hip.ptr(g("u_W")), A, ws, wsn, S())
+            return
         _hip.call("ebn_dense_bwd_pair_f32", R, E, A, _hip.ptr(ub.Y), E, _hip.ptr(ub.U), A, _hip.ptr(pv("u_W")), A, zero, _hip.ptr(g("u_W")), A,
                   _hip.ptr(ub.dY), E, ws, wsn, S())
         _hip.call("ebn_attn_bwd_pooled_f32", _hip.ptr(ub.QKV), 3 * E, _hip.ptr(ub.dY), E, _hip.ptr(ub.w), _hip.ptr(ub.duser), E, _hip.ptr(ub.dQKV), 3 * E,
diff --git a/ebnerd-benchmark_amd/ebrec/models/newsrec/_engine_segments.py b/ebnerd-benchmark_amd/ebrec/models/newsrec/_engine_segments.py
--- a/ebnerd-benchmark_amd/ebrec/models/newsrec/_engine_segments.py
+++ b/ebnerd-benchmark_amd/ebrec/models/newsrec/_engine_segments.py
@@ -105,7 +105,8 @@
         return self.graph_collectives
 
     def _graph_key(self, B, C, advanced=False):
-        return (B, C, advanced, bool(self.adam_in_finish), bool(self.defer_finish), bool(self.multi))
+        return (B, C, advanced, bool(self.adam_in_finish), bool(self.defer_finish), bool(self.multi), bool(self.fuse_user_head),
+                bool(self.fuse_user_stage))
 
     def _capture(self, B, C, advanced=False):
         torch.cuda.synchronize()
diff --git a/include/ebnerd_hip.h b/include/ebnerd_hip.h
--- a/include/ebnerd_hip.h
+++ b/include/ebnerd_hip.h
@@ -145,6 +145,12 @@
                             int32_t L, int32_t h, int32_t d, const ebn_step_state* st, int32_t site, float drop_p,
                             ebn_stream_t stream);
 int ebn_attn_bwd_pooled_supported(int32_t L, int32_t d);
+int ebn_user_attn_bwd_supported(int32_t L, int32_t h, int32_t d, int32_t A);
+int64_t ebn_user_attn_bwd_grid(int64_t n_seq, int32_t h);
+int64_t ebn_user_attn_bwd_lds_bytes(int32_t L, int32_t d);
+int ebn_user_attn_bwd_f32(const float* qkv, int64_t ld_qkv, const float* dpre, int64_t ld_dpre, const float* w_att, int64_t ld_w,
+                          const float* pool_w, const float* pool_dout, int64_t ld_pool, float* dqkv, int64_t ld_dqkv,
+                          int64_t n_seq, int32_t L, int32_t h, int32_t d, int32_t A, ebn_stream_t stream);
 
 int ebn_gemm_f32_rank1(int64_t M, int64_t N, int64_t K, float alpha, const float* A, int64_t lda, const float* B,
                        int64_t ldb, float* C, int64_t ldc, const float* row_scale, const float* seq_rows,
@@ -153,6 +159,10 @@
 int ebn_dense_bwd_pair_f32(int64_t R, int64_t K_in, int64_t N_out, const float* X, int64_t ldx, const float* dY,
                            int64_t lddy, const float* W, int64_t ldw, float beta_w, float* dW, int64_t lddw, float* dX,
                            int64_t lddx, float* workspace, int64_t workspace_floats, ebn_stream_t stream);
+int ebn_dense_bwd_trio_f32(int64_t R, int64_t K_in, int64_t N_out, const float* X, int64_t ldx, const float* dY, int64_t lddy,
+                           const float* W, int64_t ldw, float* dW, int64_t lddw, float* dX, int64_t lddx, int64_t K2, int64_t N2,
+                           const float* X2, int64_t ldx2, const float* dY2, int64_t lddy2, float* dW2, int64_t lddw2,
+                           float* workspace, int64_t workspace_floats, ebn_stream_t stream);
 
 int ebn_dense_relu_fwd_f32(int64_t M, int64_t N, int64_t K, const float* A, int64_t lda, const float* B, int64_t ldb,
                            const float* bias, float* C, int64_t ldc, float* workspace, int64_t workspace_floats,
@@ -225,6 +235,7 @@
                         float* dX, int32_t accumulate, const ebn_step_state* st,
                         ebn_stream_t stream);
 
+int ebn_user_stage_fused_supported(int32_t L, int32_t C, int32_t h, int32_t d, int32_t A);
 int ebn_user_stage_train_f32(const ebn_encoder_dims* dims, const ebn_encoder_params* p, const ebn_encoder_acts* a,
                              const float* cand, const float* labels, float* scores, float* probs, float* loss_rows,
                              float* loss_out, float* dcand, float* duser, const ebn_encoder_grads* g,
```

After: 25540, median of 5. No clear change (+0.2%).
